# matiasrodlo/arxiv-rag

Hardware: AMD Instinct MI355X
Metric: chunks embedded/sec + QPS@top-10, all-mpnet-base-v2 768-d, 1/2/4/8 MI355X (higher is better)
Workload: dtype bf16

## Files before the change

### arxiv_rag_amd/_lib.py

```python
from __future__ import annotations

import ctypes as C
import os
from pathlib import Path

_HERE = Path(__file__).resolve().parent
LIB_PATH = Path(os.environ.get("ARX_LIB", _HERE / "libarx_hip.so"))

K_CLASSES = ["search_groupmax", "gemm_qkv", "gemm_oproj", "gemm_fc1", "gemm_fc2", "attention",
             "layernorm", "embed", "pool", "search_select", "search_rescore", "gemm_raw"]


class EncoderConfigC(C.Structure):
    _fields_ = [(n, C.c_int32) for n in ("arch", "vocab_size", "hidden", "layers", "heads", "ffn", "max_pos",
                                         "pool", "pad_id", "rel_buckets", "rel_max_distance")] + [("ln_eps", C.c_float)]


class LayerWeightsC(C.Structure):
    _fields_ = [(n, C.c_void_p) for n in ("w_qkv", "b_qkv", "w_o", "b_o", "ln1_g", "ln1_b",
                                          "w_fc1", "b_fc1", "w_fc2", "b_fc2", "ln2_g", "ln2_b")]


class EncoderWeightsC(C.Structure):
    _fields_ = [(n, C.c_void_p) for n in ("word_emb", "pos_emb", "type_emb", "emb_ln_g", "emb_ln_b", "rel_bias")] \
               + [("layers", C.POINTER(LayerWeightsC))]


class TopkOptionsC(C.Structure):
    _fields_ = [("struct_bytes", C.c_int32), ("i8_max_queries", C.c_int32), ("max_row_norm", C.c_float), ("cu_limit", C.c_int32),
                ("flags", C.c_int32), ("debug_tau_mult", C.c_float), ("debug_drop_best", C.c_int32)]

    def __init__(self, **kw):
        super().__init__(**kw)
        self.struct_bytes = C.sizeof(TopkOptionsC)


class EncoderOptionsC(C.Structure):
    _fields_ = [("struct_bytes", C.c_int32), ("gemm_schedule", C.c_int32), ("attn_kernel", C.c_int32), ("flags", C.c_int32)]

    def __init__(self, **kw):
        super().__init__(**kw)
        self.struct_bytes = C.sizeof(EncoderOptionsC)


class PairHeadC(C.Structure):
    _fields_ = [("struct_bytes", C.c_int32), ("n_labels", C.c_int32)] \
               + [(n, C.c_void_p) for n in ("type_emb", "pooler_w", "pooler_b", "cls_w", "cls_b")]

    def __init__(self, **kw):
        super().__init__(**kw)
        self.struct_bytes = C.sizeof(PairHeadC)


class GemmEpilogueC(C.Structure):
    _fields_ = [("struct_bytes", C.c_int32), ("mode", C.c_int32), ("variant", C.c_int32), ("eps", C.c_float)] \
               + [(n, C.c_void_p) for n in ("bias", "resid", "a_mean", "a_rstd", "s_vec", "r_mean", "r_rstd", "r_gamma", "r_beta")] \
               + [("row_cap", C.c_int64), ("part_sum", C.c_void_p), ("part_sq", C.c_void_p), ("part_ld", C.c_int64),
                  ("out_mean", C.c_void_p), ("out_rstd", C.c_void_p), ("n_rows", C.c_void_p)]

    def __init__(self, **kw):
        super().__init__(**kw)
        self.struct_bytes = C.sizeof(GemmEpilogueC)


class FacetKeyC(C.Structure):
    _fields_ = [("kind", C.c_void_p), ("val", C.c_void_p), ("cuts", C.c_void_p), ("mode", C.c_int32), ("want_kind", C.c_int32),
                ("n_bins", C.c_int32), ("reserved", C.c_int32), ("out_off", C.c_int64)]


FACET_CODE, FACET_EXACT, FACET_INTERVAL = 0, 1, 2
TOPK_NO_PERSISTENT, TOPK_SCAN_ONLY, TOPK_TAIL_ONLY, TOPK_NO_SINGLE_ROW_TAIL, TOPK_I8_CENTRE_QUERY = 1, 2, 4, 8, 16
GEMM_DEFAULT, GEMM_PER_TILE, GEMM_PERSISTENT, GEMM_2STAGE, GEMM_SPLIT_K, GEMM_TILE_128 = 89, 8, 9, 13, 70, 71
ATTN_TRANSPOSED, ATTN_RING, ATTN_RING16, ATTN_STAGED = 1, 2, 4, 8
ENC_EXPLICIT_LAYERNORM = 1


EXPORTS = {
    "arx_version": (C.c_int32, []),
    "arx_last_error": (C.c_char_p, []),
    "arx_build_info": (C.c_int32, []),
    "arx_mpnet_bucket": (C.c_int32, [C.c_int32, C.c_int32, C.c_int32]),
    "arx_encoder_workspace_bytes": (C.c_int64, [C.POINTER(EncoderConfigC), C.c_int32, C.c_int32]),
    "arx_encoder_create": (C.c_int32, [C.POINTER(EncoderConfigC), C.POINTER(EncoderWeightsC), C.c_int32, C.c_int32,
                                       C.POINTER(C.c_void_p)]),
    "arx_encoder_create_opt": (C.c_int32, [C.POINTER(EncoderConfigC), C.POINTER(EncoderWeightsC), C.c_int32, C.c_int32,
                                           C.POINTER(EncoderOptionsC), C.POINTER(C.c_void_p)]),
    "arx_encoder_destroy": (None, [C.c_void_p]),
    "arx_encoder_forward": (C.c_int32, [C.c_void_p, C.c_void_p, C.c_int32, C.c_void_p, C.c_int32, C.c_int32, C.c_int32,
                                        C.c_void_p, C.c_int64, C.c_void_p, C.c_int64, C.c_int32, C.c_void_p]),
    "arx_encoder_attention": (C.c_int32, [C.c_void_p, C.c_void_p, C.c_void_p, C.c_int32, C.c_int32, C.c_void_p, C.c_void_p]),
    "arx_encoder_set_tap": (C.c_int32, [C.c_void_p, C.c_int32]),
    "arx_encoder_set_low_latency": (C.c_int32, [C.c_void_p, C.c_int32]),
    "arx_encoder_debug_hidden": (C.c_int32, [C.c_void_p, C.c_int32, C.c_void_p, C.c_int32, C.c_void_p]),
    "arx_encoder_set_pair_head": (C.c_int32, [C.c_void_p, C.POINTER(PairHeadC)]),
    "arx_encoder_score_pairs": (C.c_int32, [C.c_void_p, C.c_void_p, C.c_int32, C.c_void_p, C.c_void_p, C.c_int32, C.c_int32, C.c_int32,
                                            C.c_void_p, C.c_int64, C.c_void_p]),
    "arx_encoder_debug_cls": (C.c_int32, [C.c_void_p, C.c_void_p, C.c_int32, C.c_void_p]),
    "arx_pair_head_forward": (C.c_int32, [C.c_void_p, C.c_int64, C.c_int32, C.c_int32, C.POINTER(PairHeadC), C.c_void_p, C.c_int64,
                                          C.c_void_p]),
    "arx_topk_workspace_bytes": (C.c_int64, [C.c_int64, C.c_int32, C.c_int32, C.c_int32]),
    "arx_topk_search": (C.c_int32, [C.c_void_p, C.c_int64, C.c_void_p, C.c_int32, C.c_int32, C.c_int32, C.c_void_p,
                                    C.c_void_p, C.c_int64, C.c_void_p, C.c_int64, C.c_void_p]),
    "arx_topk_i8_index_bytes": (C.c_int64, [C.c_int64, C.c_int32]),
    "arx_topk_i8_index_info": (C.c_int32, [C.c_void_p, C.c_int64, C.c_int32, C.POINTER(C.c_float), C.c_void_p]),
    "arx_topk_build_i8": (C.c_int32, [C.c_void_p, C.c_int64, C.c_int32, C.c_void_p, C.c_void_p]),
    "arx_topk_search_i8": (C.c_int32, [C.c_void_p, C.c_void_p, C.c_int64, C.c_void_p, C.c_int32, C.c_int32, C.c_int32, C.c_void_p,
                                       C.c_void_p, C.c_int64, C.c_void_p, C.c_int64, C.c_void_p]),
    "arx_topk_workspace_bytes_i8": (C.c_int64, [C.c_int64, C.c_int32, C.c_int32, C.c_int32]),
    "arx_topk_search_opt": (C.c_int32, [C.c_void_p, C.c_void_p, C.c_int64, C.c_void_p, C.c_int32, C.c_int32, C.c_int32, C.c_void_p,
                                        C.c_void_p, C.c_int64, C.c_void_p, C.c_int64, C.POINTER(TopkOptionsC), C.c_void_p]),
    "arx_rows_max_norm_f16": (C.c_int32, [C.c_void_p, C.c_int64, C.c_int32, C.c_void_p, C.c_void_p]),
    "arx_stream_create_cu_mask": (C.c_int32, [C.POINTER(C.c_uint32), C.c_int32, C.POINTER(C.c_void_p)]),
    "arx_stream_destroy": (C.c_int32, [C.c_void_p]),
    "arx_device_cu_count": (C.c_int32, []),
    "arx_debug_cu_census": (C.c_int32, [C.c_void_p, C.c_int32, C.c_int32, C.c_void_p]),
    "arx_topk_stats": (C.c_int32, [C.c_void_p, C.POINTER(C.c_int64), C.POINTER(C.c_int64), C.c_void_p]),
    "arx_topk_merge": (C.c_int32, [C.c_void_p, C.c_void_p, C.c_int32, C.c_int32, C.c_int32, C.c_void_p, C.c_void_p,
                                   C.c_void_p]),
    "arx_topk_filtered_workspace_bytes": (C.c_int64, [C.c_int64, C.c_int32, C.c_int32, C.c_int32]),
    "arx_topk_search_filtered": (C.c_int32, [C.c_void_p, C.c_int64, C.c_void_p, C.c_int64, C.c_void_p, C.c_int32, C.c_int32, C.c_int32,
                                             C.c_void_p, C.c_void_p, C.c_int64, C.c_float, C.c_void_p, C.c_int64, C.c_void_p]),
    "arx_topk_search_filtered_tuned": (C.c_int32, [C.c_void_p, C.c_int64, C.c_void_p, C.c_int64, C.c_void_p, C.c_int32, C.c_int32, C.c_int32,
                                                   C.c_void_p, C.c_void_p, C.c_int64, C.c_float, C.c_void_p, C.c_int64, C.c_int32, C.c_int32,
                                                   C.c_void_p]),
    "arx_topk_filtered_stats": (C.c_int32, [C.c_void_p, C.POINTER(C.c_int64), C.POINTER(C.c_int64), C.c_void_p]),
    "arx_topk_filtered_multi_workspace_bytes": (C.c_int64, [C.c_int64, C.c_int32, C.c_int32, C.c_int32, C.c_int32]),
    "arx_topk_search_filtered_multi": (C.c_int32, [C.c_void_p, C.c_int64, C.c_void_p, C.c_int32, C.c_void_p, C.c_void_p, C.c_void_p, C.c_int32,
                                                   C.c_int32, C.c_int32, C.c_void_p, C.c_void_p, C.c_int64, C.c_float, C.c_void_p, C.c_int64,
                                                   C.c_void_p]),
    "arx_topk_search_filtered_multi_tuned": (C.c_int32, [C.c_void_p, C.c_int64, C.c_void_p, C.c_int32, C.c_void_p, C.c_void_p, C.c_void_p,
                                                         C.c_int32, C.c_int32, C.c_int32, C.c_void_p, C.c_void_p, C.c_int64, C.c_float,
                                                         C.c_void_p, C.c_int64, C.c_int32, C.c_int32, C.c_void_p]),
    "arx_topk_filtered_multi_stats": (C.c_int32, [C.c_void_p, C.POINTER(C.c_int64), C.POINTER(C.c_int64), C.c_void_p]),
    "arx_topk_prefix_workspace_bytes": (C.c_int64, [C.c_int64, C.c_int32, C.c_int32, C.c_int32]),
    "arx_topk_search_prefix": (C.c_int32, [C.c_void_p, C.c_int64, C.c_void_p, C.c_void_p, C.c_int32, C.c_int32, C.c_int32, C.c_void_p,
                                           C.c_void_p, C.c_int64, C.c_float, C.c_void_p, C.c_int64, C.c_void_p]),
    "arx_topk_search_prefix_tuned": (C.c_int32, [C.c_void_p, C.c_int64, C.c_void_p, C.c_void_p, C.c_int32, C.c_int32, C.c_int32, C.c_void_p,
                                                 C.c_void_p, C.c_int64, C.c_float, C.c_void_p, C.c_int64, C.c_int32, C.c_int32, C.c_void_p]),
    "arx_topk_prefix_stats": (C.c_int32, [C.c_void_p, C.POINTER(C.c_int64), C.POINTER(C.c_int64), C.c_void_p]),
    "arx_topk_grouped_workspace_bytes": (C.c_int64, [C.c_int64, C.c_int32, C.c_int32, C.c_int32, C.c_int32]),
    "arx_topk_search_grouped": (C.c_int32, [C.c_void_p, C.c_int64, C.c_void_p, C.c_int64, C.c_void_p, C.c_int64, C.c_void_p, C.c_int32,
                                            C.c_int32, C.c_int32, C.c_int32, C.c_void_p, C.c_void_p, C.c_void_p, C.c_int64, C.c_float,
                                            C.c_void_p, C.c_int64, C.c_void_p]),
    "arx_topk_search_grouped_tuned": (C.c_int32, [C.c_void_p, C.c_int64, C.c_void_p, C.c_int64, C.c_void_p, C.c_int64, C.c_void_p, C.c_int32,
                                                  C.c_int32, C.c_int32, C.c_int32, C.c_void_p, C.c_void_p, C.c_void_p, C.c_int64, C.c_float,
                                                  C.c_void_p, C.c_int64, C.c_int32, C.c_int32, C.c_void_p]),
    "arx_topk_grouped_stats": (C.c_int32, [C.c_void_p, C.POINTER(C.c_int64), C.POINTER(C.c_int64), C.c_void_p]),
    "arx_group_runs_info": (C.c_int32, [C.c_void_p, C.c_int64, C.c_void_p, C.c_void_p]),
    "arx_topk_search_boosted_workspace_bytes": (C.c_int64, [C.c_int64, C.c_int32, C.c_int32, C.c_int32]),
    "arx_topk_search_boosted": (C.c_int32, [C.c_void_p, C.c_int64, C.c_void_p, C.c_float, C.c_void_p, C.c_void_p, C.c_int64, C.c_void_p,
                                            C.c_int32, C.c_int32, C.c_int32, C.c_void_p, C.c_void_p, C.c_void_p, C.c_int64, C.c_float,
                                            C.c_void_p, C.c_int64, C.c_int32, C.c_int32, C.c_void_p]),
    "arx_topk_boosted_stats": (C.c_int32, [C.c_void_p, C.POINTER(C.c_int64), C.POINTER(C.c_int64), C.c_void_p]),
    "arx_prior_info": (C.c_int32, [C.c_void_p, C.c_int64, C.c_void_p, C.c_void_p]),
    "arx_range_workspace_bytes": (C.c_int64, [C.c_int64, C.c_int32, C.c_int32, C.c_int32]),
    "arx_range_search": (C.c_int32, [C.c_void_p, C.c_int64, C.c_void_p, C.c_int64, C.c_void_p, C.c_void_p, C.c_int32, C.c_int32, C.c_int32,
                                     C.c_void_p, C.c_void_p, C.c_void_p, C.c_int64, C.c_float, C.c_void_p, C.c_int64, C.c_void_p]),
    "arx_range_search_tuned": (C.c_int32, [C.c_void_p, C.c_int64, C.c_void_p, C.c_int64, C.c_void_p, C.c_void_p, C.c_int32, C.c_int32,
                                           C.c_int32, C.c_void_p, C.c_void_p, C.c_void_p, C.c_int64, C.c_float, C.c_void_p, C.c_int64,
                                           C.c_int32, C.c_int32, C.c_void_p]),
    "arx_range_stats": (C.c_int32, [C.c_void_p, C.POINTER(C.c_int64), C.POINTER(C.c_int64), C.c_void_p]),
    "arx_text_contains":(C.c_int32, [C.c_void_p, C.c_void_p, C.c_int64, C.c_void_p, C.c_void_p, C.c_int32, C.c_void_p, C.c_void_p]),
    "arx_text_regex": (C.c_int32, [C.c_void_p, C.c_void_p, C.c_int64, C.c_void_p, C.c_void_p, C.c_int32, C.c_void_p, C.c_void_p]),
    "arx_text_regex_tuned": (C.c_int32, [C.c_void_p, C.c_void_p, C.c_int64, C.c_void_p, C.c_void_p, C.c_int32, C.c_void_p, C.c_int32,
                                         C.c_void_p]),
    "arx_bitmap_count": (C.c_int32, [C.c_void_p, C.c_int64, C.c_void_p, C.c_void_p]),
    "arx_compact_plan": (C.c_int32, [C.c_void_p, C.c_int64, C.c_void_p, C.c_void_p, C.c_void_p]),
    "arx_compact_rows": (C.c_int32, [C.c_void_p, C.c_void_p, C.c_int64, C.c_int64, C.c_void_p, C.c_void_p, C.c_void_p]),
    "arx_compact_text": (C.c_int32, [C.c_void_p, C.c_void_p, C.c_int64, C.c_void_p, C.c_void_p, C.c_void_p, C.c_void_p, C.c_void_p]),
    "arx_where_eval": (C.c_int32, [C.c_void_p, C.c_int32, C.c_int64, C.c_void_p, C.c_void_p, C.c_void_p, C.c_void_p, C.c_void_p, C.c_int64, C.c_int32,
                                   C.c_void_p, C.c_int64, C.c_void_p, C.c_void_p, C.c_void_p]),
    "arx_facet_count": (C.c_int32, [C.POINTER(FacetKeyC), C.c_int32, C.c_int64, C.c_void_p, C.c_int64, C.c_int32, C.c_void_p, C.c_int64,
                                    C.c_void_p]),
    "arx_facet_count_tuned": (C.c_int32, [C.POINTER(FacetKeyC), C.c_int32, C.c_int64, C.c_void_p, C.c_int64, C.c_int32, C.c_void_p, C.c_int64,
                                          C.c_int32, C.c_int32, C.c_int32, C.c_void_p]),
    "arx_cluster_sums_workspace_bytes": (C.c_int64, [C.c_int64, C.c_int32, C.c_int32]),
    "arx_cluster_sums": (C.c_int32, [C.c_void_p, C.c_int64, C.c_int32, C.c_void_p, C.c_int64, C.c_void_p, C.c_int32, C.c_void_p, C.c_int64,
                                     C.c_void_p, C.c_void_p]),
    "arx_cluster_sums_tuned": (C.c_int32, [C.c_void_p, C.c_int64, C.c_int32, C.c_void_p, C.c_int64, C.c_void_p, C.c_int32, C.c_void_p, C.c_int64,
                                           C.c_void_p, C.c_int32, C.c_int32, C.c_void_p]),
    "arx_cluster_finish": (C.c_int32, [C.c_void_p, C.c_void_p, C.c_void_p, C.c_int32, C.c_int32, C.c_void_p, C.c_void_p, C.c_void_p]),
    "arx_cluster_assign_workspace_bytes": (C.c_int64, [C.c_int64, C.c_int32, C.c_int32]),
    "arx_cluster_assign": (C.c_int32, [C.c_void_p, C.c_int64, C.c_int32, C.c_void_p, C.c_int32, C.c_float, C.c_void_p, C.c_void_p, C.c_void_p,
                                       C.c_void_p, C.c_int64, C.c_void_p]),
    "arx_cluster_assign_tuned": (C.c_int32, [C.c_void_p, C.c_int64, C.c_int32, C.c_void_p, C.c_int32, C.c_float, C.c_void_p, C.c_void_p, C.c_void_p,
                                             C.c_void_p, C.c_int64, C.c_float, C.c_int32, C.c_void_p]),
    "arx_ivf_workspace_bytes": (C.c_int64, [C.c_int64, C.c_int32, C.c_int32, C.c_int32, C.c_int32, C.c_int32]),
    "arx_ivf_search": (C.c_int32, [C.c_void_p, C.c_int64, C.c_int32, C.c_void_p, C.c_int64, C.c_void_p, C.c_int32, C.c_int64, C.c_void_p,
                                   C.c_int32, C.c_void_p, C.c_int32, C.c_void_p, C.c_int32, C.c_void_p, C.c_void_p, C.c_void_p, C.c_int64,
                                   C.c_void_p, C.c_int64, C.c_void_p]),
    "arx_ivf_search_tuned": (C.c_int32, [C.c_void_p, C.c_int64, C.c_int32, C.c_void_p, C.c_int64, C.c_void_p, C.c_int32, C.c_int64, C.c_void_p,
                                         C.c_int32, C.c_void_p, C.c_int32, C.c_void_p, C.c_int32, C.c_void_p, C.c_void_p, C.c_void_p,
                                         C.c_int64, C.c_void_p, C.c_int64, C.c_int32, C.c_void_p]),
    "arx_ivf_multi_workspace_bytes": (C.c_int64, [C.c_int64, C.c_int32, C.c_int32, C.c_int32, C.c_int32, C.c_int32]),
    "arx_ivf_search_multi": (C.c_int32, [C.c_void_p, C.c_int64, C.c_int32, C.c_void_p, C.c_int64, C.c_void_p, C.c_int32, C.c_int64, C.c_void_p,
                                         C.c_int32, C.c_void_p, C.c_int32, C.c_void_p, C.c_int32, C.c_void_p, C.c_void_p, C.c_int32, C.c_void_p,
                                         C.c_void_p, C.c_void_p, C.c_void_p, C.c_int64, C.c_void_p, C.c_int64, C.c_void_p]),
    "arx_ivf_search_multi_tuned": (C.c_int32, [C.c_void_p, C.c_int64, C.c_int32, C.c_void_p, C.c_int64, C.c_void_p, C.c_int32, C.c_int64,
                                               C.c_void_p, C.c_int32, C.c_void_p, C.c_int32, C.c_void_p, C.c_int32, C.c_void_p, C.c_void_p,
                                               C.c_int32, C.c_void_p, C.c_void_p, C.c_void_p, C.c_void_p, C.c_int64, C.c_void_p, C.c_int64,
                                               C.c_int32, C.c_void_p]),
    "arx_binary_pack": (C.c_int32, [C.c_void_p, C.c_int64, C.c_int32, C.c_void_p, C.c_void_p, C.c_void_p]),
    "arx_binary_workspace_bytes": (C.c_int64, [C.c_int64, C.c_int32, C.c_int32, C.c_int32]),
    "arx_binary_candidates": (C.c_int32, [C.c_void_p, C.c_int64, C.c_int32, C.c_void_p, C.c_int32, C.c_void_p, C.c_int32, C.c_void_p, C.c_void_p,
                                          C.c_void_p, C.c_void_p, C.c_int64, C.c_void_p]),
    "arx_binary_candidates_tuned": (C.c_int32, [C.c_void_p, C.c_int64, C.c_int32, C.c_void_p, C.c_int32, C.c_void_p, C.c_int32, C.c_void_p,
                                                C.c_void_p, C.c_void_p, C.c_void_p, C.c_int64, C.c_int32, C.c_void_p]),
    "arx_pq_encode": (C.c_int32, [C.c_void_p, C.c_int64, C.c_int32, C.c_int32, C.c_void_p, C.c_void_p, C.c_void_p, C.c_void_p]),
    "arx_pq_lut": (C.c_int32, [C.c_void_p, C.c_int32, C.c_int32, C.c_int32, C.c_void_p, C.c_void_p, C.c_void_p]),
    "arx_pq_workspace_bytes": (C.c_int64, [C.c_int64, C.c_int32, C.c_int32, C.c_int32, C.c_int32]),
    "arx_pq_candidates": (C.c_int32, [C.c_void_p, C.c_int64, C.c_int32, C.c_int32, C.c_void_p, C.c_int32, C.c_void_p, C.c_int32, C.c_void_p,
                                      C.c_void_p, C.c_void_p, C.c_void_p, C.c_int64, C.c_void_p]),
    "arx_pq_candidates_tuned": (C.c_int32, [C.c_void_p, C.c_int64, C.c_int32, C.c_int32, C.c_void_p, C.c_int32, C.c_void_p, C.c_int32,
                                            C.c_void_p, C.c_void_p, C.c_void_p, C.c_void_p, C.c_int64, C.c_int32, C.c_void_p]),
    "arx_gather_rows": (C.c_int32, [C.c_void_p, C.c_int64, C.c_int32, C.c_int64, C.c_void_p, C.c_int64, C.c_void_p, C.c_void_p]),
    "arx_mmr_select": (C.c_int32, [C.c_void_p, C.c_void_p, C.c_void_p, C.c_int32, C.c_int32, C.c_int32, C.c_int32, C.c_float, C.c_void_p,
                                   C.c_void_p, C.c_void_p]),
    "arx_bm25_workspace_bytes": (C.c_int64, [C.c_int64, C.c_int32, C.c_int32]),
    "arx_bm25_search": (C.c_int32, [C.c_void_p, C.c_void_p, C.c_void_p, C.c_int32, C.c_int64, C.c_void_p, C.c_void_p, C.c_int32, C.c_int32,
                                    C.c_void_p, C.c_void_p, C.c_int64, C.c_void_p, C.c_int64, C.c_void_p]),
    "arx_bm25_search_tuned": (C.c_int32, [C.c_void_p, C.c_void_p, C.c_void_p, C.c_int32, C.c_int64, C.c_void_p, C.c_void_p, C.c_int32,
                                          C.c_int32, C.c_void_p, C.c_void_p, C.c_int64, C.c_void_p, C.c_int64, C.c_int32, C.c_int32,
                                          C.c_void_p]),
    "arx_bm25_search_filtered": (C.c_int32, [C.c_void_p, C.c_void_p, C.c_void_p, C.c_int32, C.c_int64, C.c_void_p, C.c_int32, C.c_void_p,
                                             C.c_void_p, C.c_void_p, C.c_int32, C.c_int32, C.c_void_p, C.c_void_p, C.c_int64, C.c_void_p,
                                             C.c_int64, C.c_void_p]),
    "arx_bm25_search_filtered_tuned": (C.c_int32, [C.c_void_p, C.c_void_p, C.c_void_p, C.c_int32, C.c_int64, C.c_void_p, C.c_int32, C.c_void_p,
                                                   C.c_void_p, C.c_void_p, C.c_int32, C.c_int32, C.c_void_p, C.c_void_p, C.c_int64,
                                                   C.c_void_p, C.c_int64, C.c_int32, C.c_int32, C.c_void_p]),
    "arx_bm25_wide_workspace_bytes": (C.c_int64, [C.c_int64, C.c_int32, C.c_int32]),
    "arx_bm25_search_wide": (C.c_int32, [C.c_void_p, C.c_void_p, C.c_void_p, C.c_int32, C.c_int64, C.c_void_p, C.c_int32, C.c_void_p,
                                         C.c_void_p, C.c_void_p, C.c_int32, C.c_int32, C.c_void_p, C.c_void_p, C.c_int64, C.c_void_p,
                                         C.c_int64, C.c_int32, C.c_int32, C.c_void_p]),
    "arx_hybrid_fuse": (C.c_int32, [C.c_void_p, C.c_void_p, C.c_int32, C.c_void_p, C.c_void_p, C.c_int32, C.c_int32, C.c_double, C.c_int32,
                                    C.c_void_p, C.c_void_p, C.c_void_p, C.c_void_p, C.c_void_p]),
    "arx_bm25_scores": (C.c_int32, [C.c_void_p, C.c_void_p, C.c_void_p, C.c_int32, C.c_int64, C.c_void_p, C.c_int32, C.c_int64, C.c_int64,
                                    C.c_int32, C.c_void_p, C.c_void_p]),
    "arx_bm25_build_workspace_bytes": (C.c_int64, [C.c_int64, C.c_int64, C.c_int32]),
    "arx_bm25_build_postings": (C.c_int32, [C.c_void_p, C.c_int64, C.c_void_p, C.c_int64, C.c_int32, C.c_void_p, C.c_void_p, C.c_void_p,
                                            C.c_void_p, C.c_void_p, C.c_void_p, C.c_int64, C.c_void_p]),
    "arx_bm25_build_postings_tuned": (C.c_int32, [C.c_void_p, C.c_int64, C.c_void_p, C.c_int64, C.c_int32, C.c_void_p, C.c_void_p, C.c_void_p,
                                                  C.c_void_p, C.c_void_p, C.c_void_p, C.c_int64, C.c_int32, C.c_int32, C.c_void_p]),
    "arx_bm25_build_impacts": (C.c_int32, [C.c_void_p, C.c_void_p, C.c_void_p, C.c_int64, C.c_void_p, C.c_int64, C.c_void_p, C.c_int32,
                                           C.c_double, C.c_void_p, C.c_void_p]),
    "arx_gemm_bf16": (C.c_int32, [C.c_void_p, C.c_void_p, C.c_void_p, C.c_void_p, C.c_void_p, C.c_int32, C.c_int32, C.c_int32,
                                  C.c_int32, C.c_int32, C.c_void_p]),
    "arx_gemm_bf16_ex": (C.c_int32, [C.c_void_p, C.c_void_p, C.c_void_p, C.c_int32, C.c_int32, C.c_int32, C.POINTER(GemmEpilogueC),
                                     C.c_void_p]),
    "arx_fold_ln": (C.c_int32, [C.c_void_p, C.c_void_p, C.c_void_p, C.c_void_p, C.c_void_p, C.c_void_p, C.c_void_p, C.c_int32, C.c_int32,
                                C.c_void_p]),
    "arx_prof_classes": (C.c_int32, [C.c_uint32]),
    "arx_wp_create": (C.c_int32, [C.c_char_p, C.c_void_p, C.c_int32, C.c_int32, C.c_int32, C.c_int32, C.c_int32, C.c_int32, C.c_int32,
                                  C.c_char_p, C.c_void_p, C.c_int32, C.POINTER(C.c_void_p)]),
    "arx_wp_destroy": (None, [C.c_void_p]),
    "arx_wp_encode": (C.c_int32, [C.c_void_p, C.c_char_p, C.c_void_p, C.c_int64, C.c_int32, C.c_void_p, C.c_void_p, C.c_void_p, C.c_int32]),
    "arx_wp_miss_count": (C.c_int32, [C.c_void_p, C.POINTER(C.c_int64), C.POINTER(C.c_int64)]),
    "arx_wp_miss_fetch": (C.c_int32, [C.c_void_p, C.c_void_p, C.c_void_p]),
    "arx_wp_cache_add": (C.c_int32, [C.c_void_p, C.c_char_p, C.c_void_p, C.c_int64, C.c_void_p, C.c_void_p]),
    "arx_wp_cache_size": (C.c_int64, [C.c_void_p]),
    "arx_wp_version": (C.c_int32, []),
    "arx_adjacent_cosine": (C.c_int32, [C.c_void_p, C.c_int64, C.c_int32, C.c_int32, C.c_void_p, C.c_void_p]),
    "arx_f32_to_bf16": (C.c_int32, [C.c_void_p, C.c_void_p, C.c_int64, C.c_void_p]),
    "arx_fill_unit_rows_f16": (C.c_int32, [C.c_void_p, C.c_int64, C.c_int32, C.c_uint64, C.c_void_p]),
    "arx_fill_unit_rows_f16_at": (C.c_int32, [C.c_void_p, C.c_int64, C.c_int32, C.c_uint64, C.c_int64, C.c_void_p]),
    "arx_fill_clustered_rows_f16_at": (C.c_int32, [C.c_void_p, C.c_int64, C.c_int32, C.c_uint64, C.c_int64, C.c_int32, C.c_float, C.c_int32,
                                                   C.c_float, C.c_void_p]),
    "arx_prof_enable": (C.c_int32, [C.c_int32]),
    "arx_prof_reset": (C.c_int32, []),
    "arx_prof_read": (C.c_int32, [C.c_int32, C.POINTER(C.c_float), C.POINTER(C.c_int32)]),
}

_lib = None


class ArxError(RuntimeError):
    pass


def load():
    global _lib
    if _lib is not None:
        return _lib
    if not LIB_PATH.exists():
        raise ArxError(
            f"{LIB_PATH} not found: the HIP extension is not built. Run `python -c 'import __graft_entry__ as g; "
            f"g.build()'` (or arxiv_rag_amd/csrc/build.sh). There is no CPU fallback for this path.")
    lib = C.CDLL(str(LIB_PATH))
    for name, (res, args) in EXPORTS.items():
        fn = getattr(lib, name)
        fn.restype = res
        fn.argtypes = args
    _lib = lib
    return lib


def check(rc: int, what: str = ""):
    if rc != 0:
        msg = load().arx_last_error().decode("utf-8", "replace")
        raise ArxError(f"{what} failed (rc={rc}): {msg}")


def prof_classes(names=None):
    mask = 0xFFFFFFFF if names is None else sum(1 << K_CLASSES.index(n) for n in names)
    check(load().arx_prof_classes(mask), "arx_prof_classes")


def prof_enable(on: bool):
    check(load().arx_prof_enable(1 if on else 0), "arx_prof_enable")


def prof_reset():
    check(load().arx_prof_reset(), "arx_prof_reset")


def prof_read():
    lib = load()
    out = {}
    for i, name in enumerate(K_CLASSES):
        ms, n = C.c_float(0), C.c_int32(0)
        check(lib.arx_prof_read(i, C.byref(ms), C.byref(n)), "arx_prof_read")
        out[name] = (float(ms.value), int(n.value))
    return out
```

### arxiv_rag_amd/csrc/encoder.hip

```cpp
#include <math.h>
#include <stdlib.h>
#include <string.h>

#include <mutex>
#include <vector>

#include "arx_common.h"
#include "encoder_kernels.h"
#include "gemm.h"
#include "gemm8.h"
#include "gemm_small.h"

extern "C" int32_t arx_mpnet_bucket(int32_t rel, int32_t num_buckets, int32_t max_distance) {
    int n = -rel;
    const int nb = num_buckets / 2;
    int ret = 0;
    if (n < 0) { ret = nb; n = -n; }
    const int max_exact = nb / 2;
    if (n < max_exact) return ret + n;
    int v = max_exact + (int)floor(log((double)n / max_exact) / log((double)max_distance / max_exact) * (nb - max_exact) + 1e-6);
    if (v > nb - 1) v = nb - 1;
    return ret + v;
}

struct arx_encoder {
    arx_encoder_config cfg;
    arx_encoder_weights w;
    std::vector<arx_layer_weights> layers;
    int max_tokens, max_seqs, tok_pad;
    char* ws = nullptr;
    int64_t ws_bytes = 0;
    int32_t* cu = nullptr;
    uint16_t *x = nullptr, *x1 = nullptr, *qkv = nullptr, *ctx = nullptr, *y = nullptr, *hbuf = nullptr;
    float* bias_tbl = nullptr;
    uint16_t* tap = nullptr;
    int tap_layer = -1;
    int ln_fold = 1;
    char* fold_ws = nullptr;
    std::vector<uint16_t*> wqkv_f, wfc1_f;
    std::vector<float*> s_qkv, c_qkv, s_fc1, c_fc1;
    float *st1_sum = nullptr, *st1_sq = nullptr, *st2_sum = nullptr, *st2_sq = nullptr;
    float *part_s = nullptr, *part_q = nullptr;
    int variant = ARX_GEMM_DEFAULT;
    int low_latency = 0;
    float* small_ws = nullptr;
    int attn_variant = ARX_ATTN_TRANSPOSED;
    int attn_dev_word = 0;
    unsigned long long* attn_stamps = nullptr;
    arx_pair_head pair{};
    int has_pair = 0;
    float* cls_ws = nullptr;
};

struct WsLayout {
    int64_t cu, x, x1, qkv, ctx, y, hbuf, bias, stats, total;
};
static WsLayout ws_layout(const arx_encoder_config& c, int max_tokens, int max_seqs) {
    const int64_t tp = round_up64(max_tokens, 256);
    WsLayout l;
    int64_t o = 0;
    auto take = [&](int64_t bytes) { int64_t r = o; o += round_up64(bytes, 256); return r; };
    l.cu = take((int64_t)(max_seqs + 1) * 4);
    l.x = take(tp * c.hidden * 2);
    l.x1 = take(tp * c.hidden * 2);
    l.qkv = take(tp * c.hidden * 3 * 2);
    l.ctx = take(tp * c.hidden * 2);
    l.y = take(tp * c.hidden * 2);
    l.hbuf = take(tp * c.ffn * 2);
    l.bias = take((int64_t)c.heads * ARX_BIAS_ROW * 4);
    l.stats = take(tp * 4 * 4 + 2 * (int64_t)(c.hidden / 64) * tp * 4);
    l.total = o;
    return l;
}

static int check_cfg(const arx_encoder_config* c) {
    ARX_REQUIRE(c != nullptr, "cfg is null");
    ARX_REQUIRE(c->arch == ARX_ARCH_MPNET || c->arch == ARX_ARCH_BERT, "unknown arch %d", c->arch);
    ARX_REQUIRE(c->hidden > 0 && c->hidden % 64 == 0 && c->hidden <= 1024, "hidden=%d must be a multiple of 64, <= 1024", c->hidden);
    ARX_REQUIRE(c->heads > 0 && c->hidden % c->heads == 0, "hidden %% heads != 0");
    const int dh = c->hidden / c->heads;
    ARX_REQUIRE(dh == 32 || dh == 64, "head_dim=%d unsupported (32 or 64)", dh);
    ARX_REQUIRE(c->ffn > 0 && c->ffn % 64 == 0, "ffn=%d must be a multiple of 64", c->ffn);
    ARX_REQUIRE(c->layers > 0 && c->vocab_size > 0 && c->max_pos > 0, "bad layers/vocab/max_pos");
    ARX_REQUIRE(c->pool == ARX_POOL_MEAN || c->pool == ARX_POOL_CLS, "unknown pool %d", c->pool);
    return ARX_OK;
}

extern "C" int64_t arx_encoder_workspace_bytes(const arx_encoder_config* cfg, int32_t max_tokens, int32_t max_seqs) {
    if (check_cfg(cfg) != ARX_OK || max_tokens <= 0 || max_seqs <= 0) return -1;
    return ws_layout(*cfg, max_tokens, max_seqs).total;
}

static int check_options(const arx_encoder_options* o) {
    if (!o) return ARX_OK;
    ARX_REQUIRE(o->struct_bytes == (int32_t)sizeof(arx_encoder_options), "arx_encoder_options: struct_bytes=%d, this library expects %d",
                o->struct_bytes, (int)sizeof(arx_encoder_options));
    const int g = o->gemm_schedule, a = o->attn_kernel;
    bool gemm_ok = g == 0 || g == ARX_GEMM_DEFAULT || g == ARX_GEMM_PER_TILE || g == ARX_GEMM_PERSISTENT || g == ARX_GEMM_2STAGE || g == ARX_GEMM_TILE_128;
    bool attn_ok = a == 0 || a == ARX_ATTN_TRANSPOSED || a == ARX_ATTN_STAGED;
#ifdef ARX_DEV_VARIANTS
    gemm_ok = gemm_ok || g == 1 || g == 2 || g == 3 || g == 4 || g == 15 || g == 33 || g == 34;
    attn_ok = attn_ok || a == ARX_ATTN_RING || a == ARX_ATTN_RING16;
#endif
    ARX_REQUIRE(gemm_ok, "arx_encoder_options.gemm_schedule=%d is not a whole-forward GEMM schedule of this build (ARX_GEMM_* in arx.h)", g);
    ARX_REQUIRE(attn_ok, "arx_encoder_options.attn_kernel=%d is not an attention kernel of this build (ARX_ATTN_* in arx.h)", a);
    ARX_REQUIRE((o->flags & ~ARX_ENC_EXPLICIT_LAYERNORM) == 0, "arx_encoder_options.flags=0x%x has unknown bits", o->flags);
    return ARX_OK;
}

extern "C" int32_t arx_encoder_create(const arx_encoder_config* cfg, const arx_encoder_weights* w, int32_t max_tokens,
                                      int32_t max_seqs, arx_encoder** out) {
    return arx_encoder_create_opt(cfg, w, max_tokens, max_seqs, nullptr, out);
}

extern "C" int32_t arx_encoder_create_opt(const arx_encoder_config* cfg, const arx_encoder_weights* w, int32_t max_tokens,
                                          int32_t max_seqs, const arx_encoder_options* opt, arx_encoder** out) {
    int rc = check_cfg(cfg);
    if (rc != ARX_OK) return rc;
    if ((rc = check_options(opt)) != ARX_OK) return rc;
    ARX_REQUIRE(w && out, "null weights/out");
    ARX_REQUIRE(max_tokens > 0 && max_seqs > 0, "max_tokens/max_seqs must be positive");
    ARX_REQUIRE(w->word_emb && w->pos_emb && w->emb_ln_g && w->emb_ln_b && w->layers, "missing embedding weights");
    ARX_REQUIRE(cfg->arch != ARX_ARCH_BERT || w->type_emb, "BERT needs type_emb");
    ARX_REQUIRE(cfg->arch != ARX_ARCH_MPNET || w->rel_bias, "MPNet needs rel_bias");
    for (int i = 0; i < cfg->layers; ++i) {
        const arx_layer_weights& L = w->layers[i];
        ARX_REQUIRE(L.w_qkv && L.b_qkv && L.w_o && L.b_o && L.ln1_g && L.ln1_b && L.w_fc1 && L.b_fc1 && L.w_fc2 &&
                        L.b_fc2 && L.ln2_g && L.ln2_b, "layer %d: missing weights", i);
    }
    arx_encoder* h = new arx_encoder();
    auto fail = [&](int code) {
        if (h->ws) (void)hipFree(h->ws);
        if (h->fold_ws) (void)hipFree(h->fold_ws);
        delete h;
        return code;
    };
    h->cfg = *cfg;
    h->w = *w;
    h->layers.assign(w->layers, w->layers + cfg->layers);
    h->w.layers = h->layers.data();
    h->max_tokens = max_tokens;
    h->max_seqs = max_seqs;
    h->tok_pad = (int)round_up64(max_tokens, 256);
    if (opt && opt->gemm_schedule) h->variant = opt->gemm_schedule;
    if (opt && opt->attn_kernel) h->attn_variant = opt->attn_kernel;
    h->ln_fold = !(opt && (opt->flags & ARX_ENC_EXPLICIT_LAYERNORM));
    const WsLayout l = ws_layout(*cfg, max_tokens, max_seqs);
    hipError_t he = hipMalloc((void**)&h->ws, l.total);
    if (he != hipSuccess) {
        arx_set_error("hipMalloc(%lld bytes workspace): %s", (long long)l.total, hipGetErrorString(he));
        h->ws = nullptr;
        return fail(ARX_ERR_HIP);
    }
    h->ws_bytes = l.total;
    (void)hipMemset(h->ws, 0, l.total);
    h->cu = (int32_t*)(h->ws + l.cu);
    h->x = (uint16_t*)(h->ws + l.x);
    h->x1 = (uint16_t*)(h->ws + l.x1);
    h->qkv = (uint16_t*)(h->ws + l.qkv);
    h->ctx = (uint16_t*)(h->ws + l.ctx);
    h->y = (uint16_t*)(h->ws + l.y);
    h->hbuf = (uint16_t*)(h->ws + l.hbuf);
    h->bias_tbl = (float*)(h->ws + l.bias);
    {
        const int64_t tp = round_up64(max_tokens, 256);
        float* st = (float*)(h->ws + l.stats);
        h->st1_sum = st; h->st1_sq = st + tp; h->st2_sum = st + 2 * tp; h->st2_sq = st + 3 * tp;
        h->part_s = st + 4 * tp; h->part_q = h->part_s + (int64_t)(cfg->hidden / 64) * tp;
    }
    if (h->ln_fold) {
        const int64_t H = cfg->hidden, F = cfg->ffn, Lc = cfg->layers;
        const int64_t per = round_up64(3 * H * H * 2, 256) + round_up64(F * H * 2, 256) + 2 * round_up64(3 * H * 4, 256) + 2 * round_up64(F * 4, 256);
        he = hipMalloc((void**)&h->fold_ws, per * Lc);
        if (he != hipSuccess) {
            arx_set_error("hipMalloc(folded weights): %s", hipGetErrorString(he));
            h->fold_ws = nullptr;
            return fail(ARX_ERR_HIP);
        }
        char* pws = h->fold_ws;
        auto takep = [&](int64_t bytes) { char* r = pws; pws += round_up64(bytes, 256); return r; };
        for (int i = 0; i < Lc; ++i) {
            const arx_layer_weights& L = h->layers[i];
            uint16_t* wq = (uint16_t*)takep(3 * H * H * 2); uint16_t* w1 = (uint16_t*)takep(F * H * 2);
            float* sq = (float*)takep(3 * H * 4); float* cq = (float*)takep(3 * H * 4);
            float* s1 = (float*)takep(F * 4); float* c1 = (float*)takep(F * 4);
            h->wqkv_f.push_back(wq); h->wfc1_f.push_back(w1);
            h->s_qkv.push_back(sq); h->c_qkv.push_back(cq); h->s_fc1.push_back(s1); h->c_fc1.push_back(c1);
            fold_ln_kernel<<<cdiv(F, 4), 256>>>((const uint16_t*)L.w_fc1, L.ln1_g, L.ln1_b, L.b_fc1, w1, s1, c1, (int)F, (int)H);
            if (i > 0) {
                const arx_layer_weights& P = h->layers[i - 1];
                fold_ln_kernel<<<cdiv(3 * H, 4), 256>>>((const uint16_t*)L.w_qkv, P.ln2_g, P.ln2_b, L.b_qkv, wq, sq, cq, (int)(3 * H), (int)H);
            }
        }
        he = hipDeviceSynchronize();
        if (he != hipSuccess) {
            arx_set_error("fold_ln_kernel: %s", hipGetErrorString(he));
            return fail(ARX_ERR_HIP);
        }
    }
    if (cfg->arch == ARX_ARCH_MPNET) {
        std::vector<float> rb((size_t)cfg->rel_buckets * cfg->heads);
        he = hipMemcpy(rb.data(), w->rel_bias, rb.size() * 4, hipMemcpyDeviceToHost);
        if (he != hipSuccess) {
            arx_set_error("copy rel_bias: %s", hipGetErrorString(he));
            return fail(ARX_ERR_HIP);
        }
        std::vector<float> tbl((size_t)cfg->heads * ARX_BIAS_ROW);
        const float log2e = 1.4426950408889634f;
        for (int d = -ARX_BIAS_CENTER; d <= ARX_BIAS_CENTER; ++d) {
            const int bk = arx_mpnet_bucket(d, cfg->rel_buckets, cfg->rel_max_distance);
            for (int hd = 0; hd < cfg->heads; ++hd)
                tbl[(size_t)hd * ARX_BIAS_ROW + d + ARX_BIAS_CENTER] = rb[(size_t)bk * cfg->heads + hd] * log2e;
        }
        he = hipMemcpy(h->bias_tbl, tbl.data(), tbl.size() * 4, hipMemcpyHostToDevice);
        if (he != hipSuccess) {
            arx_set_error("upload bias table: %s", hipGetErrorString(he));
            return fail(ARX_ERR_HIP);
        }
    }
    *out = h;
    return ARX_OK;
}

extern "C" void arx_encoder_destroy(arx_encoder* h) {
    if (!h) return;
    if (h->ws) (void)hipFree(h->ws);
    if (h->tap) (void)hipFree(h->tap);
    if (h->fold_ws) (void)hipFree(h->fold_ws);
    if (h->small_ws) (void)hipFree(h->small_ws);
    if (h->cls_ws) (void)hipFree(h->cls_ws);
    delete h;
}

extern "C" int32_t arx_encoder_set_low_latency(arx_encoder* h, int32_t on) {
    ARX_REQUIRE(h, "null handle");
    if (on && !h->small_ws) ARX_HIP_CHECK(hipMalloc((void**)&h->small_ws, ARX_SMALL_WS_BYTES));
    h->low_latency = on ? 1 : 0;
    return ARX_OK;
}

extern "C" int32_t arx_encoder_set_tap(arx_encoder* h, int32_t layer) {
    ARX_REQUIRE(h, "null handle");
    ARX_REQUIRE(layer >= -1 && layer <= h->cfg.layers, "tap layer out of range");
    if (layer >= 0 && !h->tap) ARX_HIP_CHECK(hipMalloc((void**)&h->tap, (int64_t)h->tok_pad * h->cfg.hidden * 2));
    h->tap_layer = layer;
    return ARX_OK;
}

extern "C" int32_t arx_encoder_debug_hidden(arx_encoder* h, int32_t , float* dst, int32_t n_tokens, void* stream) {
    ARX_REQUIRE(h && h->tap && dst, "no tap recorded");
    ARX_REQUIRE(n_tokens > 0 && n_tokens <= h->max_tokens, "n_tokens out of range");
    const int64_t n = (int64_t)n_tokens * h->cfg.hidden;
    bf16_to_f32_kernel<<<cdiv(n, 256), 256, 0, (hipStream_t)stream>>>(h->tap, dst, n);
    ARX_HIP_CHECK(hipGetLastError());
    return ARX_OK;
}

template <typename Kern>
static int launch_gemm_kernel(Kern kern, int smem, int threads, int BM, int BN, const uint16_t* A, int64_t lda,
                              const uint16_t* W, int64_t ldw, int M, int N, int K, const EpiParams& ep, hipStream_t st) {
    ARX_HIP_CHECK(arx_func_smem((const void*)kern, smem));
    const int tm = cdiv(M, BM), tn = cdiv(N, BN);
    kern<<<tm * tn, threads, smem, st>>>((const bf16_t*)A, lda, (const bf16_t*)W, ldw, M, N, K, tm, tn, ep);
    ARX_HIP_CHECK(hipGetLastError());
    return ARX_OK;
}

static bool fits_u32_offsets(int64_t M, int64_t lda, int64_t N, int64_t ldw, const EpiParams& ep) {
    return M * lda < (1ll << 31) && N * ldw < (1ll << 31) && M * ep.ldc < (1ll << 32) && (!ep.resid || M * ep.ldr < (1ll << 32));
}

template <int MODE>
int arx_launch_gemm(int variant, const uint16_t* A, int64_t lda, const uint16_t* W, int64_t ldw, int M, int N, int K,
                    const EpiParams& ep, hipStream_t st) {
    if (K % 64 != 0 || N % 8 != 0) {
        arx_set_error("gemm: K=%d must be a multiple of 64 and N=%d of 8", K, N);
        return ARX_ERR_ARG;
    }
    const bool wide = (N % 256 == 0);
    const bool wide8 = (N % 128 == 0 && N >= 256);
#ifdef ARX_DEV_VARIANTS
    if constexpr (MODE <= EPI_BIAS_RESID) {
        if (variant == 0) {
            if (wide) return launch_gemm_kernel(gemm_bf16_kernel<256, 256, 2, 4, true, MODE>, GemmMainloop<bf16_t, 256, 256, 2, 4, true>::SMEM_BYTES, 512, 256, 256, A, lda, W, ldw, M, N, K, ep, st);
            return launch_gemm_kernel(gemm_bf16_kernel<256, 128, 4, 2, true, MODE>, GemmMainloop<bf16_t, 256, 128, 4, 2, true>::SMEM_BYTES, 512, 256, 128, A, lda, W, ldw, M, N, K, ep, st);
        }
        if (variant == 4) {
            if (wide) return launch_gemm_kernel(gemm_bf16_kernel<256, 256, 2, 4, false, MODE>, GemmMainloop<bf16_t, 256, 256, 2, 4, false>::SMEM_BYTES, 512, 256, 256, A, lda, W, ldw, M, N, K, ep, st);
            return launch_gemm_kernel(gemm_bf16_kernel<256, 128, 4, 2, false, MODE>, GemmMainloop<bf16_t, 256, 128, 4, 2, false>::SMEM_BYTES, 512, 256, 128, A, lda, W, ldw, M, N, K, ep, st);
        }
    }
#endif
    if (variant == ARX_GEMM_TILE_128)
        return launch_gemm_kernel(gemm_v0e2_kernel<128, 128, 2, 2, MODE, 67>, GemmMainloop<bf16_t, 128, 128, 2, 2, true, 67>::SMEM_BYTES, 256, 128, 128, A, lda, W, ldw, M, N, K, ep, st);
    if (variant == ARX_GEMM_DEFAULT) variant = (K <= 1024) ? ARX_GEMM_PERSISTENT : ARX_GEMM_PER_TILE;
    if (variant == ARX_GEMM_PERSISTENT && (K / 64) % 2 != 0) variant = ARX_GEMM_PER_TILE;
    if ((variant == ARX_GEMM_PER_TILE || variant == ARX_GEMM_PERSISTENT) && wide8 && !fits_u32_offsets(M, lda, N, ldw, ep)) {
        static bool said = false;
        if (!said) {
            said = true;
            fprintf(stderr, "[arx] gemm M=%d N=%d K=%d: operand or output offsets exceed 32 bits, using the 2-stage kernel (64-bit offsets)\n", M, N, K);
        }
        variant = ARX_GEMM_2STAGE;
    }
    if (variant == ARX_GEMM_PERSISTENT && wide8) {
        auto kern = gemm_8phase_persistent_kernel<MODE>;
        ARX_HIP_CHECK(arx_func_smem((const void*)kern, Gemm8Phase<bf16_t, 0>::SMEM_BYTES));
        const int n_cu = arx_device_cus();
        const int tm = cdiv(M, 256), tn = cdiv(N, 256);
        int grid = TileWalk::grid(tm, tn) < n_cu ? TileWalk::grid(tm, tn) : n_cu;
        grid = grid / 8 * 8 > 0 ? grid / 8 * 8 : grid;
        kern<<<grid, 512, Gemm8Phase<bf16_t, 0>::SMEM_BYTES, st>>>((const bf16_t*)A, lda, (const bf16_t*)W, ldw, M, N, K, tm, tn, ep);
        ARX_HIP_CHECK(hipGetLastError());
        return ARX_OK;
    }
    if (variant == ARX_GEMM_PER_TILE && wide8) {
        auto kern = gemm_8phase_kernel<MODE>;
        ARX_HIP_CHECK(arx_func_smem((const void*)kern, Gemm8Phase<bf16_t, 0>::SMEM_BYTES));
        const int tm = cdiv(M, 256), tn = cdiv(N, 256);
        kern<<<TileWalk::grid(tm, tn), 512, Gemm8Phase<bf16_t, 0>::SMEM_BYTES, st>>>((const bf16_t*)A, lda, (const bf16_t*)W, ldw, M, N, K, tm, tn, ep);
        ARX_HIP_CHECK(hipGetLastError());
        return ARX_OK;
    }
#ifdef ARX_DEV_VARIANTS
    if (variant == 34 && wide)
        return launch_gemm_kernel(gemm_v0e2_kernel<256, 256, 2, 4, MODE, 64 + 4096>, GemmMainloop<bf16_t, 256, 256, 2, 4, true, 64 + 4096>::SMEM_BYTES, 512, 256, 256, A, lda, W, ldw, M, N, K, ep, st);
    if (variant == 33 && wide)
        return launch_gemm_kernel(gemm_a3w2_kernel<256, 256, 2, 4, MODE>, 3 * 256 * 128 + 2 * 256 * 128, 512, 256, 256, A, lda, W, ldw, M, N, K, ep, st);
    if (variant == 1) {
        if (wide) return launch_gemm_kernel(gemm_v0e2_kernel<256, 256, 2, 4, MODE>, GemmMainloop<bf16_t, 256, 256, 2, 4, true>::SMEM_BYTES, 512, 256, 256, A, lda, W, ldw, M, N, K, ep, st);
        return launch_gemm_kernel(gemm_v0e2_kernel<256, 128, 4, 2, MODE>, GemmMainloop<bf16_t, 256, 128, 4, 2, true>::SMEM_BYTES, 512, 256, 128, A, lda, W, ldw, M, N, K, ep, st);
    }
    if (variant == 15 && wide)
        return launch_gemm_kernel(gemm_v0e2_kernel<256, 256, 2, 4, MODE, 3>, GemmMainloop<bf16_t, 256, 256, 2, 4, true, 3>::SMEM_BYTES, 512, 256, 256, A, lda, W, ldw, M, N, K, ep, st);
    if (variant == 3 && wide)
        return launch_gemm_kernel(gemm_ring_kernel<256, 256, 2, 4, 4, MODE>, GemmRing<bf16_t, 256, 256, 2, 4, 4>::SMEM_BYTES, 512, 256, 256, A, lda, W, ldw, M, N, K, ep, st);
    if (variant == 2 || variant == 3)
        return launch_gemm_kernel(gemm_ring_kernel<256, 128, 2, 2, 3, MODE>, GemmRing<bf16_t, 256, 128, 2, 2, 3>::SMEM_BYTES, 256, 256, 128, A, lda, W, ldw, M, N, K, ep, st);
#endif
    if (!wide) return launch_gemm_kernel(gemm_v0e2_kernel<256, 128, 4, 2, MODE, 67>, GemmMainloop<bf16_t, 256, 128, 4, 2, true, 67>::SMEM_BYTES, 512, 256, 128, A, lda, W, ldw, M, N, K, ep, st);
    return launch_gemm_kernel(gemm_v0e2_kernel<256, 256, 2, 4, MODE, 67>, GemmMainloop<bf16_t, 256, 256, 2, 4, true, 67>::SMEM_BYTES, 512, 256, 256, A, lda, W, ldw, M, N, K, ep, st);
}

template <int MODE>
static int launch_gemm(int cls, int variant, const uint16_t* A, int64_t lda, const uint16_t* W, int64_t ldw, int M, int N, int K,
                       const EpiParams& ep, hipStream_t st, float* small_ws = nullptr) {
    ProfScope ps(cls, st);
    if (variant == ARX_GEMM_SPLIT_K) return launch_gemm_small<MODE>(A, lda, W, ldw, M, N, K, ep, small_ws, st);
#ifdef ARX_DEV_VARIANTS
    static const int dev_bw = getenv("ARX_DEV_BW") ? atoi(getenv("ARX_DEV_BW")) : 0;
    const char* stg = getenv("ARX_DEV_STAGGER");
    if (dev_bw || stg) {
        EpiParams e2 = ep; e2.dev_bw = dev_bw;
        if (stg) { int a = 0, b = 8, c = 0; sscanf(stg, "%d,%d,%d", &a, &b, &c); e2.dev_stagger = a; e2.dev_slots = b > 0 ? b : 8; e2.dev_store = c; }
        return arx_launch_gemm<MODE>(variant, A, lda, W, ldw, M, N, K, e2, st);
    }
#endif
    return arx_launch_gemm<MODE>(variant, A, lda, W, ldw, M, N, K, ep, st);
}

extern "C" int32_t arx_gemm_bf16(const void* A, const void* W, const float* bias, const void* resid, void* C, int32_t M,
                                 int32_t N, int32_t K, int32_t mode, int32_t variant, void* stream) {
    ARX_REQUIRE(A && W && bias && C, "null pointer argument");
    ARX_REQUIRE(M > 0 && N > 0 && K > 0, "bad sizes");
    ARX_REQUIRE(mode != EPI_BIAS_RESID || resid, "mode 2 needs resid");
    EpiParams ep{(uint16_t*)C, N, bias, (const uint16_t*)resid, N};
    hipStream_t st = (hipStream_t)stream;
#ifdef ARX_DEV_VARIANTS
    ep.dev_store = (variant / 100) % 10; ep.dev_bw = variant / 1000; variant %= 100;
    if (const char* stg = getenv("ARX_DEV_STAGGER")) { int a = 0, b = 8; sscanf(stg, "%d,%d", &a, &b); ep.dev_stagger = a; ep.dev_slots = b > 0 ? b : 8; }
#endif
#ifdef ARX_STAMP
    {
        static unsigned long long* d = nullptr;
        const int tiles = cdiv(M, 256) * cdiv(N, 256);
        if (!d) ARX_HIP_CHECK(hipMalloc(&d, (size_t)8 * 32 * 2 * 16384));
        if (getenv("ARX_STAMP_DUMP") && tiles <= 16384) {
            ep.stamps = d;
            int rc = ARX_ERR_ARG;
            if (mode == EPI_BIAS) rc = arx_launch_gemm<EPI_BIAS>(variant, (const uint16_t*)A, K, (const uint16_t*)W, K, M, N, K, ep, st);
            if (mode == EPI_BIAS_GELU) rc = arx_launch_gemm<EPI_BIAS_GELU>(variant, (const uint16_t*)A, K, (const uint16_t*)W, K, M, N, K, ep, st);
            if (mode == EPI_BIAS_RESID) rc = arx_launch_gemm<EPI_BIAS_RESID>(variant, (const uint16_t*)A, K, (const uint16_t*)W, K, M, N, K, ep, st);
            ARX_HIP_CHECK(hipStreamSynchronize(st));
            std::vector<unsigned long long> hbuf((size_t)tiles * 64);
            ARX_HIP_CHECK(hipMemcpy(hbuf.data(), d, hbuf.size() * 8, hipMemcpyDeviceToHost));
            double loop[2] = {0, 0}, epi[2] = {0, 0}, pro[2] = {0, 0}, x45[2] = {0, 0}, x67[2] = {0, 0};
            unsigned long long tmin = ~0ull, tmax = 0;
            for (int t = 0; t < tiles; ++t)
                for (int g = 0; g < 2; ++g) {
                    const unsigned long long* o = &hbuf[((size_t)t * 2 + g) * 32];
                    loop[g] += (double)(o[1] - o[3]); epi[g] += (double)(o[2] - o[1]); pro[g] += (double)(o[3] - o[0]);
                    if (variant == 9) { x45[g] += (double)(o[5] - o[4]); x67[g] += (double)(o[7] - o[6]); }
                    else x45[g] += (double)(o[4] - o[2]);
                    tmin = o[0] < tmin ? o[0] : tmin; tmax = o[2] > tmax ? o[2] : tmax;
                }
            if (variant == 9) {
                double gap = 0, period = 0; int n = 0;
                for (int t = 0; t + 256 < tiles; ++t) { const unsigned long long* a = &hbuf[(size_t)t * 64]; const unsigned long long* b = &hbuf[(size_t)(t + 256) * 64];
                    gap += (double)(b[0] - a[2]); period += (double)(b[0] - a[0]); ++n; }
                if (n) fprintf(stderr, "[stamp] persistent: g0 tile period %.0f clk, epilogue-end -> next loop start %.0f clk\n", period / n, gap / n);
            }
            if (const char* sf = getenv("ARX_STAMP_FILE")) {
                if (FILE* f = fopen(sf, "wb")) { fwrite(hbuf.data(), 8, hbuf.size(), f); fclose(f); }
            }
            if (variant == 9) {
                const int nkt = K / 64 < 16 ? K / 64 : 16;
                fprintf(stderr, "[stamp] k-tile durations g0:");
                for (int k = 0; k + 1 < nkt; ++k) { double a = 0; int n = 0; for (int t = 256; t < tiles; ++t) { const unsigned long long* o = &hbuf[(size_t)t * 64]; a += (double)(o[9 + k] - o[8 + k]); ++n; } fprintf(stderr, " %.0f", a / (n ? n : 1)); }
                fprintf(stderr, "\n");
            }
            fprintf(stderr, "[stamp] %s g0 %.0f g1 %.0f clk%s g0 %.0f g1 %.0f\n", variant == 9 ? "wait at k-tile 0:" : "store drain after the epilogue:", x45[0] / tiles, x45[1] / tiles,
                    variant == 9 ? ", at k-tile 1:" : " (-)", x67[0] / tiles, x67[1] / tiles);
            fprintf(stderr, "[stamp] M=%d N=%d K=%d mode=%d tiles=%d: prologue %.0f / %.0f, loop g0 %.0f g1 %.0f clk, epilogue g0 %.0f g1 %.0f clk, span %.0f clk, tiles/CU %.1f\n",
                    M, N, K, mode, tiles, pro[0] / tiles, pro[1] / tiles, loop[0] / tiles, loop[1] / tiles, epi[0] / tiles, epi[1] / tiles, (double)(tmax - tmin), tiles / 256.0);
            return rc;
        }
    }
#endif
    ProfScope ps(ARX_K_GEMM_RAW, st);
    if (variant == ARX_GEMM_SPLIT_K) {
        float* ws = nullptr;
        ARX_HIP_CHECK(hipMallocAsync((void**)&ws, ARX_SMALL_WS_BYTES, st));
        int rc = ARX_ERR_ARG;
        switch (mode) {
        case EPI_BIAS: rc = launch_gemm_small<EPI_BIAS>((const uint16_t*)A, K, (const uint16_t*)W, K, M, N, K, ep, ws, st); break;
        case EPI_BIAS_GELU: rc = launch_gemm_small<EPI_BIAS_GELU>((const uint16_t*)A, K, (const uint16_t*)W, K, M, N, K, ep, ws, st); break;
        case EPI_BIAS_RESID: rc = launch_gemm_small<EPI_BIAS_RESID>((const uint16_t*)A, K, (const uint16_t*)W, K, M, N, K, ep, ws, st); break;
        default: arx_set_error("unknown gemm mode %d", mode);
        }
        (void)hipFreeAsync(ws, st);
        return rc;
    }
    switch (mode) {
    case EPI_BIAS: return arx_launch_gemm<EPI_BIAS>(variant, (const uint16_t*)A, K, (const uint16_t*)W, K, M, N, K, ep, st);
    case EPI_BIAS_GELU: return arx_launch_gemm<EPI_BIAS_GELU>(variant, (const uint16_t*)A, K, (const uint16_t*)W, K, M, N, K, ep, st);
    case EPI_BIAS_RESID: return arx_launch_gemm<EPI_BIAS_RESID>(variant, (const uint16_t*)A, K, (const uint16_t*)W, K, M, N, K, ep, st);
    }
    arx_set_error("unknown gemm mode %d", mode);
    return ARX_ERR_ARG;
}

template <int DH, bool HB, int NW>
static int launch_attn_cfg(arx_encoder* h, int n_seqs, int max_len, hipStream_t st) {
    auto kern = attention_kernel<DH, HB, NW>;
    const int Lk = (max_len + 31) & ~31;
    const int smem = AttnSmem<DH>::total(Lk, HB);
    ARX_HIP_CHECK(arx_func_smem((const void*)kern, smem));
    const float scale_log2e = 1.4426950408889634f / sqrtf((float)DH);
    dim3 grid(cdiv(max_len, 32 * NW), h->cfg.heads, n_seqs);
    ProfScope ps(ARX_K_ATTENTION, st);
    kern<<<grid, NW * 64, smem, st>>>(h->qkv, h->ctx, h->cu, h->bias_tbl, h->cfg.hidden, scale_log2e);
    ARX_HIP_CHECK(hipGetLastError());
    return ARX_OK;
}

template <int DH, bool HB, int NW>
static int launch_attn_tr_cfg(arx_encoder* h, int n_seqs, int max_len, hipStream_t st) {
    auto kern = attention_tr_kernel<DH, HB, NW>;
    const int Lk = (max_len + 31) & ~31;
    const int smem = AttnSmem3<DH>::total(Lk, HB);
    ARX_HIP_CHECK(arx_func_smem((const void*)kern, smem));
    const float scale_log2e = 1.4426950408889634f / sqrtf((float)DH);
    dim3 grid(cdiv(max_len, 32 * NW), h->cfg.heads, n_seqs);
    ProfScope ps(ARX_K_ATTENTION, st);
    kern<<<grid, NW * 64, smem, st>>>(h->qkv, h->ctx, h->cu, h->bias_tbl, h->cfg.hidden, scale_log2e, h->attn_dev_word, h->attn_stamps);
    ARX_HIP_CHECK(hipGetLastError());
    return ARX_OK;
}

#ifdef ARX_DEV_VARIANTS
template <int DH, bool HB, int NSLOT>
static int launch_attn_ring_cfg(arx_encoder* h, int n_seqs, int max_len, hipStream_t st) {
    auto kern = attention_ring_kernel<DH, HB, NSLOT>;
    const int C0 = (max_len + 31) & ~31;
    const int smem = AttnRing<DH, NSLOT>::total(C0, HB);
    ARX_HIP_CHECK(arx_func_smem((const void*)kern, smem));
    int G = arx_device_cus() / h->cfg.heads;
    G = G < 1 ? 1 : (G > n_seqs ? n_seqs : G);
    const float scale_log2e = 1.4426950408889634f / sqrtf((float)DH);
    ProfScope ps(ARX_K_ATTENTION, st);
    kern<<<G * h->cfg.heads, 512, smem, st>>>(h->qkv, h->ctx, h->cu, h->bias_tbl, h->cfg.hidden, n_seqs, C0, scale_log2e);
    ARX_HIP_CHECK(hipGetLastError());
    return ARX_OK;
}

template <bool HB>
static int launch_attn_ring16_cfg(arx_encoder* h, int n_seqs, int max_len, hipStream_t st) {
    auto kern = attention_ring16_kernel<HB>;
    const int C0 = (max_len + 31) & ~31;
    const int smem = AttnRing16<8>::total(C0, HB);
    ARX_HIP_CHECK(arx_func_smem((const void*)kern, smem));
    int G = arx_device_cus() / h->cfg.heads;
    G = G < 1 ? 1 : (G > n_seqs ? n_seqs : G);
    const float scale_log2e = 1.4426950408889634f / sqrtf(64.0f);
    ProfScope ps(ARX_K_ATTENTION, st);
    kern<<<G * h->cfg.heads, 1024, smem, st>>>(h->qkv, h->ctx, h->cu, h->bias_tbl, h->cfg.hidden, n_seqs, C0, scale_log2e);
    ARX_HIP_CHECK(hipGetLastError());
    return ARX_OK;
}

#endif

static int launch_attn(arx_encoder* h, int n_seqs, int max_len, hipStream_t st) {
    const int dh = h->cfg.hidden / h->cfg.heads;
    const bool hb = h->cfg.arch == ARX_ARCH_MPNET;
#ifdef ARX_DEV_VARIANTS
    if (h->attn_variant == ARX_ATTN_RING16 && dh == 64 && max_len > 128 && max_len <= 256)
        return hb ? launch_attn_ring16_cfg<true>(h, n_seqs, max_len, st) : launch_attn_ring16_cfg<false>(h, n_seqs, max_len, st);
    if (h->attn_variant == ARX_ATTN_RING && max_len > 128 && max_len <= 256) {
        if (dh == 64) return hb ? launch_attn_ring_cfg<64, true, 8>(h, n_seqs, max_len, st) : launch_attn_ring_cfg<64, false, 8>(h, n_seqs, max_len, st);
        return hb ? launch_attn_ring_cfg<32, true, 8>(h, n_seqs, max_len, st) : launch_attn_ring_cfg<32, false, 8>(h, n_seqs, max_len, st);
    }
#endif
    if (h->attn_variant != ARX_ATTN_STAGED) {
        const bool w8 = max_len > 128;
        if (dh == 64) {
            if (hb) return w8 ? launch_attn_tr_cfg<64, true, 8>(h, n_seqs, max_len, st) : launch_attn_tr_cfg<64, true, 4>(h, n_seqs, max_len, st);
            return w8 ? launch_attn_tr_cfg<64, false, 8>(h, n_seqs, max_len, st) : launch_attn_tr_cfg<64, false, 4>(h, n_seqs, max_len, st);
        }
        if (hb) return w8 ? launch_attn_tr_cfg<32, true, 8>(h, n_seqs, max_len, st) : launch_attn_tr_cfg<32, true, 4>(h, n_seqs, max_len, st);
        return w8 ? launch_attn_tr_cfg<32, false, 8>(h, n_seqs, max_len, st) : launch_attn_tr_cfg<32, false, 4>(h, n_seqs, max_len, st);
    }
    const bool big = max_len > 256;
    if (dh == 64) {
        if (hb) return big ? launch_attn_cfg<64, true, 8>(h, n_seqs, max_len, st) : launch_attn_cfg<64, true, 4>(h, n_seqs, max_len, st);
        return big ? launch_attn_cfg<64, false, 8>(h, n_seqs, max_len, st) : launch_attn_cfg<64, false, 4>(h, n_seqs, max_len, st);
    }
    if (hb) return big ? launch_attn_cfg<32, true, 8>(h, n_seqs, max_len, st) : launch_attn_cfg<32, true, 4>(h, n_seqs, max_len, st);
    return big ? launch_attn_cfg<32, false, 8>(h, n_seqs, max_len, st) : launch_attn_cfg<32, false, 4>(h, n_seqs, max_len, st);
}

extern "C" int32_t arx_encoder_attention(arx_encoder* h, const void* qkv, const int32_t* lens, int32_t n_seqs, int32_t max_len,
                                         void* ctx, void* stream) {
    ARX_REQUIRE(h && qkv && lens && ctx, "null pointer argument");
    ARX_REQUIRE(n_seqs > 0 && n_seqs <= h->max_seqs && max_len > 0 && max_len <= 512, "bad n_seqs/max_len");
    hipStream_t st = (hipStream_t)stream;
    scan_lens_kernel<<<1, 256, 0, st>>>(lens, h->cu, n_seqs);
    ARX_HIP_CHECK(hipGetLastError());
    uint16_t* q0 = h->qkv; uint16_t* c0 = h->ctx;
    h->qkv = (uint16_t*)qkv; h->ctx = (uint16_t*)ctx;
    const int rc = launch_attn(h, n_seqs, max_len, st);
    h->qkv = q0; h->ctx = c0;
    return rc;
}

static void launch_ln_finalize(int T, int nparts, const float* ps, const float* pq, int64_t ld, const int32_t* n_rows, float inv_h,
                               float eps, float* mean, float* rstd, hipStream_t st) {
    const int grid = cdiv(T, 256);
    switch (nparts) {
    case 6: ln_finalize_kernel<6><<<grid, 256, 0, st>>>(ps, pq, ld, nparts, n_rows, inv_h, eps, mean, rstd); break;
    case 12: ln_finalize_kernel<12><<<grid, 256, 0, st>>>(ps, pq, ld, nparts, n_rows, inv_h, eps, mean, rstd); break;
    case 16: ln_finalize_kernel<16><<<grid, 256, 0, st>>>(ps, pq, ld, nparts, n_rows, inv_h, eps, mean, rstd); break;
    default: ln_finalize_kernel<0><<<grid, 256, 0, st>>>(ps, pq, ld, nparts, n_rows, inv_h, eps, mean, rstd); break;
    }
}

template <int MODE>
static int gemm_ex_run(int variant, const uint16_t* A, const uint16_t* W, int M, int N, int K, const EpiParams& ep, const arx_gemm_epilogue* e,
                       hipStream_t st) {
    constexpr bool STATS = (MODE == EPI_RESID_STATS || MODE == EPI_LNRESID_STATS);
    int rc;
    if (variant == ARX_GEMM_SPLIT_K) {
        float* ws = nullptr;
        ARX_HIP_CHECK(hipMallocAsync((void**)&ws, ARX_SMALL_WS_BYTES, st));
        rc = launch_gemm<MODE>(ARX_K_GEMM_RAW, variant, A, K, W, K, M, N, K, ep, st, ws);
        (void)hipFreeAsync(ws, st);
        return rc;
    }
    if ((rc = launch_gemm<MODE>(ARX_K_GEMM_RAW, variant, A, K, W, K, M, N, K, ep, st)) != ARX_OK) return rc;
    if (STATS) {
        launch_ln_finalize(M, N / 64, e->part_sum, e->part_sq, e->part_ld, e->n_rows, ep.inv_h, ep.eps, e->out_mean, e->out_rstd, st);
        ARX_HIP_CHECK(hipGetLastError());
    }
    return ARX_OK;
}

extern "C" int32_t arx_gemm_bf16_ex(const void* A, const void* W, void* C, int32_t M, int32_t N, int32_t K, const arx_gemm_epilogue* e,
                                    void* stream) {
    ARX_REQUIRE(A && W && C && e, "null pointer argument");
    ARX_REQUIRE(e->struct_bytes == (int32_t)sizeof(arx_gemm_epilogue), "arx_gemm_epilogue: struct_bytes=%d, this library expects %d",
                e->struct_bytes, (int)sizeof(arx_gemm_epilogue));
    ARX_REQUIRE(M > 0 && N > 0 && K > 0, "bad sizes");
    ARX_REQUIRE(K % 64 == 0 && N % 8 == 0, "gemm: K=%d must be a multiple of 64 and N=%d of 8", K, N);
    const int mode = e->mode, variant = e->variant;
    ARX_REQUIRE(mode >= EPI_BIAS && mode <= EPI_LNRESID_STATS, "unknown gemm mode %d", mode);
    ARX_REQUIRE(variant == ARX_GEMM_DEFAULT || variant == ARX_GEMM_PER_TILE || variant == ARX_GEMM_PERSISTENT || variant == ARX_GEMM_2STAGE ||
                    variant == ARX_GEMM_SPLIT_K || variant == ARX_GEMM_TILE_128,
                "gemm variant %d is not a shipped schedule (89, 8, 9, 13, 70, 71)", variant);
    const bool ln_in = (mode == EPI_LN_BIAS || mode == EPI_LN_BIAS_GELU), stats = (mode == EPI_RESID_STATS || mode == EPI_LNRESID_STATS);
    const bool staged = (variant == ARX_GEMM_DEFAULT || variant == ARX_GEMM_PER_TILE || variant == ARX_GEMM_PERSISTENT);
    ARX_REQUIRE(e->bias, "mode %d needs bias", mode);
    ARX_REQUIRE(!(mode == EPI_BIAS_RESID || stats) || e->resid, "mode %d needs resid", mode);
    ARX_REQUIRE(!ln_in || (e->a_mean && e->a_rstd && e->s_vec), "mode %d needs a_mean, a_rstd and s_vec", mode);
    ARX_REQUIRE(mode != EPI_LNRESID_STATS || (e->r_mean && e->r_rstd && e->r_gamma && e->r_beta), "mode 6 needs r_mean, r_rstd, r_gamma and r_beta");
    if (ln_in || mode == EPI_LNRESID_STATS)
        ARX_REQUIRE(e->row_cap >= (staged ? round_up64(M, 256) : (int64_t)M),
                    "row_cap=%lld: the row vectors must be readable up to row %lld (M=%d%s)", (long long)e->row_cap,
                    (long long)(staged ? round_up64(M, 256) : (int64_t)M), M, staged ? " rounded up to 256: variants 89, 8, 9 stage whole tiles" : "");
    if (stats) {
        ARX_REQUIRE(N % 64 == 0, "statistics modes need N %% 64 == 0 (one partial per 64-column slice), N=%d", N);
        ARX_REQUIRE(e->out_mean && e->out_rstd, "mode %d needs out_mean and out_rstd", mode);
        if (variant != ARX_GEMM_SPLIT_K) ARX_REQUIRE(e->part_sum && e->part_sq && e->part_ld >= M && e->n_rows,
                                       "mode %d on a tile kernel needs part_sum, part_sq, part_ld >= M and n_rows", mode);
    }
    if (variant == ARX_GEMM_SPLIT_K) {
        ARX_REQUIRE(M <= ARX_SMALL_M && N % 64 == 0, "small-batch gemm: M=%d (<= %d) N=%d (%% 64)", M, ARX_SMALL_M, N);
        ARX_REQUIRE(!stats || N <= 1024, "small-batch gemm: statistics modes take N <= 1024, N=%d", N);
    }
    EpiParams ep{(uint16_t*)C, N, e->bias, (const uint16_t*)e->resid, N};
    ep.a_sum = e->a_mean; ep.a_sq = e->a_rstd; ep.s_vec = e->s_vec;
    ep.r_sum = e->r_mean; ep.r_sq = e->r_rstd; ep.r_gamma = e->r_gamma; ep.r_beta = e->r_beta;
    ep.o_sum = e->part_sum; ep.o_sq = e->part_sq; ep.o_ld = e->part_ld;
    ep.fin_mean = e->out_mean; ep.fin_rstd = e->out_rstd;
    ep.inv_h = 1.0f / (float)N; ep.eps = e->eps;
    hipStream_t st = (hipStream_t)stream;
    const uint16_t* a = (const uint16_t*)A; const uint16_t* w = (const uint16_t*)W;
    switch (mode) {
    case EPI_BIAS: return gemm_ex_run<EPI_BIAS>(variant, a, w, M, N, K, ep, e, st);
    case EPI_BIAS_GELU: return gemm_ex_run<EPI_BIAS_GELU>(variant, a, w, M, N, K, ep, e, st);
    case EPI_BIAS_RESID: return gemm_ex_run<EPI_BIAS_RESID>(variant, a, w, M, N, K, ep, e, st);
    case EPI_LN_BIAS: return gemm_ex_run<EPI_LN_BIAS>(variant, a, w, M, N, K, ep, e, st);
    case EPI_LN_BIAS_GELU: return gemm_ex_run<EPI_LN_BIAS_GELU>(variant, a, w, M, N, K, ep, e, st);
    case EPI_RESID_STATS: return gemm_ex_run<EPI_RESID_STATS>(variant, a, w, M, N, K, ep, e, st);
    default: return gemm_ex_run<EPI_LNRESID_STATS>(variant, a, w, M, N, K, ep, e, st);
    }
}

extern "C" int32_t arx_fold_ln(const void* W, const float* gamma, const float* beta, const float* bias, void* Wf, float* s, float* c,
                               int32_t N, int32_t K, void* stream) {
    ARX_REQUIRE(W && gamma && beta && bias && Wf && s && c, "null pointer argument");
    ARX_REQUIRE(N > 0 && K > 0, "bad sizes");
    fold_ln_kernel<<<cdiv(N, 4), 256, 0, (hipStream_t)stream>>>((const uint16_t*)W, gamma, beta, bias, (uint16_t*)Wf, s, c, (int)N, (int)K);
    ARX_HIP_CHECK(hipGetLastError());
    return ARX_OK;
}

static int32_t encoder_run(arx_encoder* h, const int32_t* ids, int32_t seq_stride, const int32_t* lens, const int32_t* seg_b,
                           int32_t n_seqs, int32_t max_len, int32_t total_tokens, float* out_f32,
                           int64_t out_stride, void* out_f16, int64_t out16_stride, int32_t normalize,
                           void* stream) {
    ARX_REQUIRE(h && ids && lens, "null handle/ids/lens");
    ARX_REQUIRE(out_f32 || out_f16, "no output buffer");
    ARX_REQUIRE(n_seqs > 0 && max_len > 0 && max_len <= 512, "n_seqs=%d max_len=%d (max_len must be in 1..512)", n_seqs, max_len);
    ARX_REQUIRE(seq_stride >= max_len, "seq_stride < max_len");
    ARX_REQUIRE(total_tokens > 0 && (int64_t)total_tokens <= (int64_t)n_seqs * max_len, "total_tokens out of range");
    if (n_seqs > h->max_seqs || total_tokens > h->max_tokens) {
        arx_set_error("batch (%d seqs, %d tokens) exceeds handle capacity (%d, %d)", n_seqs, total_tokens, h->max_seqs, h->max_tokens);
        return ARX_ERR_CAPACITY;
    }
    ARX_REQUIRE(!out_f32 || out_stride >= h->cfg.hidden, "out_stride < hidden");
    ARX_REQUIRE(!out_f16 || out16_stride >= h->cfg.hidden, "out16_stride < hidden");
    hipStream_t st = (hipStream_t)stream;
    const arx_encoder_config& c = h->cfg;
    const int H = c.hidden, F = c.ffn, T = total_tokens;
    int rc;

    scan_lens_kernel<<<1, 256, 0, st>>>(lens, h->cu, n_seqs);
    ARX_HIP_CHECK(hipGetLastError());
    {
        ProfScope ps(ARX_K_EMBED, st);
        dim3 grid(cdiv(max_len, 4), n_seqs);
        if (c.arch == ARX_ARCH_MPNET)
            embed_ln_kernel<ARX_ARCH_MPNET><<<grid, 256, 0, st>>>(ids, seq_stride, lens, h->cu, h->w.word_emb, h->w.pos_emb, nullptr,
                                                                  h->w.emb_ln_g, h->w.emb_ln_b, h->x, H, c.vocab_size, c.max_pos, c.pad_id, c.ln_eps);
        else if (seg_b)
            embed_ln_kernel<ARX_ARCH_BERT, true><<<grid, 256, 0, st>>>(ids, seq_stride, lens, h->cu, h->w.word_emb, h->w.pos_emb,
                                                                       h->pair.type_emb, h->w.emb_ln_g, h->w.emb_ln_b, h->x, H,
                                                                       c.vocab_size, c.max_pos, c.pad_id, c.ln_eps, seg_b);
        else
            embed_ln_kernel<ARX_ARCH_BERT><<<grid, 256, 0, st>>>(ids, seq_stride, lens, h->cu, h->w.word_emb, h->w.pos_emb, h->w.type_emb,
                                                                 h->w.emb_ln_g, h->w.emb_ln_b, h->x, H, c.vocab_size, c.max_pos, c.pad_id, c.ln_eps);
        ARX_HIP_CHECK(hipGetLastError());
    }
    const int ln_grid = cdiv(T, 4);
    const int64_t tp = round_up64(h->max_tokens, 256);
    if (!h->ln_fold) {
        auto tap = [&](int layer) -> int {
            if (h->tap_layer == layer && h->tap) ARX_HIP_CHECK(hipMemcpyAsync(h->tap, h->x, (int64_t)T * H * 2, hipMemcpyDeviceToDevice, st));
            return ARX_OK;
        };
        if ((rc = tap(0)) != ARX_OK) return rc;
        for (int li = 0; li < c.layers; ++li) {
            const arx_layer_weights& L = h->layers[li];
            EpiParams ep;
            ep = EpiParams{h->qkv, 3 * (int64_t)H, L.b_qkv, nullptr, 0};
            if ((rc = launch_gemm<EPI_BIAS>(ARX_K_GEMM_QKV, h->variant, h->x, H, (const uint16_t*)L.w_qkv, H, T, 3 * H, H, ep, st)) != ARX_OK) return rc;
            if ((rc = launch_attn(h, n_seqs, max_len, st)) != ARX_OK) return rc;
            ep = EpiParams{h->y, H, L.b_o, h->x, H};
            if ((rc = launch_gemm<EPI_BIAS_RESID>(ARX_K_GEMM_OPROJ, h->variant, h->ctx, H, (const uint16_t*)L.w_o, H, T, H, H, ep, st)) != ARX_OK) return rc;
            { ProfScope ps(ARX_K_LAYERNORM, st);
              layernorm_kernel<<<ln_grid, 256, 0, st>>>(h->y, h->x1, L.ln1_g, L.ln1_b, h->cu + n_seqs, H, c.ln_eps); }
            ARX_HIP_CHECK(hipGetLastError());
            ep = EpiParams{h->hbuf, F, L.b_fc1, nullptr, 0};
            if ((rc = launch_gemm<EPI_BIAS_GELU>(ARX_K_GEMM_FC1, h->variant, h->x1, H, (const uint16_t*)L.w_fc1, H, T, F, H, ep, st)) != ARX_OK) return rc;
            ep = EpiParams{h->y, H, L.b_fc2, h->x1, H};
            if ((rc = launch_gemm<EPI_BIAS_RESID>(ARX_K_GEMM_FC2, h->variant, h->hbuf, F, (const uint16_t*)L.w_fc2, F, T, H, F, ep, st)) != ARX_OK) return rc;
            { ProfScope ps(ARX_K_LAYERNORM, st);
              layernorm_kernel<<<ln_grid, 256, 0, st>>>(h->y, h->x, L.ln2_g, L.ln2_b, h->cu + n_seqs, H, c.ln_eps); }
            ARX_HIP_CHECK(hipGetLastError());
            if ((rc = tap(li + 1)) != ARX_OK) return rc;
        }
        ProfScope pps(ARX_K_POOL, st);
        pool_norm_kernel<<<n_seqs, 256, 0, st>>>(h->x, h->cu, H, c.pool, normalize, out_f32, out_stride, (f16_t*)out_f16, out16_stride,
                                                 nullptr, nullptr, nullptr, nullptr, 0.f);
        ARX_HIP_CHECK(hipGetLastError());
        return ARX_OK;
    }

    const float inv_h = 1.0f / (float)H;
    const int gv = !h->low_latency ? h->variant : (T <= ARX_SMALL_M ? ARX_GEMM_SPLIT_K : (T <= ARX_MEDIUM_M ? ARX_GEMM_TILE_128 : h->variant));
    if (h->tap_layer == 0 && h->tap) ARX_HIP_CHECK(hipMemcpyAsync(h->tap, h->x, (int64_t)T * H * 2, hipMemcpyDeviceToDevice, st));
    for (int li = 0; li < c.layers; ++li) {
        const arx_layer_weights& L = h->layers[li];
        EpiParams ep;
        if (li == 0) {
            ep = EpiParams{h->qkv, 3 * (int64_t)H, L.b_qkv, nullptr, 0};
            if ((rc = launch_gemm<EPI_BIAS>(ARX_K_GEMM_QKV, gv, h->x, H, (const uint16_t*)L.w_qkv, H, T, 3 * H, H, ep, st, h->small_ws)) != ARX_OK) return rc;
        } else {
            ep = EpiParams{h->qkv, 3 * (int64_t)H, h->c_qkv[li], nullptr, 0};
            ep.a_sum = h->st2_sum; ep.a_sq = h->st2_sq; ep.s_vec = h->s_qkv[li]; ep.inv_h = inv_h; ep.eps = c.ln_eps;
            if ((rc = launch_gemm<EPI_LN_BIAS>(ARX_K_GEMM_QKV, gv, h->x, H, h->wqkv_f[li], H, T, 3 * H, H, ep, st, h->small_ws)) != ARX_OK) return rc;
        }
        if ((rc = launch_attn(h, n_seqs, max_len, st)) != ARX_OK) return rc;
        ep = EpiParams{h->x1, H, L.b_o, h->x, H};
        ep.o_sum = h->part_s; ep.o_sq = h->part_q; ep.o_ld = tp; ep.inv_h = inv_h; ep.eps = c.ln_eps;
        ep.fin_mean = h->st1_sum; ep.fin_rstd = h->st1_sq;
        if (li == 0) {
            if ((rc = launch_gemm<EPI_RESID_STATS>(ARX_K_GEMM_OPROJ, gv, h->ctx, H, (const uint16_t*)L.w_o, H, T, H, H, ep, st, h->small_ws)) != ARX_OK) return rc;
        } else {
            const arx_layer_weights& P = h->layers[li - 1];
            ep.r_sum = h->st2_sum; ep.r_sq = h->st2_sq; ep.r_gamma = P.ln2_g; ep.r_beta = P.ln2_b;
            if ((rc = launch_gemm<EPI_LNRESID_STATS>(ARX_K_GEMM_OPROJ, gv, h->ctx, H, (const uint16_t*)L.w_o, H, T, H, H, ep, st, h->small_ws)) != ARX_OK) return rc;
        }
        if (gv != ARX_GEMM_SPLIT_K) { ProfScope ps(ARX_K_LAYERNORM, st);
          launch_ln_finalize(T, H / 64, h->part_s, h->part_q, tp, h->cu + n_seqs, inv_h, c.ln_eps, h->st1_sum, h->st1_sq, st); }
        ARX_HIP_CHECK(hipGetLastError());
        ep = EpiParams{h->hbuf, F, h->c_fc1[li], nullptr, 0};
        ep.a_sum = h->st1_sum; ep.a_sq = h->st1_sq; ep.s_vec = h->s_fc1[li]; ep.inv_h = inv_h; ep.eps = c.ln_eps;
        if ((rc = launch_gemm<EPI_LN_BIAS_GELU>(ARX_K_GEMM_FC1, gv, h->x1, H, h->wfc1_f[li], H, T, F, H, ep, st, h->small_ws)) != ARX_OK) return rc;
        ep = EpiParams{h->x, H, L.b_fc2, h->x1, H};
        ep.r_sum = h->st1_sum; ep.r_sq = h->st1_sq; ep.r_gamma = L.ln1_g; ep.r_beta = L.ln1_b;
        ep.o_sum = h->part_s; ep.o_sq = h->part_q; ep.o_ld = tp; ep.inv_h = inv_h; ep.eps = c.ln_eps;
        ep.fin_mean = h->st2_sum; ep.fin_rstd = h->st2_sq;
        if ((rc = launch_gemm<EPI_LNRESID_STATS>(ARX_K_GEMM_FC2, gv, h->hbuf, F, (const uint16_t*)L.w_fc2, F, T, H, F, ep, st, h->small_ws)) != ARX_OK) return rc;
        if (gv != ARX_GEMM_SPLIT_K) { ProfScope ps(ARX_K_LAYERNORM, st);
          launch_ln_finalize(T, H / 64, h->part_s, h->part_q, tp, h->cu + n_seqs, inv_h, c.ln_eps, h->st2_sum, h->st2_sq, st); }
        ARX_HIP_CHECK(hipGetLastError());
        if (h->tap_layer == li + 1 && h->tap) {
            layernorm_kernel<<<ln_grid, 256, 0, st>>>(h->x, h->tap, L.ln2_g, L.ln2_b, h->cu + n_seqs, H, c.ln_eps);
            ARX_HIP_CHECK(hipGetLastError());
        }
    }
    {
        const arx_layer_weights& Ll = h->layers[c.layers - 1];
        ProfScope pps(ARX_K_POOL, st);
        pool_norm_kernel<<<n_seqs, 256, 0, st>>>(h->x, h->cu, H, c.pool, normalize, out_f32, out_stride, (f16_t*)out_f16, out16_stride,
                                                 h->st2_sum, h->st2_sq, Ll.ln2_g, Ll.ln2_b, c.ln_eps);
        ARX_HIP_CHECK(hipGetLastError());
    }
    return ARX_OK;
}

extern "C" int32_t arx_encoder_forward(arx_encoder* h, const int32_t* ids, int32_t seq_stride, const int32_t* lens,
                                       int32_t n_seqs, int32_t max_len, int32_t total_tokens, float* out_f32,
                                       int64_t out_stride, void* out_f16, int64_t out16_stride, int32_t normalize,
                                       void* stream) {
    return encoder_run(h, ids, seq_stride, lens, nullptr, n_seqs, max_len, total_tokens, out_f32, out_stride, out_f16, out16_stride,
                       normalize, stream);
}

static int check_pair_head(const arx_pair_head* p, int hidden) {
    ARX_REQUIRE(p, "null pair head");
    ARX_REQUIRE(p->struct_bytes >= (int32_t)sizeof(arx_pair_head), "arx_pair_head.struct_bytes=%d < %d", p->struct_bytes,
                (int)sizeof(arx_pair_head));
    ARX_REQUIRE(p->n_labels >= 1 && p->n_labels <= 16, "n_labels=%d must be in 1..16", p->n_labels);
    ARX_REQUIRE(p->pooler_w && p->pooler_b && p->cls_w && p->cls_b, "pair head: missing pooler / classifier weights");
    ARX_REQUIRE(hidden > 0 && hidden <= 1024, "hidden=%d must be in 1..1024", hidden);
    return ARX_OK;
}

static int launch_pair_head(const float* cls, int64_t ld, int n, int H, const arx_pair_head& p, float* out, int64_t ld_out,
                            hipStream_t st) {
    const int smem = 2 * PH_ROWS * H * (int)sizeof(float);
    ARX_HIP_CHECK(arx_func_smem((const void*)pair_head_kernel, smem));
    pair_head_kernel<<<cdiv(n, PH_ROWS), 256, smem, st>>>(cls, ld, n, H, p.pooler_w, p.pooler_b, p.cls_w, p.cls_b, p.n_labels, out,
                                                            ld_out);
    ARX_HIP_CHECK(hipGetLastError());
    return ARX_OK;
}

extern "C" int32_t arx_encoder_set_pair_head(arx_encoder* h, const arx_pair_head* head) {
    ARX_REQUIRE(h, "null handle");
    ARX_REQUIRE(h->cfg.arch == ARX_ARCH_BERT && h->cfg.pool == ARX_POOL_CLS, "a pair head needs a BERT handle with CLS pooling");
    const int rc = check_pair_head(head, h->cfg.hidden);
    if (rc != ARX_OK) return rc;
    ARX_REQUIRE(head->type_emb, "pair head: missing token-type table");
    if (!h->cls_ws) ARX_HIP_CHECK(hipMalloc((void**)&h->cls_ws, (int64_t)h->max_seqs * h->cfg.hidden * sizeof(float)));
    h->pair = *head;
    h->has_pair = 1;
    return ARX_OK;
}

extern "C" int32_t arx_encoder_score_pairs(arx_encoder* h, const int32_t* ids, int32_t seq_stride, const int32_t* lens,
                                           const int32_t* seg_b, int32_t n_seqs, int32_t max_len, int32_t total_tokens,
                                           float* out_logits, int64_t out_stride, void* stream) {
    ARX_REQUIRE(h && out_logits, "null handle/out_logits");
    ARX_REQUIRE(h->has_pair, "no pair head set (arx_encoder_set_pair_head)");
    ARX_REQUIRE(out_stride >= h->pair.n_labels, "out_stride < n_labels");
    int rc = encoder_run(h, ids, seq_stride, lens, seg_b, n_seqs, max_len, total_tokens, h->cls_ws, h->cfg.hidden, nullptr, 0, 0,
                         stream);
    if (rc != ARX_OK) return rc;
    return launch_pair_head(h->cls_ws, h->cfg.hidden, n_seqs, h->cfg.hidden, h->pair, out_logits, out_stride, (hipStream_t)stream);
}

extern "C" int32_t arx_encoder_debug_cls(arx_encoder* h, float* dst, int32_t n, void* stream) {
    ARX_REQUIRE(h && h->cls_ws && dst, "no pair head set / null dst");
    ARX_REQUIRE(n > 0 && n <= h->max_seqs, "n out of range");
    ARX_HIP_CHECK(hipMemcpyAsync(dst, h->cls_ws, (int64_t)n * h->cfg.hidden * sizeof(float), hipMemcpyDeviceToDevice, (hipStream_t)stream));
    return ARX_OK;
}

extern "C" int32_t arx_pair_head_forward(const float* cls_rows, int64_t ld, int32_t n, int32_t hidden, const arx_pair_head* head,
                                         float* out_logits, int64_t out_stride, void* stream) {
    const int rc = check_pair_head(head, hidden);
    if (rc != ARX_OK) return rc;
    ARX_REQUIRE(n >= 0 && ld >= hidden && out_stride >= head->n_labels, "bad n / ld / out_stride");
    if (n == 0) return ARX_OK;
    ARX_REQUIRE(cls_rows && out_logits, "null cls_rows/out_logits");
    return launch_pair_head(cls_rows, ld, n, hidden, *head, out_logits, out_stride, (hipStream_t)stream);
}

#ifdef ARX_DEV_VARIANTS
extern "C" int32_t arx_dev_attn_set(arx_encoder* h, int32_t word, void* stamps) {
    h->attn_dev_word = word;
    h->attn_stamps = (unsigned long long*)stamps;
    return ARX_OK;
}
#endif

extern "C" int32_t arx_build_info(void) {
#ifdef ARX_DEV_VARIANTS
    return 1;
#else
    return 0;
#endif
}

extern "C" int32_t arx_adjacent_cosine(const float* emb, int64_t ld, int32_t n, int32_t dim, float* out, void* stream) {
    ARX_REQUIRE(n >= 0 && dim > 0 && dim % 4 == 0 && ld >= dim, "bad sizes (dim must be a multiple of 4)");
    if (n < 2) return ARX_OK;
    ARX_REQUIRE(emb && out, "null pointer argument");
    adjacent_cosine_kernel<<<cdiv(n - 1, 4), 256, 0, (hipStream_t)stream>>>(emb, ld, n, dim, out);
    ARX_HIP_CHECK(hipGetLastError());
    return ARX_OK;
}

extern "C" int32_t arx_f32_to_bf16(const float* src, void* dst, int64_t n, void* stream) {
    ARX_REQUIRE(src && dst && n >= 0, "bad args");
    if (n == 0) return ARX_OK;
    f32_to_bf16_kernel<<<cdiv(n, 256), 256, 0, (hipStream_t)stream>>>(src, (uint16_t*)dst, n);
    ARX_HIP_CHECK(hipGetLastError());
    return ARX_OK;
}
```

### arxiv_rag_amd/csrc/encoder_kernels.h

```cpp
#pragma once
#include <type_traits>

#include "arx_common.h"

__global__ void scan_lens_kernel(const int32_t* __restrict__ lens, int32_t* __restrict__ cu, int n) {
    __shared__ int32_t part[1024];
    const int tid = threadIdx.x, nt = blockDim.x;
    const int per = (n + nt - 1) / nt;
    const int b0 = tid * per, b1 = min(n, b0 + per);
    int s = 0;
    for (int b = b0; b < b1; ++b) s += lens[b];
    part[tid] = s;
    __syncthreads();
    if (tid == 0) {
        int run = 0;
        for (int i = 0; i < nt; ++i) { int v = part[i]; part[i] = run; run += v; }
        cu[n] = run;
    }
    __syncthreads();
    int run = part[tid];
    for (int b = b0; b < b1; ++b) { cu[b] = run; run += lens[b]; }
}

template <int ARCH, bool SEG = false>
// ... 146 lines not shown
    constexpr int KS = DH / 16;
    constexpr int DB = DH / 32;
    extern __shared__ __attribute__((aligned(16))) char smem[];

    const int b = blockIdx.z, h = blockIdx.y;
    const int t0 = cu[b];
    const int L = cu[b + 1] - t0;
    const int q0 = blockIdx.x * (32 * NW);
    if (q0 >= L) return;
    const int Lk = (L + 31) & ~31;
    const int tid = threadIdx.x, lane = tid & 63, wid = tid >> 6;
    const int64_t ld = 3 * (int64_t)H;
    const uint16_t* Qg = qkv + (int64_t)t0 * ld + h * DH;
    const uint16_t* Kg = Qg + H;
    const uint16_t* Vg = Qg + 2 * H;

    char* Ks = smem;
    uint16_t* Vt = reinterpret_cast<uint16_t*>(smem + AttnSmem<DH>::k_bytes(Lk));
    float* Bs = reinterpret_cast<float*>(smem + AttnSmem<DH>::k_bytes(Lk) + AttnSmem<DH>::vt_bytes(Lk));
    const int vts = AttnSmem<DH>::vt_stride(Lk);
    const int bst = AttnSmem<DH>::bias_stride(Lk);

    for (int cid = tid; cid < Lk * CPR; cid += NT) {
        const int row = cid / CPR, pc = cid % CPR;
        const int c = pc ^ ((row / RPB) & (CPR - 1));
        u32x4 kv = u32x4{0u, 0u, 0u, 0u}, vv = u32x4{0u, 0u, 0u, 0u};
        if (row < L) {
            kv = *reinterpret_cast<const u32x4*>(Kg + (int64_t)row * ld + c * 8);
            vv = *reinterpret_cast<const u32x4*>(Vg + (int64_t)row * ld + pc * 8);
        }
        *reinterpret_cast<u32x4*>(Ks + (int64_t)cid * 16) = kv;
        const int k16 = row & 15;
        const int pos = (row & ~15) + (((k16 >> 2) & 1) << 3) + ((k16 >> 3) << 2) + (k16 & 3);
#pragma unroll
        for (int e = 0; e < 4; ++e) {
            Vt[(pc * 8 + 2 * e) * vts + pos] = (uint16_t)(vv[e] & 0xffffu);
            Vt[(pc * 8 + 2 * e + 1) * vts + pos] = (uint16_t)(vv[e] >> 16);
        }
    }
    if (HAS_BIAS) {
        const float* bt = bias_tbl + (int64_t)h * ARX_BIAS_ROW + ARX_BIAS_CENTER;
        for (int i = tid; i < 4 * bst; i += NT) {
            const int c = i / bst, j = i % bst;
            int d = j + c - Lk;
            d = d < -ARX_BIAS_CENTER ? -ARX_BIAS_CENTER : (d > ARX_BIAS_CENTER ? ARX_BIAS_CENTER : d);
            Bs[i] = bt[d];
        }
    }
    __syncthreads();

    const int qw = q0 + wid * 32;
    if (qw >= L) return;
    const int ql = lane & 31, hh = lane >> 5;
    const int q = qw + ql;
    const int qc = q < L ? q : L - 1;
    bf16x8 qf[KS];
#pragma unroll
    for (int ks = 0; ks < KS; ++ks)
        qf[ks] = *reinterpret_cast<const bf16x8*>(Qg + (int64_t)qc * ld + ks * 16 + hh * 8);

    f32x16 o[DB];
#pragma unroll
    for (int d = 0; d < DB; ++d)
#pragma unroll
        for (int r = 0; r < 16; ++r) o[d][r] = 0.f;
    float m_run = -INFINITY, l_run = 0.f;

    const int bc = (4 - (qc & 3)) & 3;
    const float* brow = Bs + bc * bst + (Lk - qc - bc);
    const int krow_sw = ((ql / RPB) & (CPR - 1));

    const int nkt = Lk >> 5;
    for (int kt = 0; kt < nkt; ++kt) {
        f32x16 s;
#pragma unroll
        for (int r = 0; r < 16; ++r) s[r] = 0.f;
        const char* krow = Ks + (int64_t)(kt * 32 + ql) * (DH * 2);
#pragma unroll
        for (int ks = 0; ks < KS; ++ks) {
            const bf16x8 kf = *reinterpret_cast<const bf16x8*>(krow + (((2 * ks + hh) ^ krow_sw) << 4));
            s = __builtin_amdgcn_mfma_f32_32x32x16_bf16(kf, qf[ks], s, 0, 0, 0);
        }
        float mx = -INFINITY;
#pragma unroll
        for (int g4 = 0; g4 < 4; ++g4) {
            const int kb = kt * 32 + 8 * g4 + 4 * hh;
            f32x4 bv = f32x4{0.f, 0.f, 0.f, 0.f};
            if (HAS_BIAS) bv = *reinterpret_cast<const f32x4*>(brow + kb);
#pragma unroll
            for (int e = 0; e < 4; ++e) {
                float v = s[g4 * 4 + e] * scale_log2e + bv[e];
                v = (kb + e < L) ? v : -INFINITY;
                s[g4 * 4 + e] = v;
                mx = fmaxf(mx, v);
            }
        }
        mx = fmaxf(mx, __shfl_xor(mx, 32));
        const float m_new = fmaxf(m_run, mx);
        const float alpha = exp2f(m_run - m_new);
        m_run = m_new;
        float rs = 0.f;
#pragma unroll
        for (int r = 0; r < 16; ++r) { s[r] = exp2f(s[r] - m_new); rs += s[r]; }
        l_run = l_run * alpha + rs;
#pragma unroll
        for (int d = 0; d < DB; ++d)
#pragma unroll
            for (int r = 0; r < 16; ++r) o[d][r] *= alpha;
        bf16x8 pf[2];
#pragma unroll
        for (int ss = 0; ss < 2; ++ss)
#pragma unroll
            for (int e = 0; e < 8; ++e) pf[ss][e] = (bf16_t)s[8 * ss + e];
#pragma unroll
        for (int d = 0; d < DB; ++d) {
            const uint16_t* vrow = Vt + (int64_t)(d * 32 + ql) * vts + kt * 32 + hh * 8;
#pragma unroll
            for (int ss = 0; ss < 2; ++ss) {
                const bf16x8 vf = *reinterpret_cast<const bf16x8*>(vrow + ss * 16);
                o[d] = __builtin_amdgcn_mfma_f32_32x32x16_bf16(vf, pf[ss], o[d], 0, 0, 0);
            }
        }
    }
    const float l_tot = l_run + __shfl_xor(l_run, 32);
    const float inv = 1.0f / l_tot;
    if (q < L) {
        uint16_t* orow = ctx + (int64_t)(t0 + q) * H + h * DH;
#pragma unroll
        for (int d = 0; d < DB; ++d)
#pragma unroll
            for (int g4 = 0; g4 < 4; ++g4) {
                u32x2 w2;
                w2[0] = pack_bf16x2(o[d][g4 * 4 + 0] * inv, o[d][g4 * 4 + 1] * inv);
                w2[1] = pack_bf16x2(o[d][g4 * 4 + 2] * inv, o[d][g4 * 4 + 3] * inv);
                *reinterpret_cast<u32x2*>(orow + d * 32 + 8 * g4 + 4 * hh) = w2;
            }
    }
}

typedef short s16x4 __attribute__((ext_vector_type(4)));
template <int DH> struct AttnSmem2 {
    static __host__ __device__ int kv_bytes(int Lk) { return Lk * DH * 2; }
    static __host__ __device__ int bias_stride(int Lk) { return 2 * Lk + 8; }
    static __host__ __device__ int total(int Lk, bool has) { return 2 * kv_bytes(Lk) + (has ? 4 * (2 * Lk + 8) * 4 : 0); }
};

template <int DH> struct AttnSmem3 {
    static __host__ __device__ int kv_bytes(int Lk) { return Lk * DH * 2; }
    static __host__ __device__ int bias_stride(int Lk) { return ((2 * Lk + 8 + 63) & ~63) + 64; }
    static __host__ __device__ int total(int Lk, bool has) { return 2 * kv_bytes(Lk) + (has ? 4 * bias_stride(Lk) * 4 : 0); }
};
__device__ __forceinline__ int attn_bias_off(int c) { return c == 0 ? 0 : (c == 1 ? 20 : (c == 2 ? 36 : 52)); }

template <int DH, bool HAS_BIAS, int NW>
__global__ __launch_bounds__(NW * 64, NW / 2) void attention_tr_kernel(const uint16_t* __restrict__ qkv, uint16_t* __restrict__ ctx,
                                                                        const int32_t* __restrict__ cu,
                                                                        const float* __restrict__ bias_tbl, int H,
                                                                        float scale_log2e, int dev_word, unsigned long long* dev_stamps) {
    constexpr int NT = NW * 64;
    constexpr int CPR = DH / 8;
    constexpr int RPB = 256 / (DH * 2);
#ifdef ARX_DEV_VARIANTS
    const unsigned lin = blockIdx.x + gridDim.x * (blockIdx.y + gridDim.y * blockIdx.z);
    if (dev_stamps && threadIdx.x == 0) {
        dev_stamps[4 * lin] = wall_clock64();
        dev_stamps[4 * lin + 3] = ((unsigned long long)__builtin_amdgcn_s_getreg((31 << 11) | 20) << 32) | (unsigned)__builtin_amdgcn_s_getreg((31 << 11) | 4);
    }
#endif
    constexpr int KS = DH / 16;
    constexpr int DB = DH / 32;
    constexpr int ROWB = DH * 2;
    constexpr int RPI = NT / CPR;
    extern __shared__ __attribute__((aligned(16))) char smem[];
    const int b = blockIdx.z, h = blockIdx.y;
    const int t0 = cu[b];
    const int L = cu[b + 1] - t0;
    const int q0 = blockIdx.x * (32 * NW);
    if (q0 >= L) return;
    const int Lk = (L + 31) & ~31;
    const int tid = threadIdx.x, lane = tid & 63, wid = tid >> 6;
    const uint32_t ld = 3u * (uint32_t)H;
    const uint16_t* Qg = qkv + (int64_t)t0 * ld + h * DH;
    const uint16_t* Kg = Qg + H;
    const uint16_t* Vg = Qg + 2 * H;
    char* Ks = smem;
    char* Vs = smem + AttnSmem3<DH>::kv_bytes(Lk);
    float* Bs = reinterpret_cast<float*>(smem + 2 * AttnSmem3<DH>::kv_bytes(Lk));
    const int bst = AttnSmem3<DH>::bias_stride(Lk);

    const int ql = lane & 31, hh = lane >> 5;
    const int qw = q0 + wid * 32;
    const int q = qw + ql;
    const int qc = q < L ? q : L - 1;
    bf16x8 qf[KS];
#pragma unroll
    for (int ks = 0; ks < KS; ++ks)
        qf[ks] = *reinterpret_cast<const bf16x8*>(Qg + (uint32_t)qc * ld + ks * 16 + hh * 8);
    {
        static_assert(RPI % 16 == 0, "staging pass must keep the swizzle terms constant per thread");
        typedef __attribute__((address_space(3))) void lds_v;
        typedef const __attribute__((address_space(1))) void gbl_v;
        const int pc = tid % CPR, r0 = tid / CPR;
        const int kc = pc ^ ((r0 / RPB) & (CPR - 1));
        const int vc = (DH == 64) ? (pc ^ (((r0 >> 1) & 1) << 2)) : pc;
        uint32_t lo = (uint32_t)(tid & ~63) * 16;
        int LkS = Lk;
#ifdef ARX_DEV_VARIANTS
        if (dev_word == 5) LkS = 0;
#endif
        for (int row = r0; row < LkS; row += RPI, lo += NT * 16) {
            const uint32_t gr = (uint32_t)(row < L ? row : L - 1) * ld;
            __builtin_amdgcn_global_load_lds((gbl_v*)(Kg + gr + kc * 8), (lds_v*)(Ks + lo), 16, 0, 0);
            __builtin_amdgcn_global_load_lds((gbl_v*)(Vg + gr + vc * 8), (lds_v*)(Vs + lo), 16, 0, 0);
        }
    }
    if (HAS_BIAS) {
        const float* bt = bias_tbl + (int64_t)h * ARX_BIAS_ROW + ARX_BIAS_CENTER;
        const int span = 2 * Lk + 8;
        for (int i = tid; i < 4 * span; i += NT) {
            const int c = (i >= span) + (i >= 2 * span) + (i >= 3 * span), j = i - c * span;
            int d = j + c - Lk;
            d = d < -ARX_BIAS_CENTER ? -ARX_BIAS_CENTER : (d > ARX_BIAS_CENTER ? ARX_BIAS_CENTER : d);
            Bs[c * bst + attn_bias_off(c) + j] = bt[d];
        }
    }
    __syncthreads();
#ifdef ARX_DEV_VARIANTS
    if (dev_stamps && threadIdx.x == 0) dev_stamps[4 * lin + 1] = wall_clock64();
    if (dev_word == 3) {
        if (q < L && qf[0][0] == 0x7fc1 && qf[1 % KS][1] == 0x7fc2) ctx[(int64_t)(t0 + q) * H + h * DH] = 1;
        return;
    }
#endif

    if (qw >= L) return;
    f32x16 o[DB];
    auto lds_bases = [&](const float*& bb, const char* (&kb)[KS], const char* (&vb)[DB]) {
        int lane = threadIdx.x & 63;
        asm volatile("" : "+v"(lane));
        const int ql = lane & 31, hh = lane >> 5;
        int qc = q0 + wid * 32 + ql;
        qc = qc < L ? qc : L - 1;
        const int bc = (4 - (qc & 3)) & 3;
        bb = Bs + bc * bst + attn_bias_off(bc) + (Lk - qc - bc) + 4 * hh;
        const int krow_sw = ((ql / RPB) & (CPR - 1));
#pragma unroll
        for (int ks = 0; ks < KS; ++ks) kb[ks] = Ks + ql * ROWB + (((2 * ks + hh) ^ krow_sw) << 4);
        const int g16 = lane >> 4, q_ = (lane & 15) >> 2, p_ = lane & 3;
        const int vsw = (DH == 64) ? (((q_ >> 1) & 1) << 2) : 0;
#pragma unroll
        for (int d = 0; d < DB; ++d) {
            const int col = 32 * d + 16 * (g16 & 1) + 4 * p_;
            vb[d] = Vs + (4 * hh + q_) * ROWB + (((col >> 3) ^ vsw) << 4) + ((p_ & 1) << 3);
        }
    };
    typedef __attribute__((address_space(3))) s16x4 lds_s16x4;
    typedef short s16x8 __attribute__((ext_vector_type(8)));
    f32x4 lsum;
    const s16x4 one4 = s16x4{0x3f80, 0x3f80, 0x3f80, 0x3f80};
    const int nkt = Lk >> 5;
    const int nfull = (L & 31) ? nkt - 1 : nkt;
    float l_tot;

    bool redo = false;
#ifdef ARX_DEV_VARIANTS
    redo = dev_word == 6;
#endif
    if (!redo) {
#pragma unroll
        for (int d = 0; d < DB; ++d)
#pragma unroll
            for (int r = 0; r < 16; ++r) o[d][r] = 0.f;
        lsum = f32x4{0.f, 0.f, 0.f, 0.f};
        typedef const __attribute__((address_space(3))) char* lds_cptr;
        typedef const __attribute__((address_space(3))) float* lds_fptr;
        lds_fptr bp;
        lds_cptr kp[KS], vp[DB];
        {
            const float* bb;
            const char* kb[KS];
            const char* vb[DB];
            lds_bases(bb, kb, vb);
            bp = (lds_fptr)bb;
#pragma unroll
            for (int ks = 0; ks < KS; ++ks) kp[ks] = (lds_cptr)kb[ks];
#pragma unroll
            for (int d = 0; d < DB; ++d) vp[d] = (lds_cptr)vb[d];
        }
        bf16x8 kf[KS];
#pragma unroll
        for (int ks = 0; ks < KS; ++ks) kf[ks] = *reinterpret_cast<const __attribute__((address_space(3))) bf16x8*>(kp[ks]);
        auto advance = [&](int n) {
            bp += 32 * n;
            asm volatile("" : "+v"(bp));
#pragma unroll
            for (int ks = 0; ks < KS; ++ks) { kp[ks] += 32 * ROWB * n; asm volatile("" : "+v"(kp[ks])); }
#pragma unroll
            for (int d = 0; d < DB; ++d) { vp[d] += 32 * ROWB * n; asm volatile("" : "+v"(vp[d])); }
            __builtin_amdgcn_sched_barrier(0);
        };
        auto fast = [&](auto masked_tag, auto off_tag, int kt) {
            constexpr bool MASKED = decltype(masked_tag)::value;
            constexpr int OFF = decltype(off_tag)::value;
            f32x16 s;
#pragma unroll
            for (int r = 0; r < 16; ++r) s[r] = 0.f;
#pragma unroll
            for (int ks = 0; ks < KS; ++ks) s = __builtin_amdgcn_mfma_f32_32x32x16_bf16(kf[ks], qf[ks], s, 0, 0, 0);
            __builtin_amdgcn_sched_barrier(0);
            f32x4 bv[4];
#pragma unroll
            for (int g4 = 0; g4 < 4; ++g4) bv[g4] = HAS_BIAS ? *reinterpret_cast<const __attribute__((address_space(3))) f32x4*>(bp + OFF * 32 + 8 * g4) : f32x4{0.f, 0.f, 0.f, 0.f};
            s16x4 vt[DB][4];
#pragma unroll
            for (int d = 0; d < DB; ++d)
#pragma unroll
                for (int j = 0; j < 4; ++j) vt[d][j] = __builtin_amdgcn_ds_read_tr16_b64_v4i16((lds_s16x4*)(vp[d] + (OFF * 32 + 8 * j) * ROWB));
            __builtin_amdgcn_sched_barrier(0);
            typedef float f32x2 __attribute__((ext_vector_type(2)));
            const f32x2 sc2 = f32x2{scale_log2e, scale_log2e};
#pragma unroll
            for (int g4 = 0; g4 < 4; ++g4)
#pragma unroll
                for (int e = 0; e < 4; e += 2) {
                    f32x2 v = __builtin_elementwise_fma(f32x2{s[g4 * 4 + e], s[g4 * 4 + e + 1]}, sc2, f32x2{bv[g4][e], bv[g4][e + 1]});
                    if (MASKED) {
                        v[0] = (kt * 32 + 8 * g4 + 4 * hh + e < L) ? v[0] : -INFINITY;
                        v[1] = (kt * 32 + 8 * g4 + 4 * hh + e + 1 < L) ? v[1] : -INFINITY;
                    }
                    s[g4 * 4 + e] = v[0]; s[g4 * 4 + e + 1] = v[1];
                }
            __builtin_amdgcn_sched_barrier(0);
#pragma unroll
            for (int r = 0; r < 16; ++r) s[r] = __builtin_amdgcn_exp2f(s[r]);
            uint32_t pw[8];
#pragma unroll
            for (int j = 0; j < 8; ++j) pw[j] = pack_bf16x2(s[2 * j], s[2 * j + 1]);
            __builtin_amdgcn_sched_barrier(0);
            if (!MASKED) {
#pragma unroll
                for (int ks = 0; ks < KS; ++ks) kf[ks] = *reinterpret_cast<const __attribute__((address_space(3))) bf16x8*>(kp[ks] + (OFF + 1) * 32 * ROWB);
            }
            __builtin_amdgcn_sched_barrier(0);
            bf16x8 pf[2];
#pragma unroll
            for (int ss = 0; ss < 2; ++ss) pf[ss] = __builtin_bit_cast(bf16x8, u32x4{pw[4 * ss], pw[4 * ss + 1], pw[4 * ss + 2], pw[4 * ss + 3]});
#pragma unroll
            for (int j = 0; j < 4; ++j)
                lsum = __builtin_amdgcn_mfma_f32_4x4x4bf16_1k(one4, __builtin_bit_cast(s16x4, u32x2{pw[2 * j], pw[2 * j + 1]}), lsum, 0, 0, 0);
#pragma unroll
            for (int d = 0; d < DB; ++d)
#pragma unroll
                for (int ss = 0; ss < 2; ++ss) {
                    s16x8 v8;
#pragma unroll
                    for (int e = 0; e < 4; ++e) { v8[e] = vt[d][2 * ss][e]; v8[4 + e] = vt[d][2 * ss + 1][e]; }
                    o[d] = __builtin_amdgcn_mfma_f32_32x32x16_bf16(__builtin_bit_cast(bf16x8, v8), pf[ss], o[d], 0, 0, 0);
                }
            __builtin_amdgcn_sched_barrier(0);
        };
        int kt = 0;
        for (; kt + 2 <= nfull; kt += 2) {
            fast(std::false_type{}, std::integral_constant<int, 0>{}, kt);
            fast(std::false_type{}, std::integral_constant<int, 1>{}, kt + 1);
            advance(2);
        }
        if (kt < nfull) { fast(std::false_type{}, std::integral_constant<int, 0>{}, kt); advance(1); }
        if (nfull < nkt) fast(std::true_type{}, std::integral_constant<int, 0>{}, nkt - 1);
        l_tot = lsum[0] + __shfl_xor(lsum[0], 32);
        redo = !__all(l_tot > 0x1p-100f && l_tot < 0x1p100f);
    }
    if (redo) {
#pragma unroll
    for (int d = 0; d < DB; ++d)
#pragma unroll
        for (int r = 0; r < 16; ++r) o[d][r] = 0.f;
    float m_run = -INFINITY;
    const float* bptr;
    const char* kptr[KS];
    const char* vptr[DB];
    lds_bases(bptr, kptr, vptr);
    constexpr float THR = 8.0f;
    const float inv_scale = 1.0f / scale_log2e;
    lsum = f32x4{0.f, 0.f, 0.f, 0.f};
    auto tile = [&](auto masked_tag, auto first_tag, int kt) {
        constexpr bool MASKED = decltype(masked_tag)::value;
        constexpr bool FIRST = decltype(first_tag)::value;
        f32x16 s;
        const float s0 = FIRST ? 0.f : -m_run * inv_scale;
#pragma unroll
        for (int r = 0; r < 16; ++r) s[r] = s0;
#pragma unroll
        for (int ks = 0; ks < KS; ++ks) {
            const bf16x8 kf = *reinterpret_cast<const bf16x8*>(kptr[ks]);
            s = __builtin_amdgcn_mfma_f32_32x32x16_bf16(kf, qf[ks], s, 0, 0, 0);
        }
#pragma unroll
        for (int g4 = 0; g4 < 4; ++g4) {
            f32x4 bv = f32x4{0.f, 0.f, 0.f, 0.f};
            if (HAS_BIAS) bv = *reinterpret_cast<const f32x4*>(bptr + 8 * g4);
#pragma unroll
            for (int e = 0; e < 4; ++e) {
                float v = fmaf(s[g4 * 4 + e], scale_log2e, bv[e]);
                if (MASKED) v = (kt * 32 + 8 * g4 + 4 * hh + e < L) ? v : -INFINITY;
                s[g4 * 4 + e] = v;
            }
        }
        float mx = -INFINITY;
#pragma unroll
        for (int r = 0; r < 16; r += 2) mx = fmaxf(mx, fmaxf(s[r], s[r + 1]));
        mx = fmaxf(mx, __shfl_xor(mx, 32));
        if (FIRST) {
            m_run = mx;
#pragma unroll
            for (int r = 0; r < 16; ++r) s[r] -= mx;
        } else if (__any(mx > THR)) {
            const float d = fmaxf(mx, 0.f);
            const float alpha = __builtin_amdgcn_exp2f(-d);
            m_run += d;
#pragma unroll
            for (int r = 0; r < 16; ++r) s[r] -= d;
#pragma unroll
            for (int r = 0; r < 4; ++r) lsum[r] *= alpha;
#pragma unroll
            for (int dd = 0; dd < DB; ++dd)
#pragma unroll
                for (int r = 0; r < 16; ++r) o[dd][r] *= alpha;
        }
#pragma unroll
        for (int r = 0; r < 16; ++r) s[r] = __builtin_amdgcn_exp2f(s[r]);
        uint32_t pw[8];
#pragma unroll
        for (int j = 0; j < 8; ++j) pw[j] = pack_bf16x2(s[2 * j], s[2 * j + 1]);
        bf16x8 pf[2];
#pragma unroll
        for (int ss = 0; ss < 2; ++ss) pf[ss] = __builtin_bit_cast(bf16x8, u32x4{pw[4 * ss], pw[4 * ss + 1], pw[4 * ss + 2], pw[4 * ss + 3]});
#pragma unroll
        for (int j = 0; j < 4; ++j)
            lsum = __builtin_amdgcn_mfma_f32_4x4x4bf16_1k(one4, __builtin_bit_cast(s16x4, u32x2{pw[2 * j], pw[2 * j + 1]}), lsum, 0, 0, 0);
#pragma unroll
        for (int d = 0; d < DB; ++d) {
#pragma unroll
            for (int ss = 0; ss < 2; ++ss) {
                const s16x4 lo = __builtin_amdgcn_ds_read_tr16_b64_v4i16((lds_s16x4*)(vptr[d] + (16 * ss) * ROWB));
                const s16x4 hi = __builtin_amdgcn_ds_read_tr16_b64_v4i16((lds_s16x4*)(vptr[d] + (16 * ss + 8) * ROWB));
                s16x8 v8;
#pragma unroll
                for (int e = 0; e < 4; ++e) { v8[e] = lo[e]; v8[4 + e] = hi[e]; }
                o[d] = __builtin_amdgcn_mfma_f32_32x32x16_bf16(__builtin_bit_cast(bf16x8, v8), pf[ss], o[d], 0, 0, 0);
            }
        }
        bptr += 32;
#pragma unroll
        for (int ks = 0; ks < KS; ++ks) kptr[ks] += 32 * ROWB;
#pragma unroll
        for (int d = 0; d < DB; ++d) vptr[d] += 32 * ROWB;
    };
    if (nfull > 0) tile(std::false_type{}, std::true_type{}, 0); else tile(std::true_type{}, std::true_type{}, 0);
    for (int kt = 1; kt < nfull; ++kt) tile(std::false_type{}, std::false_type{}, kt);
    if (nfull < nkt && nkt > 1) tile(std::true_type{}, std::false_type{}, nkt - 1);
    l_tot = lsum[0] + __shfl_xor(lsum[0], 32);
    }

    const float inv = 1.0f / l_tot;
    u32x4 pc[DB][2];
#pragma unroll
    for (int d = 0; d < DB; ++d) {
        uint32_t w[4][2];
#pragma unroll
        for (int g4 = 0; g4 < 4; ++g4) {
            w[g4][0] = pack_bf16x2(o[d][g4 * 4 + 0] * inv, o[d][g4 * 4 + 1] * inv);
            w[g4][1] = pack_bf16x2(o[d][g4 * 4 + 2] * inv, o[d][g4 * 4 + 3] * inv);
        }
#pragma unroll
        for (int g = 0; g < 2; ++g)
#pragma unroll
            for (int k = 0; k < 2; ++k) {
                const auto sw = __builtin_amdgcn_permlane32_swap(w[g][k], w[g + 2][k], false, false);
                pc[d][g][k] = sw[0]; pc[d][g][2 + k] = sw[1];
            }
    }
    if (q < L) {
        uint16_t* orow = ctx + (int64_t)(t0 + q) * H + h * DH + 16 * hh;
#pragma unroll
        for (int d = 0; d < DB; ++d) {
            *reinterpret_cast<u32x4*>(orow + d * 32) = pc[d][0];
            *reinterpret_cast<u32x4*>(orow + d * 32 + 8) = pc[d][1];
        }
    }
#ifdef ARX_DEV_VARIANTS
    if (dev_stamps && (threadIdx.x & 63) == 0) atomicMax(&dev_stamps[4 * lin + 2], (unsigned long long)wall_clock64());
#endif
}

#ifdef ARX_DEV_VARIANTS
template <int DH, int NSLOT_ = 8> struct AttnRing {
    static constexpr int NT = 512, NSLOT = NSLOT_, AHEAD = NSLOT - 1, SLOT_KEYS = 64;
    static constexpr int ROWB = DH * 2;
    static constexpr int SLOT_BYTES = 2 * SLOT_KEYS * ROWB;
    static constexpr int GPS = SLOT_BYTES / (NT * 16);
    static_assert(GPS >= 1 && GPS * NT * 16 == SLOT_BYTES, "slot must be whole passes of the block");
    static __host__ __device__ int bias_stride(int C0) { return (2 * C0 + 8 + 52 + 63) & ~63; }
    static __host__ __device__ int total(int C0, bool has) { return NSLOT * SLOT_BYTES + (has ? 4 * bias_stride(C0) * 4 : 0); }
};

#define ARX_VMCNT_CASE(N) case N: asm volatile("s_waitcnt vmcnt(" #N ")" ::: "memory"); break;
#define ARX_VMCNT_CASE4(A, B, C_, D) ARX_VMCNT_CASE(A) ARX_VMCNT_CASE(B) ARX_VMCNT_CASE(C_) ARX_VMCNT_CASE(D)
__device__ __forceinline__ void attn_wait_vm(int n) {
    switch (n) {
    ARX_VMCNT_CASE4(0, 1, 2, 3) ARX_VMCNT_CASE4(4, 5, 6, 7) ARX_VMCNT_CASE4(8, 9, 10, 11) ARX_VMCNT_CASE4(12, 13, 14, 15)
    ARX_VMCNT_CASE4(16, 17, 18, 19) ARX_VMCNT_CASE4(20, 21, 22, 23) ARX_VMCNT_CASE4(24, 25, 26, 27) ARX_VMCNT_CASE4(28, 29, 30, 31)
    ARX_VMCNT_CASE4(32, 33, 34, 35) ARX_VMCNT_CASE4(36, 37, 38, 39) ARX_VMCNT_CASE4(40, 41, 42, 43) ARX_VMCNT_CASE(44)
    default: asm volatile("s_waitcnt vmcnt(0)" ::: "memory"); break;
    }
}
#undef ARX_VMCNT_CASE4
#undef ARX_VMCNT_CASE

template <int DH, int NSLOT> struct AttnStream {
    using R = AttnRing<DH, NSLOT>;
    static constexpr int NT = R::NT, ROWB = R::ROWB, SLOT_BYTES = R::SLOT_BYTES, GPS = R::GPS, CPR = DH / 8, RPB = 256 / R::ROWB;
    const uint16_t* qkv; const int32_t* cu; char* ring;
    int H, h, G, n_seqs;
    uint32_t ld;
    int p_b, p_t0, p_L, p_step, p_nqp, p_nsteps, p_slot, c_slot;
    int inflight, pend_st;
    unsigned st_bits;

    __device__ __forceinline__ void p_load_item() {
        p_L = 0; p_step = 0;
        while (p_b < n_seqs) {
            const __attribute__((address_space(4))) int32_t* cuc = (const __attribute__((address_space(4))) int32_t*)cu;
            const int t0 = cuc[p_b], L = cuc[p_b + 1] - t0;
            if (L > 0) { p_t0 = t0; p_L = L; p_nqp = L > 128 ? 2 : 1; p_nsteps = p_nqp + ((L + 63) >> 6); break; }
            p_b += G;
        }
    }
    __device__ __forceinline__ void issue_next() {
        const uint16_t* base = qkv + (int64_t)p_t0 * ld + h * DH;
        const bool isq = p_step < p_nqp;
        const int r0 = isq ? 128 * p_step : 64 * (p_step - p_nqp);
        int t = threadIdx.x;
        asm volatile("" : "+v"(t));
        char* dst = ring + p_slot * SLOT_BYTES + (__builtin_amdgcn_readfirstlane(t) & ~63) * 16;
#pragma unroll
        for (int it = 0; it < GPS; ++it) {
            const int cid = it * NT + t, r128 = cid / CPR, pcn = cid % CPR;
            int row, col0, c;
            if (isq) { row = r0 + r128; col0 = 0; c = pcn ^ ((r128 / RPB) & (CPR - 1)); }
            else if (r128 < 64) { row = r0 + r128; col0 = H; c = pcn ^ ((r128 / RPB) & (CPR - 1)); }
            else { row = r0 + r128 - 64; col0 = 2 * H; c = (DH == 64) ? (pcn ^ (((r128 >> 1) & 1) << 2)) : pcn; }
            row = row < p_L ? row : p_L - 1;
            __builtin_amdgcn_global_load_lds((const __attribute__((address_space(1))) void*)(base + (uint32_t)row * ld + col0 + c * 8),
                                             (__attribute__((address_space(3))) void*)(dst + it * NT * 16), 16, 0, 0);
        }
        if (pend_st) st_bits |= 1u << inflight;
        pend_st = 0;
        ++inflight;
        p_slot = (p_slot + 1) & (R::NSLOT - 1);
        if (++p_step == p_nsteps) { p_b += G; p_load_item(); }
    }
    __device__ __forceinline__ const char* step_begin() {
        attn_wait_vm((inflight - 1) * GPS + (DH / 8) * __builtin_popcount(st_bits >> 1) + pend_st);
        asm volatile("" ::: "memory");
        __builtin_amdgcn_s_barrier();
        asm volatile("" ::: "memory");
        st_bits >>= 1;
        --inflight;
        if (p_L > 0) issue_next();
        const char* slot = ring + c_slot * SLOT_BYTES;
        c_slot = (c_slot + 1) & (R::NSLOT - 1);
        return slot;
    }
};

template <int DH, bool HAS_BIAS, bool MASKED, bool first>
__device__ __forceinline__ void attn_ring_tile(const char* kbase, int k0, int v0, const bf16x8 (&qf)[DH / 16], f32x16 (&o)[DH / 32],
                                               f32x4& lsum, float& m_run, const float* bp, int kt, int hh, int L,
                                               float scale_log2e, float inv_scale) {
    constexpr int KS = DH / 16, DB = DH / 32, ROWB = DH * 2;
    constexpr float THR = 8.0f;
    typedef __attribute__((address_space(3))) s16x4 lds_s16x4;
    typedef short s16x8 __attribute__((ext_vector_type(8)));
    f32x16 s;
    const float s0 = first ? 0.f : -m_run * inv_scale;
#pragma unroll
    for (int r = 0; r < 16; ++r) s[r] = s0;
#pragma unroll
    for (int ks = 0; ks < KS; ++ks) {
        const bf16x8 kf = *reinterpret_cast<const bf16x8*>(kbase + (k0 ^ (ks << 5)));
        s = __builtin_amdgcn_mfma_f32_32x32x16_bf16(kf, qf[ks], s, 0, 0, 0);
    }
#pragma unroll
    for (int g4 = 0; g4 < 4; ++g4) {
        f32x4 bv = f32x4{0.f, 0.f, 0.f, 0.f};
        if (HAS_BIAS) bv = *reinterpret_cast<const f32x4*>(bp + 8 * g4);
#pragma unroll
        for (int e = 0; e < 4; ++e) {
            float v = fmaf(s[g4 * 4 + e], scale_log2e, bv[e]);
            if (MASKED) v = (kt * 32 + 8 * g4 + 4 * hh + e < L) ? v : -INFINITY;
            s[g4 * 4 + e] = v;
        }
    }
    float mx = -INFINITY;
#pragma unroll
    for (int r = 0; r < 16; r += 2) mx = fmaxf(mx, fmaxf(s[r], s[r + 1]));
    mx = fmaxf(mx, __shfl_xor(mx, 32));
    if (first) {
        m_run = mx;
#pragma unroll
        for (int r = 0; r < 16; ++r) s[r] -= mx;
    } else if (__any(mx > THR)) {
        const float d = fmaxf(mx, 0.f);
        const float alpha = __builtin_amdgcn_exp2f(-d);
        m_run += d;
#pragma unroll
        for (int r = 0; r < 16; ++r) s[r] -= d;
#pragma unroll
        for (int r = 0; r < 4; ++r) lsum[r] *= alpha;
#pragma unroll
        for (int dd = 0; dd < DB; ++dd)
#pragma unroll
            for (int r = 0; r < 16; ++r) o[dd][r] *= alpha;
    }
#pragma unroll
    for (int r = 0; r < 16; ++r) s[r] = __builtin_amdgcn_exp2f(s[r]);
    uint32_t pw[8];
#pragma unroll
    for (int j = 0; j < 8; ++j) pw[j] = pack_bf16x2(s[2 * j], s[2 * j + 1]);
    bf16x8 pf[2];
#pragma unroll
    for (int ss = 0; ss < 2; ++ss) pf[ss] = __builtin_bit_cast(bf16x8, u32x4{pw[4 * ss], pw[4 * ss + 1], pw[4 * ss + 2], pw[4 * ss + 3]});
    const s16x4 one4 = s16x4{0x3f80, 0x3f80, 0x3f80, 0x3f80};
#pragma unroll
    for (int j = 0; j < 4; ++j)
        lsum = __builtin_amdgcn_mfma_f32_4x4x4bf16_1k(one4, __builtin_bit_cast(s16x4, u32x2{pw[2 * j], pw[2 * j + 1]}), lsum, 0, 0, 0);
    const uint32_t vaddr = (uint32_t)(size_t)(const __attribute__((address_space(3))) char*)kbase + (uint32_t)v0;
#pragma unroll
    for (int d = 0; d < DB; ++d) {
        const uint32_t va = vaddr ^ (uint32_t)(d << 6);
        s16x4 vt[2][2];
#pragma unroll
        for (int ss = 0; ss < 2; ++ss) {
            asm volatile("ds_read_b64_tr_b16 %0, %1 offset:%2" : "=v"(vt[ss][0]) : "v"(va), "n"((16 * ss) * ROWB));
            asm volatile("ds_read_b64_tr_b16 %0, %1 offset:%2" : "=v"(vt[ss][1]) : "v"(va), "n"((16 * ss + 8) * ROWB));
// ... 363 lines not shown
#pragma unroll 1
        for (int p = 0; p < nqp; ++p) {
            const char* slot = st.step_begin();
            if (wave_on && (wid >> 3) == p) {
                const char* qrow = slot + (wid & 7) * 16 * ROWB;
#pragma unroll
                for (int ks = 0; ks < 2; ++ks) qf[ks] = *reinterpret_cast<const bf16x8*>(qrow + (k0 ^ (ks << 6)));
            }
        }
        const bool ragged = (L & 31) != 0;
#pragma unroll 1
        for (int sidx = 0; sidx < nkv; ++sidx) {
            const char* slot = st.step_begin();
            if (wave_on) {
#pragma unroll 1
                for (int t2 = 0; t2 < 2; ++t2) {
                    const int kt = 2 * sidx + t2;
                    if (kt >= nkt) break;
                    const char* kbase = slot + t2 * 32 * ROWB;
                    const bool msk = ragged && kt == nkt - 1;
                    if (kt == 0) {
                        if (msk) attn_ring16_tile<HAS_BIAS, true, true>(kbase, k0, v0, qf, o, lsum, m_run, bptr, kt, g, L, scale_log2e, inv_scale);
                        else attn_ring16_tile<HAS_BIAS, false, true>(kbase, k0, v0, qf, o, lsum, m_run, bptr, kt, g, L, scale_log2e, inv_scale);
                    } else {
                        if (msk) attn_ring16_tile<HAS_BIAS, true, false>(kbase, k0, v0, qf, o, lsum, m_run, bptr + 32 * kt, kt, g, L, scale_log2e, inv_scale);
                        else attn_ring16_tile<HAS_BIAS, false, false>(kbase, k0, v0, qf, o, lsum, m_run, bptr + 32 * kt, kt, g, L, scale_log2e, inv_scale);
                    }
                }
            }
        }
        if (wave_on) {
            float l_tot = lsum[0];
            {
                const auto a = __builtin_amdgcn_permlane16_swap(__float_as_uint(l_tot), __float_as_uint(l_tot), false, false);
                l_tot = __uint_as_float(a[0]) + __uint_as_float(a[1]);
                const auto c2 = __builtin_amdgcn_permlane32_swap(__float_as_uint(l_tot), __float_as_uint(l_tot), false, false);
                l_tot = __uint_as_float(c2[0]) + __uint_as_float(c2[1]);
            }
            const float inv = 1.0f / l_tot;
            uint16_t* orow = ctx + (int64_t)(t0 + qc) * H + h * 64 + 4 * g;
            if (q < L) {
#pragma unroll
                for (int db = 0; db < 4; ++db) {
                    u32x2 w2;
                    w2[0] = pack_bf16x2(o[db][0] * inv, o[db][1] * inv);
                    w2[1] = pack_bf16x2(o[db][2] * inv, o[db][3] * inv);
                    asm volatile("global_store_dwordx2 %0, %1, off\n\ts_nop 1" :: "v"(orow + 16 * db), "v"(w2) : "memory");
                }
            }
            st.pend_st += 4;
        }
        b += G;
    }
}

#endif

__global__ __launch_bounds__(256) void pool_norm_kernel(const uint16_t* __restrict__ x, const int32_t* __restrict__ cu,
                                                         int H, int pool_mode, int normalize,
                                                         float* __restrict__ out32, int64_t ld32,
                                                         f16_t* __restrict__ out16, int64_t ld16,
                                                         const float* __restrict__ ln_sum, const float* __restrict__ ln_sq,
                                                         const float* __restrict__ ln_g, const float* __restrict__ ln_b, float eps) {
    __shared__ float acc_s[4][1024];
    __shared__ float red[4];
    const int b = blockIdx.x, tid = threadIdx.x, lane = tid & 63, w = tid >> 6;
    const int t0 = cu[b], L = cu[b + 1] - t0;
    const int nch = H >> 3;
    float a[2][8];
#pragma unroll
    for (int c = 0; c < 2; ++c)
#pragma unroll
        for (int e = 0; e < 8; ++e) a[c][e] = 0.f;
    const int nrows = (pool_mode == ARX_POOL_CLS) ? (L > 0 ? 1 : 0) : L;
    for (int r = w; r < nrows; r += 4) {
        const uint16_t* in = x + (int64_t)(t0 + r) * H;
        float mu = 0.f, rs = 1.f;
        if (ln_sum) { mu = ln_sum[t0 + r]; rs = ln_sq[t0 + r]; }
#pragma unroll
        for (int c = 0; c < 2; ++c) {
            const int ch = lane + 64 * c;
            if (ch < nch) {
                const u32x4 q = *reinterpret_cast<const u32x4*>(in + ch * 8);
#pragma unroll
                for (int e = 0; e < 4; ++e) {
                    float lo, hi;
                    unpack_bf16x2(q[e], lo, hi);
                    a[c][2 * e] += (lo - mu) * rs; a[c][2 * e + 1] += (hi - mu) * rs;
                }
            }
        }
    }
#pragma unroll
    for (int c = 0; c < 2; ++c) {
        const int ch = lane + 64 * c;
        if (ch < nch)
#pragma unroll
            for (int e = 0; e < 8; ++e) acc_s[w][ch * 8 + e] = a[c][e];
    }
    __syncthreads();
    float v[4];
    float sq = 0.f;
    const float denom = (pool_mode == ARX_POOL_CLS) ? 1.0f : fmaxf((float)L, 1e-9f);
#pragma unroll
    for (int c = 0; c < 4; ++c) {
        const int col = tid + 256 * c;
        v[c] = 0.f;
        if (col < H) {
            v[c] = (acc_s[0][col] + acc_s[1][col] + acc_s[2][col] + acc_s[3][col]) / denom;
            if (ln_sum && L > 0) v[c] = fmaf(v[c], ln_g[col], ln_b[col]);
            sq += v[c] * v[c];
        }
    }
    sq = wave_sum(sq);
    if (lane == 0) red[w] = sq;
    __syncthreads();
    const float nrm = sqrtf(red[0] + red[1] + red[2] + red[3]);
    const float sc = normalize ? 1.0f / fmaxf(nrm, 1e-12f) : 1.0f;
#pragma unroll
    for (int c = 0; c < 4; ++c) {
        const int col = tid + 256 * c;
        if (col < H) {
            const float y = v[c] * sc;
            if (out32) out32[(int64_t)b * ld32 + col] = y;
            if (out16) out16[(int64_t)b * ld16 + col] = (f16_t)y;
        }
    }
}

template <int NP>
__global__ __launch_bounds__(256) void ln_finalize_kernel(const float* __restrict__ ps, const float* __restrict__ pq, int64_t ld,
                                                           int nparts, const int32_t* __restrict__ n_rows_ptr, float inv_h, float eps,
                                                           float* __restrict__ mean, float* __restrict__ rstd) {
    const int m = blockIdx.x * 256 + threadIdx.x;
    if (m >= *n_rows_ptr) return;
    float s = 0.f, q = 0.f;
    if constexpr (NP > 0) {
        float vs[NP], vq[NP];
#pragma unroll
        for (int p = 0; p < NP; ++p) { vs[p] = ps[p * ld + m]; vq[p] = pq[p * ld + m]; }
#pragma unroll
        for (int p = 0; p < NP; ++p) { s += vs[p]; q += vq[p]; }
    } else {
        for (int p = 0; p < nparts; ++p) { s += ps[p * ld + m]; q += pq[p * ld + m]; }
    }
    const float mu = s * inv_h;
    mean[m] = mu;
    rstd[m] = rsqrtf(fmaxf(q * inv_h - mu * mu, 0.f) + eps);
}

__global__ __launch_bounds__(256) void fold_ln_kernel(const uint16_t* __restrict__ W, const float* __restrict__ gamma,
                                                       const float* __restrict__ beta, const float* __restrict__ bias,
                                                       uint16_t* __restrict__ Wf, float* __restrict__ s, float* __restrict__ c,
                                                       int N, int K) {
    const int lane = threadIdx.x & 63;
    const int n = blockIdx.x * 4 + (threadIdx.x >> 6);
    if (n >= N) return;
    float ss = 0.f, cc = 0.f;
    for (int k = lane; k < K; k += 64) {
        const float w = bf16_bits_to_f32(W[(int64_t)n * K + k]);
        const bf16_t wf = (bf16_t)(w * gamma[k]);
        Wf[(int64_t)n * K + k] = __builtin_bit_cast(uint16_t, wf);
        ss += (float)wf;
        cc = fmaf(beta[k], w, cc);
    }
    ss = wave_sum(ss); cc = wave_sum(cc);
    if (lane == 0) { s[n] = ss; c[n] = bias[n] + cc; }
}

__global__ __launch_bounds__(256) void adjacent_cosine_kernel(const float* __restrict__ e, int64_t ld, int n, int D,
                                                               float* __restrict__ out) {
    const int lane = threadIdx.x & 63;
    const int i = blockIdx.x * 4 + (threadIdx.x >> 6);
    if (i + 1 >= n) return;
    const float* a = e + (int64_t)i * ld;
    const float* b = a + ld;
    float dot = 0.f, na = 0.f, nb = 0.f;
    for (int c = lane * 4; c < D; c += 256) {
        const f32x4 x = *reinterpret_cast<const f32x4*>(a + c), y = *reinterpret_cast<const f32x4*>(b + c);
#pragma unroll
        for (int r = 0; r < 4; ++r) { dot = fmaf(x[r], y[r], dot); na = fmaf(x[r], x[r], na); nb = fmaf(y[r], y[r], nb); }
    }
    dot = wave_sum(dot); na = wave_sum(na); nb = wave_sum(nb);
    if (lane == 0) out[i] = dot / (sqrtf(na) * sqrtf(nb));
}

constexpr int PH_ROWS = 16;
__global__ __launch_bounds__(256) void pair_head_kernel(const float* __restrict__ cls, int64_t ld, int n, int H,
                                                         const float* __restrict__ wp, const float* __restrict__ bp,
                                                         const float* __restrict__ wc, const float* __restrict__ bc, int n_labels,
                                                         float* __restrict__ out, int64_t ld_out) {
    extern __shared__ float ph_sm[];
    float* xs = ph_sm;
    float* ps = ph_sm + PH_ROWS * H;
    const int r0 = blockIdx.x * PH_ROWS, tid = threadIdx.x, lane = tid & 63, w = tid >> 6;
    const int nr = min(PH_ROWS, n - r0);
    for (int i = tid; i < PH_ROWS * H; i += 256) {
        const int r = i / H, k = i - r * H;
        xs[i] = r < nr ? cls[(int64_t)(r0 + r) * ld + k] : 0.f;
    }
    __syncthreads();
    for (int j = w; j < H; j += 4) {
        const float* wr = wp + (int64_t)j * H;
        float acc[PH_ROWS];
#pragma unroll
        for (int r = 0; r < PH_ROWS; ++r) acc[r] = 0.f;
        for (int k = lane; k < H; k += 64) {
            const float wv = wr[k];
#pragma unroll
            for (int r = 0; r < PH_ROWS; ++r) acc[r] = fmaf(wv, xs[r * H + k], acc[r]);
        }
        const float bj = bp[j];
#pragma unroll
        for (int r = 0; r < PH_ROWS; ++r) {
            const float v = wave_sum(acc[r]);
            if (lane == r) ps[r * H + j] = tanhf(v + bj);
        }
    }
    __syncthreads();
    for (int o = w; o < nr * n_labels; o += 4) {
        const int r = o / n_labels, l = o - r * n_labels;
        const float* wr = wc + (int64_t)l * H;
        float acc = 0.f;
        for (int k = lane; k < H; k += 64) acc = fmaf(wr[k], ps[r * H + k], acc);
        acc = wave_sum(acc);
        if (lane == 0) out[(int64_t)(r0 + r) * ld_out + l] = acc + bc[l];
    }
}

__global__ void bf16_to_f32_kernel(const uint16_t* __restrict__ src, float* __restrict__ dst, int64_t n) {
    const int64_t i = (int64_t)blockIdx.x * blockDim.x + threadIdx.x;
    if (i < n) dst[i] = bf16_bits_to_f32(src[i]);
}
__global__ void f32_to_bf16_kernel(const float* __restrict__ src, uint16_t* __restrict__ dst, int64_t n) {
    const int64_t i = (int64_t)blockIdx.x * blockDim.x + threadIdx.x;
    if (i < n) { bf16_t v = (bf16_t)src[i]; dst[i] = __builtin_bit_cast(uint16_t, v); }
}
```

### include/arx.h

```cpp
#ifndef ARX_H
#define ARX_H

#include <stdint.h>

#ifdef __cplusplus
extern "C" {
#endif

#define ARX_VERSION 112

#define ARX_OK            0
#define ARX_ERR_ARG      -1
#define ARX_ERR_HIP      -2
#define ARX_ERR_CAPACITY -3

#define ARX_ARCH_MPNET 0
#define ARX_ARCH_BERT  1
#define ARX_POOL_MEAN  0
#define ARX_POOL_CLS   1

typedef struct {
    int32_t arch;
    int32_t vocab_size;
    int32_t hidden;
    int32_t layers;
    int32_t heads;
    int32_t ffn;
    int32_t max_pos;
    int32_t pool;
    int32_t pad_id;
    int32_t rel_buckets;
    int32_t rel_max_distance;
    float   ln_eps;
} arx_encoder_config;

typedef struct {
    const void*  w_qkv;
    const float* b_qkv;
    const void*  w_o;
    const float* b_o;
    const float* ln1_g; const float* ln1_b;
    const void*  w_fc1;
    const float* b_fc1;
    const void*  w_fc2;
    const float* b_fc2;
    const float* ln2_g; const float* ln2_b;
} arx_layer_weights;

typedef struct {
    const float* word_emb;
    const float* pos_emb;
    const float* type_emb;
    const float* emb_ln_g; const float* emb_ln_b;
    const float* rel_bias;
    const arx_layer_weights* layers;
} arx_encoder_weights;

typedef struct arx_encoder arx_encoder;

int32_t     arx_version(void);
const char* arx_last_error(void);

int32_t arx_mpnet_bucket(int32_t relative_position, int32_t num_buckets, int32_t max_distance);

int64_t arx_encoder_workspace_bytes(const arx_encoder_config* cfg, int32_t max_tokens, int32_t max_seqs);

int32_t arx_encoder_create(const arx_encoder_config* cfg, const arx_encoder_weights* w,
                           int32_t max_tokens, int32_t max_seqs, arx_encoder** out);
void    arx_encoder_destroy(arx_encoder* h);

#define ARX_GEMM_DEFAULT    89
#define ARX_GEMM_PER_TILE    8
#define ARX_GEMM_PERSISTENT  9
#define ARX_GEMM_2STAGE     13
#define ARX_GEMM_SPLIT_K    70
#define ARX_GEMM_TILE_128   71
#define ARX_ATTN_TRANSPOSED  1
#define ARX_ATTN_RING        2
#define ARX_ATTN_RING16      4
#define ARX_ATTN_STAGED      8
#define ARX_ENC_EXPLICIT_LAYERNORM 1
typedef struct {
    int32_t struct_bytes;
    int32_t gemm_schedule;
    int32_t attn_kernel;
    int32_t flags;
} arx_encoder_options;
int32_t arx_encoder_create_opt(const arx_encoder_config* cfg, const arx_encoder_weights* w, int32_t max_tokens, int32_t max_seqs,
                               const arx_encoder_options* opt, arx_encoder** out);

int32_t arx_encoder_forward(arx_encoder* h, const int32_t* ids, int32_t seq_stride,
                            const int32_t* lens, int32_t n_seqs, int32_t max_len, int32_t total_tokens,
                            float* out_f32, int64_t out_stride,
                            void* out_f16, int64_t out16_stride,
                            int32_t normalize, void* stream);

int32_t arx_encoder_attention(arx_encoder* h, const void* qkv, const int32_t* lens, int32_t n_seqs, int32_t max_len,
                              void* ctx, void* stream);

int32_t arx_encoder_debug_hidden(arx_encoder* h, int32_t layer_slot, float* dst, int32_t n_tokens, void* stream);

int32_t arx_encoder_set_low_latency(arx_encoder* h, int32_t on);

int32_t arx_encoder_set_tap(arx_encoder* h, int32_t layer);

typedef struct {
    int32_t struct_bytes;
    int32_t n_labels;
    const float* type_emb;
    const float* pooler_w; const float* pooler_b;
    const float* cls_w;    const float* cls_b;
} arx_pair_head;

int32_t arx_encoder_set_pair_head(arx_encoder* h, const arx_pair_head* head);
int32_t arx_encoder_score_pairs(arx_encoder* h, const int32_t* ids, int32_t seq_stride, const int32_t* lens, const int32_t* seg_b,
                                int32_t n_seqs, int32_t max_len, int32_t total_tokens, float* out_logits, int64_t out_stride,
                                void* stream);
int32_t arx_encoder_debug_cls(arx_encoder* h, float* dst, int32_t n, void* stream);
int32_t arx_pair_head_forward(const float* cls_rows, int64_t ld, int32_t n, int32_t hidden, const arx_pair_head* head,
                              float* out_logits, int64_t out_stride, void* stream);

int32_t arx_build_info(void);

int64_t arx_topk_workspace_bytes(int64_t n_rows, int32_t n_queries, int32_t dim, int32_t k);
int32_t arx_topk_search(const void* corpus, int64_t n_rows, const void* queries, int32_t n_queries,
                        int32_t dim, int32_t k, float* out_scores, int64_t* out_ids, int64_t idx_base,
                        void* ws, int64_t ws_bytes, void* stream);

int64_t arx_topk_i8_index_bytes(int64_t n_rows, int32_t dim);
int64_t arx_topk_workspace_bytes_i8(int64_t n_rows, int32_t n_queries, int32_t dim, int32_t k);
int32_t arx_topk_build_i8(const void* corpus, int64_t n_rows, int32_t dim, void* index_i8, void* stream);
int32_t arx_topk_i8_index_info(const void* index_i8, int64_t n_rows, int32_t dim, float* host_out, void* stream);
int32_t arx_topk_search_i8(const void* corpus, const void* index_i8, int64_t n_rows, const void* queries, int32_t n_queries,
                           int32_t dim, int32_t k, float* out_scores, int64_t* out_ids, int64_t idx_base,
                           void* ws, int64_t ws_bytes, void* stream);

#define ARX_TOPK_NO_PERSISTENT 1
#define ARX_TOPK_NO_SINGLE_ROW_TAIL 8
#define ARX_TOPK_I8_CENTRE_QUERY 16
#define ARX_TOPK_SCAN_ONLY     2
#define ARX_TOPK_TAIL_ONLY     4
typedef struct {
    int32_t struct_bytes;
    int32_t i8_max_queries;
    float   max_row_norm;
    int32_t cu_limit;
    int32_t flags;
    float   debug_tau_mult;
    int32_t debug_drop_best;
} arx_topk_options;
int32_t arx_topk_search_opt(const void* corpus, const void* index_i8, int64_t n_rows, const void* queries, int32_t n_queries,
                            int32_t dim, int32_t k, float* out_scores, int64_t* out_ids, int64_t idx_base,
                            void* ws, int64_t ws_bytes, const arx_topk_options* opt, void* stream);

int32_t arx_rows_max_norm_f16(const void* rows, int64_t n_rows, int32_t dim, float* out_max, void* stream);

int32_t arx_topk_stats(const void* ws, int64_t* flagged_queries, int64_t* extra_groups, void* stream);

int32_t arx_stream_create_cu_mask(const uint32_t* cu_mask, int32_t n_words, void** out);
int32_t arx_stream_destroy(void* stream);
int32_t arx_device_cu_count(void);
int32_t arx_debug_cu_census(uint32_t* out, int32_t n_blocks, int32_t spin_cycles, void* stream);

int32_t arx_topk_merge(const float* scores, const int64_t* ids, int32_t n_parts, int32_t n_queries,
                       int32_t k, float* out_scores, int64_t* out_ids, void* stream);

int64_t arx_topk_filtered_workspace_bytes(int64_t n_rows, int32_t n_queries, int32_t dim, int32_t k);
int32_t arx_topk_search_filtered(const void* corpus, int64_t n_rows, const uint64_t* allow, int64_t n_allowed, const void* queries,
                                 int32_t n_queries, int32_t dim, int32_t k, float* out_scores, int64_t* out_ids, int64_t idx_base,
                                 float max_row_norm, void* ws, int64_t ws_bytes, void* stream);
int32_t arx_topk_search_filtered_tuned(const void* corpus, int64_t n_rows, const uint64_t* allow, int64_t n_allowed, const void* queries,
                                       int32_t n_queries, int32_t dim, int32_t k, float* out_scores, int64_t* out_ids, int64_t idx_base,
                                       float max_row_norm, void* ws, int64_t ws_bytes, int32_t path, int32_t cand_cap, void* stream);
int32_t arx_topk_filtered_stats(const void* ws, int64_t* overflowed_queries, int64_t* candidate_groups, void* stream);

int64_t arx_topk_filtered_multi_workspace_bytes(int64_t n_rows, int32_t n_queries, int32_t n_filters, int32_t dim, int32_t k);
int32_t arx_topk_search_filtered_multi(const void* corpus, int64_t n_rows, const uint64_t* allow, int32_t n_filters,
                                       const int64_t* n_allowed, const int32_t* filter_of, const void* queries, int32_t n_queries,
                                       int32_t dim, int32_t k, float* out_scores, int64_t* out_ids, int64_t idx_base, float max_row_norm,
                                       void* ws, int64_t ws_bytes, void* stream);
int32_t arx_topk_search_filtered_multi_tuned(const void* corpus, int64_t n_rows, const uint64_t* allow, int32_t n_filters,
                                             const int64_t* n_allowed, const int32_t* filter_of, const void* queries, int32_t n_queries,
                                             int32_t dim, int32_t k, float* out_scores, int64_t* out_ids, int64_t idx_base,
                                             float max_row_norm, void* ws, int64_t ws_bytes, int32_t path, int32_t cand_cap, void* stream);
int32_t arx_topk_filtered_multi_stats(const void* ws, int64_t* overflowed_queries, int64_t* candidate_groups, void* stream);

int64_t arx_topk_prefix_workspace_bytes(int64_t n_rows, int32_t n_queries, int32_t dim, int32_t k);
int32_t arx_topk_search_prefix(const void* corpus, int64_t n_rows, const void* queries, const int64_t* row_limit, int32_t n_queries,
                               int32_t dim, int32_t k, float* out_scores, int64_t* out_ids, int64_t idx_base, float max_row_norm,
                               void* ws, int64_t ws_bytes, void* stream);
int32_t arx_topk_search_prefix_tuned(const void* corpus, int64_t n_rows, const void* queries, const int64_t* row_limit, int32_t n_queries,
                                     int32_t dim, int32_t k, float* out_scores, int64_t* out_ids, int64_t idx_base, float max_row_norm,
                                     void* ws, int64_t ws_bytes, int32_t path, int32_t cand_cap, void* stream);
int32_t arx_topk_prefix_stats(const void* ws, int64_t* overflowed_queries, int64_t* candidate_groups, void* stream);

int64_t arx_topk_grouped_workspace_bytes(int64_t n_rows, int32_t n_queries, int32_t dim, int32_t n_groups, int32_t chunks_per_group);
int32_t arx_topk_search_grouped(const void* corpus, int64_t n_rows, const int32_t* group_of, int64_t max_run_rows, const uint64_t* allow,
                                int64_t n_allowed, const void* queries, int32_t n_queries, int32_t dim, int32_t n_groups,
                                int32_t chunks_per_group, float* out_scores, int64_t* out_ids, int32_t* out_groups, int64_t idx_base,
                                float max_row_norm, void* ws, int64_t ws_bytes, void* stream);
int32_t arx_topk_search_grouped_tuned(const void* corpus, int64_t n_rows, const int32_t* group_of, int64_t max_run_rows,
                                      const uint64_t* allow, int64_t n_allowed, const void* queries, int32_t n_queries, int32_t dim,
                                      int32_t n_groups, int32_t chunks_per_group, float* out_scores, int64_t* out_ids, int32_t* out_groups,
                                      int64_t idx_base, float max_row_norm, void* ws, int64_t ws_bytes, int32_t path, int32_t cand_cap,
                                      void* stream);
int32_t arx_topk_grouped_stats(const void* ws, int64_t* overflowed_queries, int64_t* candidate_groups, void* stream);
int32_t arx_group_runs_info(const int32_t* group_of, int64_t n_rows, int64_t* out, void* stream);

int64_t arx_topk_search_boosted_workspace_bytes(int64_t n_rows, int32_t n_queries, int32_t dim, int32_t k);
int32_t arx_topk_search_boosted(const void* corpus, int64_t n_rows, const float* prior, float max_abs_prior, const float* weight,
                                const uint64_t* allow, int64_t n_allowed, const void* queries, int32_t n_queries, int32_t dim, int32_t k,
                                float* out_scores, float* out_base, int64_t* out_ids, int64_t idx_base, float max_row_norm, void* ws,
                                int64_t ws_bytes, int32_t path, int32_t cand_cap, void* stream);
int32_t arx_topk_boosted_stats(const void* ws, int64_t* overflowed_queries, int64_t* candidate_groups, void* stream);
int32_t arx_prior_info(const float* prior, int64_t n_rows, int64_t* out, void* stream);

int64_t arx_range_workspace_bytes(int64_t n_rows, int32_t n_queries, int32_t dim, int32_t max_results);
int32_t arx_range_search(const void* corpus, int64_t n_rows, const uint64_t* allow, int64_t n_allowed, const void* queries,
                         const float* min_score, int32_t n_queries, int32_t dim, int32_t max_results, float* out_scores, int64_t* out_ids,
                         int32_t* out_counts, int64_t idx_base, float max_row_norm, void* ws, int64_t ws_bytes, void* stream);
int32_t arx_range_search_tuned(const void* corpus, int64_t n_rows, const uint64_t* allow, int64_t n_allowed, const void* queries,
                               const float* min_score, int32_t n_queries, int32_t dim, int32_t max_results, float* out_scores,
                               int64_t* out_ids, int32_t* out_counts, int64_t idx_base, float max_row_norm, void* ws, int64_t ws_bytes,
                               int32_t path, int32_t cand_cap, void* stream);
int32_t arx_range_stats(const void* ws, int64_t* overflowed_queries, int64_t* candidate_groups, void* stream);

int32_t arx_text_contains(const uint8_t* blob, const int64_t* row_off, int64_t n_rows,
                          const uint8_t* pat_blob, const int32_t* pat_off, int32_t n_pat,
                          uint64_t* out_bits, void* stream);
int32_t arx_text_regex(const uint8_t* blob, const int64_t* row_off, int64_t n_rows,
                       const uint8_t* tables, const int32_t* table_off, int32_t n_re,
                       uint64_t* out_bits, void* stream);
int32_t arx_text_regex_tuned(const uint8_t* blob, const int64_t* row_off, int64_t n_rows,
                             const uint8_t* tables, const int32_t* table_off, int32_t n_re,
                             uint64_t* out_bits, int32_t waves_per_block, void* stream);
int32_t arx_bitmap_count(const uint64_t* bits, int64_t n_rows, int64_t* out_count, void* stream);

int32_t arx_compact_plan(const uint64_t* keep, int64_t n_rows, int64_t* word_rank, int64_t* out_count, void* stream);
int32_t arx_compact_rows(const void* src, void* dst, int64_t row_bytes, int64_t n_rows, const uint64_t* keep, const int64_t* word_rank,
                         void* stream);
int32_t arx_compact_text(const uint8_t* blob, const int64_t* row_off, int64_t n_rows, const uint64_t* keep, const int64_t* word_rank,
                         uint8_t* new_blob, int64_t* new_row_off, void* stream);

typedef struct {
    double  operand;
    int32_t column;
    int32_t want_kind;
    int32_t op;
    int32_t negate;
    int32_t set_off;
    int32_t set_len;
// ... 1 lines not shown
int32_t arx_where_eval(const int64_t* col_table, int32_t n_cols, int64_t n_rows,
                       const arx_where_leaf* leaves, const int32_t* leaf_off,
                       const int32_t* tokens, const int32_t* token_off,
                       const double* set_vals, int64_t n_set_vals, int32_t n_filters,
                       const uint64_t* and_with, int64_t and_stride,
                       uint64_t* out_bits, int64_t* out_counts, void* stream);

#define ARX_FACET_CODE     0
#define ARX_FACET_EXACT    1
#define ARX_FACET_INTERVAL 2
typedef struct arx_facet_key {
    const uint8_t* kind;
    const double*  val;
    const double*  cuts;
    int32_t mode;
    int32_t want_kind;
    int32_t n_bins;
    int32_t reserved;
    int64_t out_off;
} arx_facet_key;
int32_t arx_facet_count(const arx_facet_key* keys, int32_t n_keys, int64_t n_rows,
                        const uint64_t* allow, int64_t allow_stride, int32_t n_filters,
                        int32_t* out, int64_t out_stride, void* stream);
int32_t arx_facet_count_tuned(const arx_facet_key* keys, int32_t n_keys, int64_t n_rows,
                              const uint64_t* allow, int64_t allow_stride, int32_t n_filters,
                              int32_t* out, int64_t out_stride,
                              int32_t block_threads, int32_t blocks_x, int32_t lds_bins, void* stream);

int64_t arx_cluster_sums_workspace_bytes(int64_t n_members, int32_t C, int32_t dim);
int32_t arx_cluster_sums(const void* rows, int64_t n_rows, int32_t dim, const int32_t* order, int64_t n_members, const int64_t* start,
                         int32_t C, void* partials, int64_t ws_bytes, float* sums, void* stream);
int32_t arx_cluster_sums_tuned(const void* rows, int64_t n_rows, int32_t dim, const int32_t* order, int64_t n_members, const int64_t* start,
                               int32_t C, void* partials, int64_t ws_bytes, float* sums, int32_t block_threads, int32_t runs_per_block,
                               void* stream);
int32_t arx_cluster_finish(const float* sums, const int64_t* start, const float* prev, int32_t C, int32_t dim, float* out_f32,
                           void* out_f16, void* stream);

int64_t arx_cluster_assign_workspace_bytes(int64_t n_rows, int32_t C, int32_t dim);
int32_t arx_cluster_assign(const void* rows, int64_t n_rows, int32_t dim, const void* centroids_f16, int32_t C, float max_centroid_norm,
                           int32_t* out_labels, float* out_scores, int64_t* stats, void* ws, int64_t ws_bytes, void* stream);
int32_t arx_cluster_assign_tuned(const void* rows, int64_t n_rows, int32_t dim, const void* centroids_f16, int32_t C,
                                 float max_centroid_norm, int32_t* out_labels, float* out_scores, int64_t* stats, void* ws,
                                 int64_t ws_bytes, float tau_mult, int32_t rows_per_block, void* stream);

int64_t arx_ivf_workspace_bytes(int64_t n_members, int32_t n_lists, int32_t n_queries, int32_t n_probe, int32_t dim, int32_t k);
int32_t arx_ivf_search(const void* corpus, int64_t n_rows, int32_t dim, const int32_t* order, int64_t n_members, const int64_t* start,
                       int32_t n_lists, int64_t max_list_rows, const void* queries, int32_t n_queries, const int32_t* probes,
                       int32_t n_probe, const uint64_t* allow, int32_t k, float* out_scores, int64_t* out_ids, int64_t* out_scanned,
                       int64_t idx_base, void* ws, int64_t ws_bytes, void* stream);
int32_t arx_ivf_search_tuned(const void* corpus, int64_t n_rows, int32_t dim, const int32_t* order, int64_t n_members, const int64_t* start,
                             int32_t n_lists, int64_t max_list_rows, const void* queries, int32_t n_queries, const int32_t* probes,
                             int32_t n_probe, const uint64_t* allow, int32_t k, float* out_scores, int64_t* out_ids,
                             int64_t* out_scanned, int64_t idx_base, void* ws, int64_t ws_bytes, int32_t rows_per_block, void* stream);
int64_t arx_ivf_multi_workspace_bytes(int64_t n_members, int32_t n_lists, int32_t n_queries, int32_t n_probe, int32_t dim, int32_t k);
int32_t arx_ivf_search_multi(const void* corpus, int64_t n_rows, int32_t dim, const int32_t* order, int64_t n_members, const int64_t* start,
                             int32_t n_lists, int64_t max_list_rows, const void* queries, int32_t n_queries, const int32_t* probes,
                             int32_t n_probe, const uint64_t* allow, int32_t n_filters, const int32_t* filter_of, const float* min_score,
                             int32_t k, float* out_scores, int64_t* out_ids, int64_t* out_scanned, int64_t* out_hits, int64_t idx_base,
                             void* ws, int64_t ws_bytes, void* stream);
int32_t arx_ivf_search_multi_tuned(const void* corpus, int64_t n_rows, int32_t dim, const int32_t* order, int64_t n_members,
                                   const int64_t* start, int32_t n_lists, int64_t max_list_rows, const void* queries, int32_t n_queries,
                                   const int32_t* probes, int32_t n_probe, const uint64_t* allow, int32_t n_filters,
                                   const int32_t* filter_of, const float* min_score, int32_t k, float* out_scores, int64_t* out_ids,
                                   int64_t* out_scanned, int64_t* out_hits, int64_t idx_base, void* ws, int64_t ws_bytes,
                                   int32_t rows_per_block, void* stream);

int32_t arx_binary_pack(const void* rows, int64_t n_rows, int32_t dim, const float* centre, uint64_t* out_codes, void* stream);
int64_t arx_binary_workspace_bytes(int64_t n_rows, int32_t n_queries, int32_t dim, int32_t n_candidates);
int32_t arx_binary_candidates(const uint64_t* codes, int64_t n_rows, int32_t dim, const uint64_t* qcodes, int32_t n_queries,
                              const uint64_t* allow, int32_t n_candidates, int32_t* out_cand, int32_t* out_dist, int64_t* out_count,
                              void* ws, int64_t ws_bytes, void* stream);
int32_t arx_binary_candidates_tuned(const uint64_t* codes, int64_t n_rows, int32_t dim, const uint64_t* qcodes, int32_t n_queries,
                                    const uint64_t* allow, int32_t n_candidates, int32_t* out_cand, int32_t* out_dist,
                                    int64_t* out_count, void* ws, int64_t ws_bytes, int32_t rows_per_block, void* stream);

int32_t arx_pq_encode(const void* rows, int64_t n_rows, int32_t dim, int32_t dsub, const float* centre, const float* codebooks,
                      uint8_t* out_codes, void* stream);
int32_t arx_pq_lut(const void* queries, int32_t n_queries, int32_t dim, int32_t dsub, const float* codebooks, uint8_t* out_lut,
                   void* stream);
int64_t arx_pq_workspace_bytes(int64_t n_rows, int32_t n_queries, int32_t dim, int32_t dsub, int32_t n_candidates);
int32_t arx_pq_candidates(const uint8_t* codes, int64_t n_rows, int32_t dim, int32_t dsub, const uint8_t* lut, int32_t n_queries,
                          const uint64_t* allow, int32_t n_candidates, int32_t* out_cand, int32_t* out_sum, int64_t* out_count, void* ws,
                          int64_t ws_bytes, void* stream);
int32_t arx_pq_candidates_tuned(const uint8_t* codes, int64_t n_rows, int32_t dim, int32_t dsub, const uint8_t* lut, int32_t n_queries,
                                const uint64_t* allow, int32_t n_candidates, int32_t* out_cand, int32_t* out_sum, int64_t* out_count,
                                void* ws, int64_t ws_bytes, int32_t rows_per_block, void* stream);

int32_t arx_gather_rows(const void* shard, int64_t n_rows, int32_t dim, int64_t idx_base, const int64_t* ids, int64_t count,
                        void* out, void* stream);
int32_t arx_mmr_select(const void* q, const void* cand, const int64_t* ids, int32_t n_queries, int32_t n, int32_t dim, int32_t m,
                       float lambda, int32_t* order, float* mmr, void* stream);

int64_t arx_bm25_workspace_bytes(int64_t n_rows, int32_t n_queries, int32_t n);
int32_t arx_bm25_search(const int64_t* term_ptr, const uint32_t* post_row, const float* post_w, int32_t vocab, int64_t n_rows,
                        const int32_t* q_terms, const int32_t* q_nterms, int32_t n_queries, int32_t n, float* out_scores,
                        int64_t* out_ids, int64_t idx_base, void* ws, int64_t ws_bytes, void* stream);
int32_t arx_bm25_search_tuned(const int64_t* term_ptr, const uint32_t* post_row, const float* post_w, int32_t vocab, int64_t n_rows,
                              const int32_t* q_terms, const int32_t* q_nterms, int32_t n_queries, int32_t n, float* out_scores,
                              int64_t* out_ids, int64_t idx_base, void* ws, int64_t ws_bytes, int32_t tile_rows, int32_t max_blocks,
                              void* stream);
int32_t arx_bm25_search_filtered(const int64_t* term_ptr, const uint32_t* post_row, const float* post_w, int32_t vocab, int64_t n_rows,
                                 const uint64_t* allow, int32_t n_filters, const int32_t* filter_of, const int32_t* q_terms,
                                 const int32_t* q_nterms, int32_t n_queries, int32_t n, float* out_scores, int64_t* out_ids,
                                 int64_t idx_base, void* ws, int64_t ws_bytes, void* stream);
int32_t arx_bm25_search_filtered_tuned(const int64_t* term_ptr, const uint32_t* post_row, const float* post_w, int32_t vocab,
                                       int64_t n_rows, const uint64_t* allow, int32_t n_filters, const int32_t* filter_of,
                                       const int32_t* q_terms, const int32_t* q_nterms, int32_t n_queries, int32_t n,
                                       float* out_scores, int64_t* out_ids, int64_t idx_base, void* ws, int64_t ws_bytes,
                                       int32_t tile_rows, int32_t max_blocks, void* stream);
int64_t arx_bm25_wide_workspace_bytes(int64_t n_rows, int32_t n_queries, int32_t n);
int32_t arx_bm25_search_wide(const int64_t* term_ptr, const uint32_t* post_row, const float* post_w, int32_t vocab, int64_t n_rows,
                             const uint64_t* allow, int32_t n_filters, const int32_t* filter_of, const int32_t* q_terms,
                             const int32_t* q_nterms, int32_t n_queries, int32_t n, float* out_scores, int64_t* out_ids,
                             int64_t idx_base, void* ws, int64_t ws_bytes, int32_t tile_rows, int32_t max_blocks, void* stream);
int32_t arx_hybrid_fuse(const float* dense_scores, const int64_t* dense_ids, int32_t n_dense, const float* kw_scores,
                        const int64_t* kw_ids, int32_t n_kw, int32_t n_queries, double alpha, int32_t k, double* out_fused,
                        int64_t* out_ids, float* out_dense, float* out_kw, void* stream);
int32_t arx_bm25_scores(const int64_t* term_ptr, const uint32_t* post_row, const float* post_w, int32_t vocab, int64_t n_rows,
                        const int32_t* q_terms, int32_t n_terms, int64_t row_lo, int64_t row_hi, int32_t tile_rows, float* out,
                        void* stream);
int64_t arx_bm25_build_workspace_bytes(int64_t n_tokens, int64_t n_docs, int32_t vocab);
int32_t arx_bm25_build_postings(const int32_t* pieces, int64_t n_tokens, const int64_t* doc_ptr, int64_t n_docs, int32_t vocab,
                                int64_t* term_ptr, uint32_t* post_row, int32_t* post_tf, int64_t* n_postings, int32_t* bad_id,
                                void* ws, int64_t ws_bytes, void* stream);
int32_t arx_bm25_build_postings_tuned(const int32_t* pieces, int64_t n_tokens, const int64_t* doc_ptr, int64_t n_docs, int32_t vocab,
                                      int64_t* term_ptr, uint32_t* post_row, int32_t* post_tf, int64_t* n_postings, int32_t* bad_id,
                                      void* ws, int64_t ws_bytes, int32_t tile_tokens, int32_t max_blocks, void* stream);
int32_t arx_bm25_build_impacts(const int64_t* term_ptr, const uint32_t* post_row, const int32_t* post_tf, int64_t n_postings,
                               const int64_t* doc_ptr, int64_t n_docs, const double* idf, int32_t vocab, double avgdl, float* post_w,
                               void* stream);

int32_t arx_gemm_bf16(const void* A, const void* W, const float* bias, const void* resid, void* C,
                      int32_t M, int32_t N, int32_t K, int32_t mode, int32_t variant, void* stream);

typedef struct {
    int32_t struct_bytes;
    int32_t mode;
    int32_t variant;
    float eps;
    const float* bias;
    const void* resid;
    const float *a_mean, *a_rstd;
    const float* s_vec;
    const float *r_mean, *r_rstd;
    const float *r_gamma, *r_beta;
    int64_t row_cap;
    float *part_sum, *part_sq;
    int64_t part_ld;
    float *out_mean, *out_rstd;
    const int32_t* n_rows;
} arx_gemm_epilogue;
int32_t arx_gemm_bf16_ex(const void* A, const void* W, void* C, int32_t M, int32_t N, int32_t K, const arx_gemm_epilogue* e, void* stream);

int32_t arx_fold_ln(const void* W, const float* gamma, const float* beta, const float* bias, void* Wf, float* s, float* c,
                    int32_t N, int32_t K, void* stream);

int32_t arx_adjacent_cosine(const float* emb, int64_t ld, int32_t n, int32_t dim, float* out, void* stream);

int32_t arx_wp_create(const char* vocab_blob, const int64_t* vocab_off , int32_t n_vocab, int32_t unk_id,
                      int32_t bos_id, int32_t eos_id, int32_t pad_id, int32_t lowercase, int32_t max_chars_per_word,
                      const char* trigger_blob, const int64_t* trigger_off , int32_t n_triggers, void** out);
void arx_wp_destroy(void* tokenizer);
int32_t arx_wp_encode(void* tokenizer, const char* text_blob, const int64_t* text_off , int64_t n, int32_t max_len,
                      int32_t* ids, int32_t* lens, uint8_t* fallback, int32_t n_threads);
int32_t arx_wp_miss_count(void* tokenizer, int64_t* n_strings, int64_t* n_bytes);
int32_t arx_wp_miss_fetch(void* tokenizer, char* blob, int64_t* off );
int32_t arx_wp_cache_add(void* tokenizer, const char* seg_blob, const int64_t* seg_off , int64_t n, const int32_t* ids,
                         const int64_t* ids_off );
int64_t arx_wp_cache_size(void* tokenizer);
int32_t arx_wp_version(void);

int32_t arx_f32_to_bf16(const float* src, void* dst, int64_t n, void* stream);
int32_t arx_fill_unit_rows_f16(void* dst, int64_t n_rows, int32_t dim, uint64_t seed, void* stream);
int32_t arx_fill_unit_rows_f16_at(void* dst, int64_t n_rows, int32_t dim, uint64_t seed, int64_t row_base, void* stream);
int32_t arx_fill_clustered_rows_f16_at(void* dst, int64_t n_rows, int32_t dim, uint64_t seed, int64_t row_base, int32_t n_clusters,
                                       float spread, int32_t n_hot_dims, float hot_gain, void* stream);

#define ARX_K_SEARCH_GROUPMAX 0
#define ARX_K_GEMM_QKV        1
#define ARX_K_GEMM_OPROJ      2
#define ARX_K_GEMM_FC1        3
#define ARX_K_GEMM_FC2        4
#define ARX_K_ATTENTION       5
#define ARX_K_LAYERNORM       6
#define ARX_K_EMBED           7
#define ARX_K_POOL            8
#define ARX_K_SEARCH_SELECT   9
#define ARX_K_SEARCH_RESCORE 10
#define ARX_K_GEMM_RAW       11
#define ARX_K_CLASSES        12
int32_t arx_prof_enable(int32_t on);
int32_t arx_prof_classes(uint32_t mask);
int32_t arx_prof_reset(void);
int32_t arx_prof_read(int32_t kernel_class, float* total_ms, int32_t* launches);

#ifdef __cplusplus
}
#endif
#endif
```

Baseline: 21310.

## Fold softmax scale into Q projection weights and seed scores with bias

Folds the attention scale (log2e/sqrt(dh)) into the Q rows of the LN-folded QKV weights and bias at encoder creation, so the attention kernel no longer multiplies scores by the scale. For MPNet relative-position bias, the bias is loaded into the MFMA accumulator as its initial value instead of being added with an FMA afterwards. This removes per-score FMA work and reorders bias loads in the attention inner loop. The trade-off is extra rounding, since the scaled Q weights are stored in bf16, and layer 0 now uses a folded weight copy.

Measured after the change: 21360 (median of 6 runs). Within noise of the previous version (+0.2%).

```diff
diff --git a/arxiv_rag_amd/_lib.py b/arxiv_rag_amd/_lib.py
--- a/arxiv_rag_amd/_lib.py
+++ b/arxiv_rag_amd/_lib.py
@@ -71,7 +71,7 @@
 FACET_CODE, FACET_EXACT, FACET_INTERVAL = 0, 1, 2
 TOPK_NO_PERSISTENT, TOPK_SCAN_ONLY, TOPK_TAIL_ONLY, TOPK_NO_SINGLE_ROW_TAIL, TOPK_I8_CENTRE_QUERY = 1, 2, 4, 8, 16
 GEMM_DEFAULT, GEMM_PER_TILE, GEMM_PERSISTENT, GEMM_2STAGE, GEMM_SPLIT_K, GEMM_TILE_128 = 89, 8, 9, 13, 70, 71
-ATTN_TRANSPOSED, ATTN_RING, ATTN_RING16, ATTN_STAGED = 1, 2, 4, 8
+ATTN_TRANSPOSED, ATTN_RING, ATTN_RING16, ATTN_STAGED, ATTN_TRANSPOSED_UNSCALED_Q = 1, 2, 4, 8, 16
 ENC_EXPLICIT_LAYERNORM = 1
 
 
@@ -89,6 +89,7 @@
     "arx_encoder_forward": (C.c_int32, [C.c_void_p, C.c_void_p, C.c_int32, C.c_void_p, C.c_int32, C.c_int32, C.c_int32,
                                         C.c_void_p, C.c_int64, C.c_void_p, C.c_int64, C.c_int32, C.c_void_p]),
     "arx_encoder_attention": (C.c_int32, [C.c_void_p, C.c_void_p, C.c_void_p, C.c_int32, C.c_int32, C.c_void_p, C.c_void_p]),
+    "arx_encoder_attention_prescaled": (C.c_int32, [C.c_void_p, C.c_void_p, C.c_void_p, C.c_int32, C.c_int32, C.c_void_p, C.c_void_p]),
     "arx_encoder_set_tap": (C.c_int32, [C.c_void_p, C.c_int32]),
     "arx_encoder_set_low_latency": (C.c_int32, [C.c_void_p, C.c_int32]),
     "arx_encoder_debug_hidden": (C.c_int32, [C.c_void_p, C.c_int32, C.c_void_p, C.c_int32, C.c_void_p]),
@@ -249,6 +250,8 @@
                                      C.c_void_p]),
     "arx_fold_ln": (C.c_int32, [C.c_void_p, C.c_void_p, C.c_void_p, C.c_void_p, C.c_void_p, C.c_void_p, C.c_void_p, C.c_int32, C.c_int32,
                                 C.c_void_p]),
+    "arx_fold_ln_scaled": (C.c_int32, [C.c_void_p, C.c_void_p, C.c_void_p, C.c_void_p, C.c_void_p, C.c_void_p, C.c_void_p, C.c_int32, C.c_int32,
+                                       C.c_int32, C.c_float, C.c_void_p]),
     "arx_prof_classes": (C.c_int32, [C.c_uint32]),
     "arx_wp_create": (C.c_int32, [C.c_char_p, C.c_void_p, C.c_int32, C.c_int32, C.c_int32, C.c_int32, C.c_int32, C.c_int32, C.c_int32,
                                   C.c_char_p, C.c_void_p, C.c_int32, C.POINTER(C.c_void_p)]),
diff --git a/arxiv_rag_amd/csrc/encoder.hip b/arxiv_rag_amd/csrc/encoder.hip
--- a/arxiv_rag_amd/csrc/encoder.hip
+++ b/arxiv_rag_amd/csrc/encoder.hip
@@ -36,6 +36,7 @@
     uint16_t* tap = nullptr;
     int tap_layer = -1;
     int ln_fold = 1;
+    int q_prescaled = 0;
     char* fold_ws = nullptr;
     std::vector<uint16_t*> wqkv_f, wfc1_f;
     std::vector<float*> s_qkv, c_qkv, s_fc1, c_fc1;
@@ -97,7 +98,7 @@
                 o->struct_bytes, (int)sizeof(arx_encoder_options));
     const int g = o->gemm_schedule, a = o->attn_kernel;
     bool gemm_ok = g == 0 || g == ARX_GEMM_DEFAULT || g == ARX_GEMM_PER_TILE || g == ARX_GEMM_PERSISTENT || g == ARX_GEMM_2STAGE || g == ARX_GEMM_TILE_128;
-    bool attn_ok = a == 0 || a == ARX_ATTN_TRANSPOSED || a == ARX_ATTN_STAGED;
+    bool attn_ok = a == 0 || a == ARX_ATTN_TRANSPOSED || a == ARX_ATTN_STAGED || a == ARX_ATTN_TRANSPOSED_UNSCALED_Q;
 #ifdef ARX_DEV_VARIANTS
     gemm_ok = gemm_ok || g == 1 || g == 2 || g == 3 || g == 4 || g == 15 || g == 33 || g == 34;
     attn_ok = attn_ok || a == ARX_ATTN_RING || a == ARX_ATTN_RING16;
@@ -145,6 +146,7 @@
     if (opt && opt->gemm_schedule) h->variant = opt->gemm_schedule;
     if (opt && opt->attn_kernel) h->attn_variant = opt->attn_kernel;
     h->ln_fold = !(opt && (opt->flags & ARX_ENC_EXPLICIT_LAYERNORM));
+    h->q_prescaled = h->ln_fold && h->attn_variant == ARX_ATTN_TRANSPOSED;
     const WsLayout l = ws_layout(*cfg, max_tokens, max_seqs);
     hipError_t he = hipMalloc((void**)&h->ws, l.total);
     if (he != hipSuccess) {
@@ -169,6 +171,8 @@
         h->part_s = st + 4 * tp; h->part_q = h->part_s + (int64_t)(cfg->hidden / 64) * tp;
     }
     if (h->ln_fold) {
+        const float q_alpha = 1.4426950408889634f / sqrtf((float)(cfg->hidden / cfg->heads));
+        const int n_q = h->q_prescaled ? cfg->hidden : 0;
         const int64_t H = cfg->hidden, F = cfg->ffn, Lc = cfg->layers;
         const int64_t per = round_up64(3 * H * H * 2, 256) + round_up64(F * H * 2, 256) + 2 * round_up64(3 * H * 4, 256) + 2 * round_up64(F * 4, 256);
         he = hipMalloc((void**)&h->fold_ws, per * Lc);
@@ -186,10 +190,12 @@
             float* s1 = (float*)takep(F * 4); float* c1 = (float*)takep(F * 4);
             h->wqkv_f.push_back(wq); h->wfc1_f.push_back(w1);
             h->s_qkv.push_back(sq); h->c_qkv.push_back(cq); h->s_fc1.push_back(s1); h->c_fc1.push_back(c1);
-            fold_ln_kernel<<<cdiv(F, 4), 256>>>((const uint16_t*)L.w_fc1, L.ln1_g, L.ln1_b, L.b_fc1, w1, s1, c1, (int)F, (int)H);
+            fold_ln_kernel<<<cdiv(F, 4), 256>>>((const uint16_t*)L.w_fc1, L.ln1_g, L.ln1_b, L.b_fc1, w1, s1, c1, (int)F, (int)H, 0, 1.0f);
             if (i > 0) {
                 const arx_layer_weights& P = h->layers[i - 1];
-                fold_ln_kernel<<<cdiv(3 * H, 4), 256>>>((const uint16_t*)L.w_qkv, P.ln2_g, P.ln2_b, L.b_qkv, wq, sq, cq, (int)(3 * H), (int)H);
+                fold_ln_kernel<<<cdiv(3 * H, 4), 256>>>((const uint16_t*)L.w_qkv, P.ln2_g, P.ln2_b, L.b_qkv, wq, sq, cq, (int)(3 * H), (int)H, n_q, q_alpha);
+            } else if (h->q_prescaled) {
+                fold_ln_kernel<<<cdiv(3 * H, 4), 256>>>((const uint16_t*)L.w_qkv, nullptr, nullptr, L.b_qkv, wq, sq, cq, (int)(3 * H), (int)H, n_q, q_alpha);
             }
         }
         he = hipDeviceSynchronize();
@@ -454,16 +460,18 @@
     return ARX_OK;
 }
 
-template <int DH, bool HB, int NW>
+template <int DH, bool HB, int NW, bool PRESCALED = false>
 static int launch_attn_tr_cfg(arx_encoder* h, int n_seqs, int max_len, hipStream_t st) {
     auto kern = attention_tr_kernel<DH, HB, NW>;
+    auto kern_ps = attention_tr_prescaled_kernel<DH, HB, NW>;
     const int Lk = (max_len + 31) & ~31;
     const int smem = AttnSmem3<DH>::total(Lk, HB);
-    ARX_HIP_CHECK(arx_func_smem((const void*)kern, smem));
+    ARX_HIP_CHECK(arx_func_smem(PRESCALED ? (const void*)kern_ps : (const void*)kern, smem));
     const float scale_log2e = 1.4426950408889634f / sqrtf((float)DH);
     dim3 grid(cdiv(max_len, 32 * NW), h->cfg.heads, n_seqs);
     ProfScope ps(ARX_K_ATTENTION, st);
-    kern<<<grid, NW * 64, smem, st>>>(h->qkv, h->ctx, h->cu, h->bias_tbl, h->cfg.hidden, scale_log2e, h->attn_dev_word, h->attn_stamps);
+    if (PRESCALED) kern_ps<<<grid, NW * 64, smem, st>>>(h->qkv, h->ctx, h->cu, h->bias_tbl, h->cfg.hidden, h->attn_dev_word, h->attn_stamps);
+    else kern<<<grid, NW * 64, smem, st>>>(h->qkv, h->ctx, h->cu, h->bias_tbl, h->cfg.hidden, scale_log2e, h->attn_dev_word, h->attn_stamps);
     ARX_HIP_CHECK(hipGetLastError());
     return ARX_OK;
 }
@@ -501,9 +509,19 @@
 
 #endif
 
-static int launch_attn(arx_encoder* h, int n_seqs, int max_len, hipStream_t st) {
+static int launch_attn(arx_encoder* h, int n_seqs, int max_len, hipStream_t st, bool prescaled = false) {
     const int dh = h->cfg.hidden / h->cfg.heads;
     const bool hb = h->cfg.arch == ARX_ARCH_MPNET;
+    if (prescaled) {
+        ARX_REQUIRE(h->attn_variant == ARX_ATTN_TRANSPOSED, "pre-scaled attention is the default transposing-read kernel's form");
+        const bool w8 = max_len > 128;
+        if (dh == 64) {
+            if (hb) return w8 ? launch_attn_tr_cfg<64, true, 8, true>(h, n_seqs, max_len, st) : launch_attn_tr_cfg<64, true, 4, true>(h, n_seqs, max_len, st);
+            return w8 ? launch_attn_tr_cfg<64, false, 8, true>(h, n_seqs, max_len, st) : launch_attn_tr_cfg<64, false, 4, true>(h, n_seqs, max_len, st);
+        }
+        if (hb) return w8 ? launch_attn_tr_cfg<32, true, 8, true>(h, n_seqs, max_len, st) : launch_attn_tr_cfg<32, true, 4, true>(h, n_seqs, max_len, st);
+        return w8 ? launch_attn_tr_cfg<32, false, 8, true>(h, n_seqs, max_len, st) : launch_attn_tr_cfg<32, false, 4, true>(h, n_seqs, max_len, st);
+    }
 #ifdef ARX_DEV_VARIANTS
     if (h->attn_variant == ARX_ATTN_RING16 && dh == 64 && max_len > 128 && max_len <= 256)
         return hb ? launch_attn_ring16_cfg<true>(h, n_seqs, max_len, st) : launch_attn_ring16_cfg<false>(h, n_seqs, max_len, st);
@@ -530,8 +548,8 @@
     return big ? launch_attn_cfg<32, false, 8>(h, n_seqs, max_len, st) : launch_attn_cfg<32, false, 4>(h, n_seqs, max_len, st);
 }
 
-extern "C" int32_t arx_encoder_attention(arx_encoder* h, const void* qkv, const int32_t* lens, int32_t n_seqs, int32_t max_len,
-                                         void* ctx, void* stream) {
+static int attention_tap(arx_encoder* h, const void* qkv, const int32_t* lens, int32_t n_seqs, int32_t max_len, void* ctx, void* stream,
+                         bool prescaled) {
     ARX_REQUIRE(h && qkv && lens && ctx, "null pointer argument");
     ARX_REQUIRE(n_seqs > 0 && n_seqs <= h->max_seqs && max_len > 0 && max_len <= 512, "bad n_seqs/max_len");
     hipStream_t st = (hipStream_t)stream;
@@ -539,9 +557,20 @@
     ARX_HIP_CHECK(hipGetLastError());
     uint16_t* q0 = h->qkv; uint16_t* c0 = h->ctx;
     h->qkv = (uint16_t*)qkv; h->ctx = (uint16_t*)ctx;
-    const int rc = launch_attn(h, n_seqs, max_len, st);
+    const int rc = launch_attn(h, n_seqs, max_len, st, prescaled);
     h->qkv = q0; h->ctx = c0;
     return rc;
+}
+
+extern "C" int32_t arx_encoder_attention(arx_encoder* h, const void* qkv, const int32_t* lens, int32_t n_seqs, int32_t max_len,
+                                         void* ctx, void* stream) {
+    return attention_tap(h, qkv, lens, n_seqs, max_len, ctx, stream, false);
+}
+
+extern "C" int32_t arx_encoder_attention_prescaled(arx_encoder* h, const void* qkv, const int32_t* lens, int32_t n_seqs, int32_t max_len,
+                                                   void* ctx, void* stream) {
+    ARX_REQUIRE(h && h->q_prescaled, "the handle does not run the pre-scaled attention form");
+    return attention_tap(h, qkv, lens, n_seqs, max_len, ctx, stream, true);
 }
 
 static void launch_ln_finalize(int T, int nparts, const float* ps, const float* pq, int64_t ld, const int32_t* n_rows, float inv_h,
@@ -630,7 +659,18 @@
                                int32_t N, int32_t K, void* stream) {
     ARX_REQUIRE(W && gamma && beta && bias && Wf && s && c, "null pointer argument");
     ARX_REQUIRE(N > 0 && K > 0, "bad sizes");
-    fold_ln_kernel<<<cdiv(N, 4), 256, 0, (hipStream_t)stream>>>((const uint16_t*)W, gamma, beta, bias, (uint16_t*)Wf, s, c, (int)N, (int)K);
+    fold_ln_kernel<<<cdiv(N, 4), 256, 0, (hipStream_t)stream>>>((const uint16_t*)W, gamma, beta, bias, (uint16_t*)Wf, s, c, (int)N, (int)K, 0, 1.0f);
+    ARX_HIP_CHECK(hipGetLastError());
+    return ARX_OK;
+}
+
+extern "C" int32_t arx_fold_ln_scaled(const void* W, const float* gamma, const float* beta, const float* bias, void* Wf, float* s, float* c,
+                                      int32_t N, int32_t K, int32_t n_scaled, float alpha, void* stream) {
+    ARX_REQUIRE(W && bias && Wf && s && c, "null pointer argument");
+    ARX_REQUIRE((gamma == nullptr) == (beta == nullptr), "gamma and beta come together");
+    ARX_REQUIRE(N > 0 && K > 0 && n_scaled >= 0 && n_scaled <= N, "bad sizes");
+    fold_ln_kernel<<<cdiv(N, 4), 256, 0, (hipStream_t)stream>>>((const uint16_t*)W, gamma, beta, bias, (uint16_t*)Wf, s, c, (int)N, (int)K, (int)n_scaled,
+                                                                alpha);
     ARX_HIP_CHECK(hipGetLastError());
     return ARX_OK;
 }
@@ -714,14 +754,15 @@
         const arx_layer_weights& L = h->layers[li];
         EpiParams ep;
         if (li == 0) {
-            ep = EpiParams{h->qkv, 3 * (int64_t)H, L.b_qkv, nullptr, 0};
-            if ((rc = launch_gemm<EPI_BIAS>(ARX_K_GEMM_QKV, gv, h->x, H, (const uint16_t*)L.w_qkv, H, T, 3 * H, H, ep, st, h->small_ws)) != ARX_OK) return rc;
+            ep = EpiParams{h->qkv, 3 * (int64_t)H, h->q_prescaled ? h->c_qkv[0] : L.b_qkv, nullptr, 0};
+            const uint16_t* w0 = h->q_prescaled ? h->wqkv_f[0] : (const uint16_t*)L.w_qkv;
+            if ((rc = launch_gemm<EPI_BIAS>(ARX_K_GEMM_QKV, gv, h->x, H, w0, H, T, 3 * H, H, ep, st, h->small_ws)) != ARX_OK) return rc;
         } else {
             ep = EpiParams{h->qkv, 3 * (int64_t)H, h->c_qkv[li], nullptr, 0};
             ep.a_sum = h->st2_sum; ep.a_sq = h->st2_sq; ep.s_vec = h->s_qkv[li]; ep.inv_h = inv_h; ep.eps = c.ln_eps;
             if ((rc = launch_gemm<EPI_LN_BIAS>(ARX_K_GEMM_QKV, gv, h->x, H, h->wqkv_f[li], H, T, 3 * H, H, ep, st, h->small_ws)) != ARX_OK) return rc;
         }
-        if ((rc = launch_attn(h, n_seqs, max_len, st)) != ARX_OK) return rc;
+        if ((rc = launch_attn(h, n_seqs, max_len, st, h->q_prescaled)) != ARX_OK) return rc;
         ep = EpiParams{h->x1, H, L.b_o, h->x, H};
         ep.o_sum = h->part_s; ep.o_sq = h->part_q; ep.o_ld = tp; ep.inv_h = inv_h; ep.eps = c.ln_eps;
         ep.fin_mean = h->st1_sum; ep.fin_rstd = h->st1_sq;
diff --git a/arxiv_rag_amd/csrc/encoder_kernels.h b/arxiv_rag_amd/csrc/encoder_kernels.h
--- a/arxiv_rag_amd/csrc/encoder_kernels.h
+++ b/arxiv_rag_amd/csrc/encoder_kernels.h
@@ -322,11 +322,11 @@
 };
 __device__ __forceinline__ int attn_bias_off(int c) { return c == 0 ? 0 : (c == 1 ? 20 : (c == 2 ? 36 : 52)); }
 
-template <int DH, bool HAS_BIAS, int NW>
-__global__ __launch_bounds__(NW * 64, NW / 2) void attention_tr_kernel(const uint16_t* __restrict__ qkv, uint16_t* __restrict__ ctx,
-                                                                        const int32_t* __restrict__ cu,
-                                                                        const float* __restrict__ bias_tbl, int H,
-                                                                        float scale_log2e, int dev_word, unsigned long long* dev_stamps) {
+template <int DH, bool HAS_BIAS, int NW, bool PRESCALED>
+__device__ __forceinline__ void attention_tr_body(const uint16_t* __restrict__ qkv, uint16_t* __restrict__ ctx,
+                                                  const int32_t* __restrict__ cu,
+                                                  const float* __restrict__ bias_tbl, int H,
+                                                  float scale_log2e, int dev_word, unsigned long long* dev_stamps) {
     constexpr int NT = NW * 64;
     constexpr int CPR = DH / 8;
     constexpr int RPB = 256 / (DH * 2);
@@ -457,9 +457,15 @@
 #pragma unroll
             for (int d = 0; d < DB; ++d) vp[d] = (lds_cptr)vb[d];
         }
+        constexpr bool SEED = PRESCALED && HAS_BIAS;
         bf16x8 kf[KS];
 #pragma unroll
         for (int ks = 0; ks < KS; ++ks) kf[ks] = *reinterpret_cast<const __attribute__((address_space(3))) bf16x8*>(kp[ks]);
+        f32x4 sb[4];
+        if constexpr (SEED) {
+#pragma unroll
+            for (int g4 = 0; g4 < 4; ++g4) sb[g4] = *reinterpret_cast<const __attribute__((address_space(3))) f32x4*>(bp + 8 * g4);
+        }
         auto advance = [&](int n) {
             bp += 32 * n;
             asm volatile("" : "+v"(bp));
@@ -474,13 +480,15 @@
             constexpr int OFF = decltype(off_tag)::value;
             f32x16 s;
 #pragma unroll
-            for (int r = 0; r < 16; ++r) s[r] = 0.f;
+            for (int r = 0; r < 16; ++r) s[r] = SEED ? sb[r >> 2][r & 3] : 0.f;
 #pragma unroll
             for (int ks = 0; ks < KS; ++ks) s = __builtin_amdgcn_mfma_f32_32x32x16_bf16(kf[ks], qf[ks], s, 0, 0, 0);
             __builtin_amdgcn_sched_barrier(0);
             f32x4 bv[4];
-#pragma unroll
-            for (int g4 = 0; g4 < 4; ++g4) bv[g4] = HAS_BIAS ? *reinterpret_cast<const __attribute__((address_space(3))) f32x4*>(bp + OFF * 32 + 8 * g4) : f32x4{0.f, 0.f, 0.f, 0.f};
+            if constexpr (!PRESCALED) {
+#pragma unroll
+                for (int g4 = 0; g4 < 4; ++g4) bv[g4] = HAS_BIAS ? *reinterpret_cast<const __attribute__((address_space(3))) f32x4*>(bp + OFF * 32 + 8 * g4) : f32x4{0.f, 0.f, 0.f, 0.f};
+            }
             s16x4 vt[DB][4];
 #pragma unroll
             for (int d = 0; d < DB; ++d)
@@ -493,7 +501,8 @@
             for (int g4 = 0; g4 < 4; ++g4)
 #pragma unroll
                 for (int e = 0; e < 4; e += 2) {
-                    f32x2 v = __builtin_elementwise_fma(f32x2{s[g4 * 4 + e], s[g4 * 4 + e + 1]}, sc2, f32x2{bv[g4][e], bv[g4][e + 1]});
+                    f32x2 v = f32x2{s[g4 * 4 + e], s[g4 * 4 + e + 1]};
+                    if constexpr (!PRESCALED) v = __builtin_elementwise_fma(v, sc2, f32x2{bv[g4][e], bv[g4][e + 1]});
                     if (MASKED) {
                         v[0] = (kt * 32 + 8 * g4 + 4 * hh + e < L) ? v[0] : -INFINITY;
                         v[1] = (kt * 32 + 8 * g4 + 4 * hh + e + 1 < L) ? v[1] : -INFINITY;
@@ -510,6 +519,10 @@
             if (!MASKED) {
 #pragma unroll
                 for (int ks = 0; ks < KS; ++ks) kf[ks] = *reinterpret_cast<const __attribute__((address_space(3))) bf16x8*>(kp[ks] + (OFF + 1) * 32 * ROWB);
+                if constexpr (SEED) {
+#pragma unroll
+                    for (int g4 = 0; g4 < 4; ++g4) sb[g4] = *reinterpret_cast<const __attribute__((address_space(3))) f32x4*>(bp + (OFF + 1) * 32 + 8 * g4);
+                }
             }
             __builtin_amdgcn_sched_barrier(0);
             bf16x8 pf[2];
@@ -551,7 +564,8 @@
     const char* vptr[DB];
     lds_bases(bptr, kptr, vptr);
     constexpr float THR = 8.0f;
-    const float inv_scale = 1.0f / scale_log2e;
+    const float sc = PRESCALED ? 1.0f : scale_log2e;
+    const float inv_scale = PRESCALED ? 1.0f : 1.0f / scale_log2e;
     lsum = f32x4{0.f, 0.f, 0.f, 0.f};
     auto tile = [&](auto masked_tag, auto first_tag, int kt) {
         constexpr bool MASKED = decltype(masked_tag)::value;
@@ -571,7 +585,7 @@
             if (HAS_BIAS) bv = *reinterpret_cast<const f32x4*>(bptr + 8 * g4);
 #pragma unroll
             for (int e = 0; e < 4; ++e) {
-                float v = fmaf(s[g4 * 4 + e], scale_log2e, bv[e]);
+                float v = fmaf(s[g4 * 4 + e], sc, bv[e]);
                 if (MASKED) v = (kt * 32 + 8 * g4 + 4 * hh + e < L) ? v : -INFINITY;
                 s[g4 * 4 + e] = v;
             }
@@ -661,6 +675,22 @@
 #ifdef ARX_DEV_VARIANTS
     if (dev_stamps && (threadIdx.x & 63) == 0) atomicMax(&dev_stamps[4 * lin + 2], (unsigned long long)wall_clock64());
 #endif
+}
+
+template <int DH, bool HAS_BIAS, int NW>
+__global__ __launch_bounds__(NW * 64, NW / 2) void attention_tr_kernel(const uint16_t* __restrict__ qkv, uint16_t* __restrict__ ctx,
+                                                                        const int32_t* __restrict__ cu,
+                                                                        const float* __restrict__ bias_tbl, int H,
+                                                                        float scale_log2e, int dev_word, unsigned long long* dev_stamps) {
+    attention_tr_body<DH, HAS_BIAS, NW, false>(qkv, ctx, cu, bias_tbl, H, scale_log2e, dev_word, dev_stamps);
+}
+
+template <int DH, bool HAS_BIAS, int NW>
+__global__ __launch_bounds__(NW * 64, NW / 2) void attention_tr_prescaled_kernel(const uint16_t* __restrict__ qkv, uint16_t* __restrict__ ctx,
+                                                                                  const int32_t* __restrict__ cu,
+                                                                                  const float* __restrict__ bias_tbl, int H, int dev_word,
+                                                                                  unsigned long long* dev_stamps) {
+    attention_tr_body<DH, HAS_BIAS, NW, true>(qkv, ctx, cu, bias_tbl, H, 1.0f, dev_word, dev_stamps);
 }
 
 #ifdef ARX_DEV_VARIANTS
@@ -1330,20 +1360,21 @@
 __global__ __launch_bounds__(256) void fold_ln_kernel(const uint16_t* __restrict__ W, const float* __restrict__ gamma,
                                                        const float* __restrict__ beta, const float* __restrict__ bias,
                                                        uint16_t* __restrict__ Wf, float* __restrict__ s, float* __restrict__ c,
-                                                       int N, int K) {
+                                                       int N, int K, int n_scaled, float alpha) {
     const int lane = threadIdx.x & 63;
     const int n = blockIdx.x * 4 + (threadIdx.x >> 6);
     if (n >= N) return;
+    const float a = n < n_scaled ? alpha : 1.0f;
     float ss = 0.f, cc = 0.f;
     for (int k = lane; k < K; k += 64) {
         const float w = bf16_bits_to_f32(W[(int64_t)n * K + k]);
-        const bf16_t wf = (bf16_t)(w * gamma[k]);
+        const bf16_t wf = (bf16_t)((gamma ? w * gamma[k] : w) * a);
         Wf[(int64_t)n * K + k] = __builtin_bit_cast(uint16_t, wf);
         ss += (float)wf;
-        cc = fmaf(beta[k], w, cc);
+        if (beta) cc = fmaf(beta[k], w, cc);
     }
     ss = wave_sum(ss); cc = wave_sum(cc);
-    if (lane == 0) { s[n] = ss; c[n] = bias[n] + cc; }
+    if (lane == 0) { s[n] = ss; c[n] = (bias[n] + cc) * a; }
 }
 
 __global__ __launch_bounds__(256) void adjacent_cosine_kernel(const float* __restrict__ e, int64_t ld, int n, int D,
diff --git a/include/arx.h b/include/arx.h
--- a/include/arx.h
+++ b/include/arx.h
@@ -79,6 +79,7 @@
 #define ARX_ATTN_RING        2
 #define ARX_ATTN_RING16      4
 #define ARX_ATTN_STAGED      8
+#define ARX_ATTN_TRANSPOSED_UNSCALED_Q 16
 #define ARX_ENC_EXPLICIT_LAYERNORM 1
 typedef struct {
     int32_t struct_bytes;
@@ -97,6 +98,8 @@
 
 int32_t arx_encoder_attention(arx_encoder* h, const void* qkv, const int32_t* lens, int32_t n_seqs, int32_t max_len,
                               void* ctx, void* stream);
+int32_t arx_encoder_attention_prescaled(arx_encoder* h, const void* qkv, const int32_t* lens, int32_t n_seqs, int32_t max_len,
+                                        void* ctx, void* stream);
 
 int32_t arx_encoder_debug_hidden(arx_encoder* h, int32_t layer_slot, float* dst, int32_t n_tokens, void* stream);
 
@@ -404,6 +407,8 @@
 } arx_gemm_epilogue;
 int32_t arx_gemm_bf16_ex(const void* A, const void* W, void* C, int32_t M, int32_t N, int32_t K, const arx_gemm_epilogue* e, void* stream);
 
+int32_t arx_fold_ln_scaled(const void* W, const float* gamma, const float* beta, const float* bias, void* Wf, float* s, float* c,
+                           int32_t N, int32_t K, int32_t n_scaled, float alpha, void* stream);
 int32_t arx_fold_ln(const void* W, const float* gamma, const float* beta, const float* bias, void* Wf, float* s, float* c,
                     int32_t N, int32_t K, void* stream);
 
```
